# mataiyuan/ASD-SLAM

Hardware: AMD Instinct MI355X
Metric: frames/sec end-to-end tracking+LocalBA, KITTI 00 mono @2000 keypoints (higher is better)
Workload: dtype f32

## Files before the change

### asd-slam_amd/capi.py

```python
import ctypes as C
import os

import numpy as np

_HERE = os.path.dirname(os.path.abspath(__file__))


def lib_path():
    return os.environ.get("ASDHIP_LIB") or os.path.join(_HERE, "libasdhip.so")


class AsdError(RuntimeError):
    def __init__(self, code, msg):
        super().__init__(f"libasdhip error {code}: {msg}")
        self.code = code


class asd_config(C.Structure):
    _fields_ = [("n_features", C.c_int32), ("scale_factor", C.c_float), ("n_levels", C.c_int32),
                ("ini_th_fast", C.c_int32), ("min_th_fast", C.c_int32), ("max_width", C.c_int32),
                ("max_height", C.c_int32), ("max_patches", C.c_int32), ("device", C.c_int32)]


BANK_MAX_ROWS = 1 << 22
# ... 974 lines not shown
        kfs, rows, rank, fixed, pose = i32(ck), i32(cp), i32(cp), i32(cf), i32(cq)
        pfix, e_point, e_pose, e_kf, e_idx = np.full(max(cq, 1), 9, np.uint8), i32(ce), i32(ce), i32(ce), i32(ce)
        e_oct = np.full(max(ce, 1), 99, np.uint8)
        xw = np.full((max(cp, 1), 3), np.nan) if want_Xw else None
        a = asd_ba_graph_args()
        a.kf, a.n_neigh, a.neigh = int(kf), len(neigh), neigh.ctypes.data
        a.kf_capacity, a.local_kfs = ck, kfs.ctypes.data
        a.point_capacity, a.local_rows, a.point_rank = cp, rows.ctypes.data, rank.ctypes.data
        a.fixed_capacity, a.fixed_kfs = cf, fixed.ctypes.data
        a.pose_capacity, a.pose_kfs, a.pose_fixed = cq, pose.ctypes.data, pfix.ctypes.data
        a.edge_capacity, a.e_point, a.e_pose, a.e_kf, a.e_idx, a.e_octave = ce, e_point.ctypes.data, e_pose.ctypes.data, e_kf.ctypes.data, e_idx.ctypes.data, e_oct.ctypes.data
        a.Xw = None if xw is None else xw.ctypes.data
        a.n_local_kfs = a.n_points = a.n_fixed = a.n_poses = a.n_edges = -1
        rc = self.lib.asd_local_ba_graph(self.ctx, C.byref(a))
        out = dict(n_local_kfs=a.n_local_kfs, n_points=a.n_points, n_fixed=a.n_fixed, n_poses=a.n_poses, n_edges=a.n_edges)
        if rc == 0:
            out.update(local_kfs=kfs[:a.n_local_kfs].copy(), local_rows=rows[:a.n_points].copy(), point_rank=rank[:a.n_points].copy(),
                       fixed_kfs=fixed[:a.n_fixed].copy(), pose_kfs=pose[:a.n_poses].copy(), pose_fixed=pfix[:a.n_poses].copy(),
                       e_point=e_point[:a.n_edges].copy(), e_pose=e_pose[:a.n_edges].copy(), e_kf=e_kf[:a.n_edges].copy(),
                       e_idx=e_idx[:a.n_edges].copy(), e_octave=e_oct[:a.n_edges].copy())
            if want_Xw:
                out["Xw"] = xw[:a.n_points].copy()
        return rc, out

    def local_ba_graph(self, kf, neigh, want_Xw=False, caps=(64, 4096, 64, 128, 16384)):
        rc, out = self.local_ba_graph_raw(kf, neigh, caps, want_Xw)
        if rc == -5 and out["n_local_kfs"] > 0:
            rc, out = self.local_ba_graph_raw(kf, neigh, (out["n_local_kfs"], out["n_points"], out["n_fixed"], out["n_poses"], out["n_edges"]), want_Xw)
        self._chk(rc)
        return out

    def local_ba_apply_raw(self, erase, n_points, apply, bad_capacity):
        erase = _c(erase, np.uint8)
        bad, ref = np.full(max(int(bad_capacity), 1), -7, np.int32), np.full(max(int(n_points), 1), -7, np.int32)
        a = asd_ba_apply_args()
        a.n_edges, a.erase, a.apply, a.n_erased = len(erase), erase.ctypes.data, int(bool(apply)), -1
        a.bad_capacity, a.bad_rows, a.n_bad, a.n_points, a.new_ref = int(bad_capacity), bad.ctypes.data, -1, int(n_points), ref.ctypes.data
        rc = self.lib.asd_local_ba_apply(self.ctx, C.byref(a))
        out = dict(n_erased=a.n_erased, n_bad=a.n_bad)
        if rc == 0:
            out.update(bad_rows=bad[:a.n_bad].copy(), new_ref=ref[:int(n_points)].copy())
        return rc, out

    def local_ba_apply(self, erase, n_points, apply=False, bad_capacity=64):
        rc, out = self.local_ba_apply_raw(erase, n_points, apply, bad_capacity)
        if rc == -5 and out["n_bad"] > bad_capacity:
            rc, out = self.local_ba_apply_raw(erase, n_points, apply, out["n_bad"])
        self._chk(rc)
        return out

    def map_debug(self):
        out = np.zeros(8, np.int64)
        self._chk(self.lib.asd_debug_map(self.ctx, _p(out)))
        return tuple(int(x) for x in out)

    def track_local_points_map(self, slot_cur, n_cur, Tcw, K, occupied, cur_Xw, th, nn_ratio, pose7, cos_limit=0.5, obs_positive=None, split=False):
        Tcw, K, occupied, cur_Xw = _c(Tcw, np.float32), _c(K, np.float32), _c(occupied, np.uint8), _c(cur_Xw, np.float32)
        match, outl = np.empty(n_cur, np.int32), np.empty(max(n_cur, 1), np.uint8)
        pose = _c(pose7, np.float64).copy()
        n, ninl = C.c_int32(), C.c_int32()
        if split:
            self._chk(self.lib.asd_track_async(self.ctx))
        self._chk(self.lib.asd_track_local_points_map(self.ctx, slot_cur, _p(Tcw), _p(K), C.c_float(cos_limit), _p(occupied), _p(cur_Xw), C.c_float(th),
                                                      C.c_float(nn_ratio), _p(None if obs_positive is None else _c(obs_positive, np.uint8)), _p(pose),
                                                      _p(match), C.byref(n), _p(outl), C.byref(ninl)))
        if split:
            self._track_job = (match, n, pose, outl, ninl, n_cur)
            return None
        return match, n.value, pose, outl[:n_cur], ninl.value

    def bank_put(self, first_row, desc):
        desc = _c(desc, np.float32)
        self._chk(self.lib.asd_bank_put(self.ctx, first_row, desc.shape[0], _p(desc)))

    def bank_put_from_frame(self, slot, first_row, n):
        self._chk(self.lib.asd_bank_put_from_frame(self.ctx, slot, first_row, n))

    def bank_get(self, first_row, n, desc=True, attr=True):
        d = np.empty((max(n, 0), 128), np.float32) if desc else None
        a = np.empty((max(n, 0), 8), np.float32) if attr else None
        self.lib.asd_debug_bank_get.restype = C.c_int32
        self._chk(self.lib.asd_debug_bank_get(self.ctx, C.c_int32(first_row), C.c_int32(n), _p(d), _p(a)))
        return d, a

    def match_project_frame_bank(self, slot_cur, slot_last, n_cur, has_mp, Xw, mp_rows, Tcw, K, th, check_ori=True, obs_positive=None):
        has_mp, Xw, mp_rows = _c(has_mp, np.uint8), _c(Xw, np.float32), _c(mp_rows, np.int32)
        Tcw, K = _c(Tcw, np.float32), _c(K, np.float32)
        out = np.empty(n_cur, np.int32)
        n = C.c_int32()
        self._chk(self.lib.asd_match_project_frame_bank(self.ctx, slot_cur, slot_last, _p(has_mp), _p(Xw), _p(mp_rows),
                                                        _p(Tcw), _p(K), C.c_float(th), int(check_ori), _p(out), C.byref(n),
                                                        _p(None if obs_positive is None else _c(obs_positive, np.uint8))))
        return out, n.value

    def match_project_points_bank(self, slot_cur, n_cur, in_view, proj, level, view_cos, rows, occupied, th, nn_ratio, obs_positive=None):
        in_view, proj, level = _c(in_view, np.uint8), _c(proj, np.float32), _c(level, np.int32)
        view_cos, rows, occupied = _c(view_cos, np.float32), _c(rows, np.int32), _c(occupied, np.uint8)
        out = np.empty(n_cur, np.int32)
        n = C.c_int32()
        self._chk(self.lib.asd_match_project_points_bank(self.ctx, slot_cur, len(in_view), _p(in_view), _p(proj), _p(level),
                                                         _p(view_cos), _p(rows), _p(occupied), C.c_float(th),
                                                         C.c_float(nn_ratio), _p(out), C.byref(n),
                                                         _p(None if obs_positive is None else _c(obs_positive, np.uint8))))
        return out, n.value

    def frustum(self, slot_cur, Xw, normal, min_dist, max_dist, Tcw, K, cos_limit=0.5):
        Xw, normal = _c(Xw, np.float32), _c(normal, np.float32)
        min_dist, max_dist = _c(min_dist, np.float32), _c(max_dist, np.float32)
        Tcw, K = _c(Tcw, np.float32), _c(K, np.float32)
        n = Xw.shape[0]
        in_view = np.zeros(n, np.uint8)
        proj = np.zeros((n, 2), np.float32)
        level = np.zeros(n, np.int32)
        vc = np.zeros(n, np.float32)
        self._chk(self.lib.asd_frustum(self.ctx, slot_cur, n, _p(Xw), _p(normal), _p(min_dist), _p(max_dist),
                                       _p(Tcw), _p(K), C.c_float(cos_limit), _p(in_view), _p(proj), _p(level),
                                       _p(vc)))
        return in_view, proj, level, vc

    def match_init(self, slot1, slot2, prev_matched, window=100, nn_ratio=0.9, check_ori=True):
        pm = _c(prev_matched, np.float32).copy()
        out = np.empty(pm.shape[0], np.int32)
        n = C.c_int32()
        self._chk(self.lib.asd_match_init(self.ctx, slot1, slot2, _p(pm), window, C.c_float(nn_ratio),
                                          int(check_ori), _p(out), C.byref(n)))
        return out, n.value, pm

    def match_bow(self, slot_kf, slot_f, n_f, nodes_kf, nodes_f, has_mp_kf, nn_ratio=0.7, check_ori=True):
        fa, ka = make_fv(nodes_kf)
        fb, kb = make_fv(nodes_f)
        has = _c(has_mp_kf, np.uint8)
        out = np.empty(n_f, np.int32)
        n = C.c_int32()
        self._chk(self.lib.asd_match_bow(self.ctx, slot_kf, slot_f, C.byref(fa), C.byref(fb), _p(has), C.c_float(nn_ratio),
                                         int(check_ori), _p(out), C.byref(n)))
        return out, n.value

    def match_bow_kf(self, slot1, slot2, n1, nodes1, nodes2, has_mp1, has_mp2, nn_ratio=0.85, check_ori=True):
        fa, ka = make_fv(nodes1)
        fb, kb = make_fv(nodes2)
        h1, h2 = _c(has_mp1, np.uint8), _c(has_mp2, np.uint8)
        out = np.empty(n1, np.int32)
        n = C.c_int32()
        self._chk(self.lib.asd_match_bow_kf(self.ctx, slot1, slot2, C.byref(fa), C.byref(fb), _p(h1), _p(h2), C.c_float(nn_ratio),
                                            int(check_ori), _p(out), C.byref(n)))
        return out, n.value

    def match_triangulate(self, slot1, slot2, n1, nodes1, nodes2, has_mp1, has_mp2, F12, ex, ey, check_ori=False):
        fa, ka = make_fv(nodes1)
        fb, kb = make_fv(nodes2)
        h1, h2, F = _c(has_mp1, np.uint8), _c(has_mp2, np.uint8), _c(F12, np.float32)
        out = np.empty(n1, np.int32)
        n = C.c_int32()
        self._chk(self.lib.asd_match_triangulate(self.ctx, slot1, slot2, C.byref(fa), C.byref(fb), _p(h1), _p(h2), _p(F),
                                                 C.c_float(ex), C.c_float(ey), int(check_ori), _p(out), C.byref(n)))
        return out, n.value

    def pose_optimize(self, pose7, Xw, obs, inv_sigma2, K):
        pose = _c(pose7, np.float64).copy()
        Xw, obs, inv_sigma2, K = (_c(a, np.float64) for a in (Xw, obs, inv_sigma2, K))
        n = Xw.shape[0]
        outlier = np.zeros(n, np.uint8)
        ninl = C.c_int32()
        self._chk(self.lib.asd_pose_optimize(self.ctx, _p(pose), n, _p(Xw), _p(obs), _p(inv_sigma2), _p(K),
                                             _p(outlier), C.byref(ninl)))
        return pose, outlier, ninl.value
# ... 296 lines not shown
```

### asd-slam_amd/csrc/ctx.h

```cpp
#pragma once
#include <hip/hip_runtime.h>

#include <atomic>
#include <cstdarg>
#include <cstdio>
#include <cstdlib>
#include <cstring>
#include <functional>
#include <mutex>
#include <string>
#include <vector>

#include "../../include/asd_slam.h"

#define ASD_HIP_CHECK(ctx, expr)                                                          \
  do {                                                                                    \
    hipError_t _e = (expr);                                                               \
    if (_e != hipSuccess) {                                                               \
      (ctx)->set_error("%s failed: %s (%s:%d)", #expr, hipGetErrorString(_e), __FILE__, __LINE__); \
      return ASD_ERR_HIP;                                                                 \
    }                                                                                     \
  } while (0)

struct AsdPerDeviceOnce {
  std::atomic<uint64_t> bits{0};
  bool need(int dev) const { return !((bits.load(std::memory_order_acquire) >> (dev & 63)) & 1); }
  void done(int dev) { bits.fetch_or(1ull << (dev & 63), std::memory_order_release); }
};

struct AsdDevBuf {
  void* p = nullptr;
  size_t cap = 0, used = 0;
  hipError_t reserve(size_t bytes) {
    used = 0;
    if (bytes <= cap) return hipSuccess;
    if (p) (void)hipFree(p);
    p = nullptr; cap = 0;
    const size_t want = bytes + bytes / 4 + 4096;
    const hipError_t e = hipMalloc(&p, want);
    if (e == hipSuccess) cap = want;
    return e;
  }
  template <typename T> T* carve(size_t count) {
    char* q = static_cast<char*>(p) + used;
    used += (count * sizeof(T) + 255) / 256 * 256;
    return reinterpret_cast<T*>(q);
  }
  static size_t padded(size_t bytes) { return (bytes + 255) / 256 * 256; }
  void release() { if (p) (void)hipFree(p); p = nullptr; cap = used = 0; }
};


hipError_t asd_copy_rows(hipStream_t st, void* dst, const void* src, size_t bytes);

#if defined(__HIPCC__)
#define asd_syncthreads() do { asm volatile("s_waitcnt lgkmcnt(0)" ::: "memory"); __syncthreads(); } while (0)
__device__ inline int asd_syncthreads_or(int pred) { asm volatile("s_waitcnt lgkmcnt(0)" ::: "memory"); return __syncthreads_or(pred); }
#endif


struct AsdWinQuery { float x, y, r; int min_level, max_level, qrow; };
struct AsdBetweenArgs {
  int n_cur, n_last, n_cand;
  const int* match1;
  const double* io1;
  const float* Xw_last;
  const int* last_cand;
  float T_pred[16];
  uint8_t* occ;
  float* cur_Xw;
  uint8_t* skip;
  float* T1;
};
#if defined(__HIPCC__)
template <class F>
__device__ inline void asd_frustum_bank_point(const F& a, const float* T_dev, const uint8_t* skip, const int q) {
#pragma clang fp contract(off)
  AsdWinQuery Q{0.f, 0.f, 0.f, 0, 0, -1};
  const int row = a.rows[q];
  const float4 A0 = reinterpret_cast<const float4*>(a.attr)[2 * (size_t)row], A1 = reinterpret_cast<const float4*>(a.attr)[2 * (size_t)row + 1];
  a.xw_out[3 * (size_t)q] = A0.x; a.xw_out[3 * (size_t)q + 1] = A0.y; a.xw_out[3 * (size_t)q + 2] = A0.z;
  if (!skip || !skip[q]) {
    float T[16], Ow[3];
    for (int i = 0; i < 16; ++i) T[i] = T_dev[i];
    for (int i = 0; i < 3; ++i) Ow[i] = T_dev[16 + i];
    const float P[3] = {A0.x, A0.y, A0.z}, Pn[3] = {A0.w, A1.x, A1.y};
    const float min_dist = A1.z, max_dist = A1.w;
    float Pc[3];
    for (int r = 0; r < 3; ++r) {
      const float t0 = T[r * 4 + 0] * P[0] + T[r * 4 + 1] * P[1] + T[r * 4 + 2] * P[2];
      Pc[r] = (float)((double)t0 + (double)T[r * 4 + 3]);
    }
    bool ok = !(Pc[2] < 0.0f);
    const float invz = 1.0f / Pc[2];
    const float u = a.fx * Pc[0] * invz + a.cx, v = a.fy * Pc[1] * invz + a.cy;
    if (u < a.min_x || u > a.max_x || v < a.min_y || v > a.max_y) ok = false;
    const float maxD = 1.2f * max_dist, minD = 0.8f * min_dist;
    const float PO[3] = {P[0] - Ow[0], P[1] - Ow[1], P[2] - Ow[2]};
    const double nn = (double)PO[0] * PO[0] + (double)PO[1] * PO[1] + (double)PO[2] * PO[2];
    const float dist = (float)sqrt(nn);
    if (dist < minD || dist > maxD) ok = false;
    const double dot = (double)PO[0] * Pn[0] + (double)PO[1] * Pn[1] + (double)PO[2] * Pn[2];
    const float vc = (float)(dot / dist);
    if (vc < a.cos_limit) ok = false;
    if (ok) {
      const float ratio = max_dist / dist;
      int lvl = 0;
      for (int k = 1; k < a.n_levels; ++k) lvl += ratio >= a.level_thr[k];
      float r = vc > 0.998 ? 2.5f : 4.0f;
      if (a.bfactor) r *= a.th;
      Q = AsdWinQuery{u, v, r * a.scale[lvl], lvl - 1, lvl, row};
    }
  }
  a.queries[q] = Q;
}
__device__ inline void asd_between_body(const AsdBetweenArgs& a_dev, const int t, const int nt) {
#pragma clang fp contract(off)
  const AsdBetweenArgs a = a_dev;
  __shared__ int s_nmatch;
  if (t == 0) s_nmatch = 0;
  for (int c = t; c < a.n_cand; c += nt) a.skip[c] = 0;
  asd_syncthreads();
  const uint8_t* outl = reinterpret_cast<const uint8_t*>(a.io1 + 8);
  int mine = 0;
  for (int j = t; j < a.n_cur; j += nt) {
    const int i = a.match1[j];
    mine += i >= 0;
    const int src = i >= 0 ? i : 0;
    for (int k = 0; k < 3; ++k) a.cur_Xw[3 * (size_t)j + k] = a.n_last > 0 ? a.Xw_last[3 * (size_t)src + k] : 0.f;
    const bool keep = i >= 0 && !outl[j];
    a.occ[j] = keep ? 1 : 0;
    if (i >= 0 && a.last_cand) { const int c = a.last_cand[i]; if (c >= 0 && c < a.n_cand) a.skip[c] = 1; }
  }
  if (mine) atomicAdd(&s_nmatch, mine);
  asd_syncthreads();
  if (t == 0) {
    float T[16];
    if (s_nmatch >= 3) {
      const double* p = a.io1;
      const double x = p[0], y = p[1], z = p[2], w = p[3];
      const double tx = 2 * x, ty = 2 * y, tz = 2 * z;
      const double twx = tx * w, twy = ty * w, twz = tz * w, txx = tx * x, txy = ty * x, txz = tz * x, tyy = ty * y, tyz = tz * y, tzz = tz * z;
      const double R[9] = {1 - (tyy + tzz), txy - twz, txz + twy, txy + twz, 1 - (txx + tzz), tyz - twx, txz - twy, tyz + twx, 1 - (txx + tyy)};
      for (int i = 0; i < 3; ++i) {
        for (int j = 0; j < 3; ++j) T[i * 4 + j] = (float)R[i * 3 + j];
        T[i * 4 + 3] = (float)p[4 + i];
      }
      T[12] = T[13] = T[14] = 0.f;
      T[15] = 1.f;
    } else {
      for (int i = 0; i < 16; ++i) T[i] = a.T_pred[i];
    }
    for (int i = 0; i < 16; ++i) a.T1[i] = T[i];
    for (int i = 0; i < 3; ++i) {
      double sum = 0;
      for (int k = 0; k < 3; ++k) sum += (double)T[k * 4 + i] * (double)T[k * 4 + 3];
      a.T1[16 + i] = (float)(-1.0 * sum);
    }
  }
}
#endif

struct AsdXfer {
  char* h = nullptr;
  char* d = nullptr;
  size_t cap = 0, used = 0;
  hipError_t begin(hipStream_t st, size_t bytes) {
    used = 0;
    bytes += 4096;
    if (bytes <= cap) return hipSuccess;
    if (h) { (void)hipStreamSynchronize(st); (void)hipHostFree(h); (void)hipFree(d); }
    h = nullptr; d = nullptr; cap = 0;
    const size_t want = bytes + bytes / 2;
    hipError_t e = hipHostMalloc(&h, want);
    if (e == hipSuccess) e = hipMalloc(&d, want);
    if (e == hipSuccess) cap = want;
    return e;
  }
  size_t reserve(size_t bytes) { const size_t off = used; used += (bytes + 255) / 256 * 256; return off; }
  size_t add(const void* src, size_t bytes) { const size_t off = reserve(bytes); memcpy(h + off, src, bytes); return off; }
  size_t zeros(size_t bytes) { const size_t off = reserve(bytes); memset(h + off, 0, bytes); return off; }
  hipError_t upload(hipStream_t st) {
    if (!used) return hipSuccess;
    static const bool by_kernel = getenv("ASD_UPLOAD_COPY") == nullptr;
    return by_kernel ? asd_copy_rows(st, d, h, (used + 15) / 16 * 16) : hipMemcpyAsync(d, h, used, hipMemcpyHostToDevice, st);
  }
  hipError_t download(hipStream_t st) { return used ? hipMemcpyAsync(h, d, used, hipMemcpyDeviceToHost, st) : hipSuccess; }
  template <typename T> T* dev(size_t off) { return reinterpret_cast<T*>(d + off); }
  template <typename T> T* host(size_t off) { return reinterpret_cast<T*>(h + off); }
  void release() { if (h) (void)hipHostFree(h); if (d) (void)hipFree(d); h = d = nullptr; cap = used = 0; }
};

struct AsdFrameSlot {
  int n = 0;
  float min_x = 0, max_x = 0, min_y = 0, max_y = 0;
  float inv_w = 0, inv_h = 0;
  std::vector<asd_keypoint> kps;
// ... 192 lines not shown
```

### asd-slam_amd/csrc/matcher.h

```cpp
#pragma once
#include <chrono>
#include <vector>

#include "ctx.h"

using WinQuery = AsdWinQuery;

struct MatcherState {
  int q_cap = 0, cand_cap = 0, h_cand_cap = 0, qdesc_cap = 0;
  int last_total[4] = {1 << 15, 1 << 15, 1 << 15, 1 << 15};
  WinQuery *d_queries = nullptr, *h_queries = nullptr;
  int *d_q_off = nullptr, *d_q_cnt = nullptr, *d_total = nullptr, *d_idx = nullptr;
  float* d_dist = nullptr;
  int *h_q = nullptr;
  int* h_idx = nullptr;
  float* h_dist = nullptr;
  float *d_qdesc = nullptr, *h_qdesc = nullptr;
  float* d_bank = nullptr;
  int bank_cap = 0;
  float* d_attr = nullptr;
  int attr_cap = 0;
  float* d_cxw = nullptr;
  size_t cxw_cap = 0;
  float* h_attr[2] = {nullptr, nullptr};
  size_t h_attr_cap[2] = {0, 0};
  hipEvent_t ev_attr[2] = {nullptr, nullptr};
  int attr_turn = 0;
  bool replay_host = false;
};

struct SearchResult { const int* off; const int* cnt; const int* idx; const float* dist; };

struct ListQuery { int qrow, cbeg, cend, ooff; };

MatcherState* matcher_state(asd_ctx* ctx);
AsdFrameSlot* matcher_slot(asd_ctx* ctx, int s);
int matcher_ensure_queries(asd_ctx* ctx, MatcherState* m, int nq);
int matcher_ensure_qdesc(asd_ctx* ctx, MatcherState* m, int n);
int matcher_upload_qdesc(asd_ctx* ctx, MatcherState* m, const float* desc, int n);
int matcher_window_search(asd_ctx* ctx, MatcherState* m, const AsdFrameSlot& F, int nq, const float* d_q, SearchResult* res, int kind = 3);
int matcher_list_search(asd_ctx* ctx, MatcherState* m, const AsdFrameSlot& A, const AsdFrameSlot& B, const asd_feature_vector* fvA,
                        const asd_feature_vector* fvB, const uint8_t* skipA, bool skip_if_set, std::vector<ListQuery>& lq, const float** dist_out);

int matcher_check_bank_rows(asd_ctx* ctx, const MatcherState* m, const int32_t* rows, const uint8_t* used, int n, bool attr_too);

int matcher_replay_frame(asd_ctx* ctx, MatcherState* m, const AsdFrameSlot& C, const AsdFrameSlot& L, const float* d_q, const uint8_t* obs_pos,
                         int check_orientation, int32_t* match_cur, int32_t* n_matches, std::chrono::steady_clock::time_point tm0);
int matcher_replay_points(asd_ctx* ctx, MatcherState* m, const AsdFrameSlot& F, int n_mp, const float* d_q, const uint8_t* occupied,
                          const uint8_t* obs_pos, float nn_ratio, int32_t* match_cur, int32_t* n_matches);

template <class Make>
int matcher_fill_queries(asd_ctx* ctx, MatcherState* m, int n, Make make) {
  const int rc = matcher_ensure_queries(ctx, m, n);
  if (rc != ASD_OK) return rc;
  for (int i = 0; i < n; ++i) {
    WinQuery& Q = m->h_queries[i];
    Q = WinQuery{0.f, 0.f, 0.f, 0, 0, -1};
    make(i, Q);
  }
  return ASD_OK;
}
inline void matcher_transform(const float* T, const float* X, float* out) {
  for (int r = 0; r < 3; ++r) {
    const float t0 = T[r * 4 + 0] * X[0] + T[r * 4 + 1] * X[1] + T[r * 4 + 2] * X[2];
    out[r] = (float)((double)t0 + (double)T[r * 4 + 3]);
  }
}
inline void matcher_camera_centre(const float* R, int ld, const float* t, int inc, float* Ow) {
  for (int i = 0; i < 3; ++i) {
    double sum = 0;
    for (int k = 0; k < 3; ++k) sum += (double)R[k * ld + i] * (double)t[k * inc];
    Ow[i] = (float)(-1.0 * sum);
  }
}
inline void matcher_keyframe_centre(const float* Tcw, float* Ow) {
  for (int i = 0; i < 3; ++i) {
    const float t0 = Tcw[0 * 4 + i] * Tcw[3] + Tcw[1 * 4 + i] * Tcw[7] + Tcw[2 * 4 + i] * Tcw[11];
    Ow[i] = (float)((double)t0 * -1.0);
  }
}
```

### asd-slam_amd/csrc/matcher.hip

```cpp
#include <algorithm>
#include <chrono>
#include <cmath>
#include <cstring>
#include <array>
#include <functional>
#include <memory>

#include "matcher.h"
#include "resolve2.h"

namespace {

constexpr int GC = ASD_GRID_COLS, GR = ASD_GRID_ROWS;

struct GridDev {
  const float4* kp;
  const int* cell_start;
  const int* cell_items;
  float min_x, min_y, inv_w, inv_h;
};

#ifndef ASD_SEARCH_WAVES
#define ASD_SEARCH_WAVES 8
#endif
constexpr int kSearchWaves = ASD_SEARCH_WAVES;
constexpr int kSearchCols = 16;
constexpr int kSearchList = 128;
struct SortArgs {
  const uint8_t* occ;
  float th_cut;
  uint16_t* top_idx;
};
template <bool SORT>
__global__ __launch_bounds__(64 * kSearchWaves) void k_window_search(GridDev G, const WinQuery* __restrict__ queries, int nq,
                                                       const float* __restrict__ qdesc, const float* __restrict__ cdesc,
                                                       int* __restrict__ q_off, int* __restrict__ q_cnt,
                                                       int* __restrict__ total, int cap, int* __restrict__ out_idx,
                                                       float* __restrict__ out_dist, SortArgs S) {
  const int lane = threadIdx.x & 63, wave = threadIdx.x >> 6;
  const int q = blockIdx.x * kSearchWaves + wave;
  __shared__ int wg_cnt[kSearchWaves], wg_base;
  __shared__ int cand_l[kSearchWaves][kSearchList];
  __shared__ unsigned dist_l[SORT ? kSearchWaves : 1][kSearchList];
  const bool live = q < nq;
  const WinQuery Q = live ? queries[q] : WinQuery{0.f, 0.f, 0.f, 0, 0, -1};
  int cnt = 0, off = 0;
  bool empty = Q.qrow < 0;
  const int nMinCellX = max(0, (int)floorf((Q.x - G.min_x - Q.r) * G.inv_w));
  const int nMaxCellX = min(ASD_GRID_COLS - 1, (int)ceilf((Q.x - G.min_x + Q.r) * G.inv_w));
  const int nMinCellY = max(0, (int)floorf((Q.y - G.min_y - Q.r) * G.inv_h));
  const int nMaxCellY = min(ASD_GRID_ROWS - 1, (int)ceilf((Q.y - G.min_y + Q.r) * G.inv_h));
  if (nMinCellX >= ASD_GRID_COLS || nMaxCellX < 0 || nMinCellY >= ASD_GRID_ROWS || nMaxCellY < 0) empty = true;
  const bool check = (Q.min_level > 0) || (Q.max_level >= 0);
  auto accept = [&](const float4& kp) {
    const int oct = __float_as_int(kp.z);
    bool ok = true;
    if (check) {
      if (oct < Q.min_level) ok = false;
      if (Q.max_level >= 0 && oct > Q.max_level) ok = false;
    }
    const float dx = kp.x - Q.x, dy = kp.y - Q.y;
    if (!(fabsf(dx) < Q.r && fabsf(dy) < Q.r)) ok = false;
    return ok;
  };
  const int qrow_u = __builtin_amdgcn_readfirstlane(Q.qrow < 0 ? 0 : Q.qrow);
  auto distance = [&](int idx) {
    const float4* a = reinterpret_cast<const float4*>(qdesc + (size_t)qrow_u * 128);
    const float4* bb = reinterpret_cast<const float4*>(cdesc + (size_t)idx * 128);
    float sqd = 0.f;
#pragma unroll 16
    for (int k = 0; k < 32; ++k) {
      const float4 x = a[k], y = bb[k];
      float d;
      d = x.x - y.x; sqd = sqd + d * d;
      d = x.y - y.y; sqd = sqd + d * d;
      d = x.z - y.z; sqd = sqd + d * d;
      d = x.w - y.w; sqd = sqd + d * d;
    }
    return sqd;
  };
  auto score = [&](int idx, int p) {
    const float sqd = distance(idx);
    out_idx[off + p] = idx;
    out_dist[off + p] = sqd;
  };
  auto walk = [&](int pass) {
    int pos = 0;
    for (int ix = nMinCellX; ix <= nMaxCellX; ++ix) {
      const int b = G.cell_start[ix * ASD_GRID_ROWS + nMinCellY], e = G.cell_start[ix * ASD_GRID_ROWS + nMaxCellY + 1];
      for (int base = b; base < e; base += 64) {
        const int it = base + lane;
        bool ok = false;
        int idx = 0;
        if (it < e) {
          idx = G.cell_items[it];
          ok = accept(G.kp[idx]);
          if (SORT && ok && S.occ && S.occ[idx]) ok = false;
        }
        const unsigned long long m = __ballot(ok);
        if (pass == 1 && ok) {
          const int p = pos + __popcll(m & ((1ull << lane) - 1));
          if (off + p < cap) score(idx, p);
        }
        pos += __popcll(m);
      }
    }
    return pos;
  };
  const int ncol = nMaxCellX - nMinCellX + 1;
  bool fast = !empty && ncol <= kSearchCols;
  int cb[kSearchCols], ce[kSearchCols];
  if (fast) {
#pragma unroll
    for (int c = 0; c < kSearchCols; ++c) {
      const int ix = min(nMinCellX + c, nMaxCellX);
      cb[c] = G.cell_start[ix * ASD_GRID_ROWS + nMinCellY];
      ce[c] = G.cell_start[ix * ASD_GRID_ROWS + nMaxCellY + 1];
    }
#pragma unroll
    for (int c = 0; c < kSearchCols; ++c) {
      if (c >= ncol) ce[c] = cb[c];
      if (ce[c] - cb[c] > 64) fast = false;
    }
  }
  if (fast) {
    int idxc[kSearchCols];
#pragma unroll
    for (int c = 0; c < kSearchCols; ++c) idxc[c] = cb[c] + lane < ce[c] ? G.cell_items[cb[c] + lane] : -1;
    float4 kpc[kSearchCols];
#pragma unroll
    for (int c = 0; c < kSearchCols; ++c) kpc[c] = idxc[c] >= 0 ? G.kp[idxc[c]] : make_float4(0.f, 0.f, 0.f, 0.f);
    if (SORT && S.occ) {
      uint8_t oc[kSearchCols];
#pragma unroll
      for (int c = 0; c < kSearchCols; ++c) oc[c] = idxc[c] >= 0 ? S.occ[idxc[c]] : (uint8_t)0;
#pragma unroll
      for (int c = 0; c < kSearchCols; ++c) if (oc[c]) idxc[c] = -1;
    }
    int pos = 0;
#pragma unroll
    for (int c = 0; c < kSearchCols; ++c) {
      const bool ok = idxc[c] >= 0 && accept(kpc[c]);
      const unsigned long long m = __ballot(ok);
      if (ok) {
        const int p = pos + __popcll(m & ((1ull << lane) - 1));
        if (p < kSearchList) cand_l[wave][p] = idxc[c];
      }
      pos += __popcll(m);
    }
    cnt = pos;
    if (cnt > kSearchList) fast = false;
  } else if (!empty) {
    cnt = walk(0);
  }
  if (lane == 0) wg_cnt[wave] = cnt;
  asd_syncthreads();
  if (threadIdx.x == 0) {
    int sum = 0;
    for (int w = 0; w < kSearchWaves; ++w) sum += wg_cnt[w];
    wg_base = sum ? atomicAdd(total, sum) : 0;
  }
  asd_syncthreads();
  off = wg_base;
  for (int w = 0; w < wave; ++w) off += wg_cnt[w];
  if (!SORT) {
    if (cnt > 0) {
      if (fast) {
        for (int p = lane; p < cnt; p += 64)
          if (off + p < cap) score(cand_l[wave][p], p);
      } else {
        (void)walk(1);
      }
    }
    if (lane == 0 && live) { q_cnt[q] = cnt; q_off[q] = cnt ? off : 0; }
    return;
  }
  if (!live) return;
  const bool fits = off + cnt <= cap;
  int n_keep = 0, s_off = off;
  auto put = [&](int base, int rank, int idx, float d) {
    out_idx[base + rank] = idx;
    out_dist[base + rank] = d;
    if (rank < kTop) S.top_idx[(size_t)q * kTop + rank] = (uint16_t)idx;
  };
  if (cnt > 0 && fits) {
    if (fast) {
      const bool v0 = lane < cnt, v1 = lane + 64 < cnt;
      const int i0 = v0 ? cand_l[wave][lane] : 0, i1 = v1 ? cand_l[wave][lane + 64] : 0;
      const float d0 = v0 ? distance(i0) : 0.f, d1 = v1 ? distance(i1) : 0.f;
      const unsigned b0 = __float_as_uint(d0), b1 = __float_as_uint(d1);
      if (v0) dist_l[wave][lane] = b0;
      if (v1) dist_l[wave][lane + 64] = b1;
      asm volatile("s_waitcnt lgkmcnt(0)" ::: "memory");
      __builtin_amdgcn_wave_barrier();
      int r0 = 0, r1 = 0;
      for (int i = 0; i < cnt; ++i) {
        const unsigned di = dist_l[wave][i];
        r0 += (di < b0) || (di == b0 && i < lane);
        r1 += (di < b1) || (di == b1 && i < lane + 64);
      }
      if (v0) put(off, r0, i0, d0);
      if (v1) put(off, r1, i1, d1);
      n_keep = __popcll(__ballot(v0 && d0 <= S.th_cut)) + __popcll(__ballot(v1 && d1 <= S.th_cut));
    } else {
      (void)walk(1);
      asm volatile("s_waitcnt vmcnt(0)" ::: "memory");
      __builtin_amdgcn_fence(__ATOMIC_SEQ_CST, "workgroup");
      s_off = cap + off;
      constexpr int R = 4;
      for (int pb = 0; pb < cnt; pb += 64 * R) {
        int pi[R], ii[R], rk[R]; unsigned bi[R];
#pragma unroll
        for (int r = 0; r < R; ++r) {
          pi[r] = pb + 64 * r + lane;
          const int pc = min(pi[r], cnt - 1);
          ii[r] = __hip_atomic_load(out_idx + off + pc, __ATOMIC_RELAXED, __HIP_MEMORY_SCOPE_AGENT);
          bi[r] = __float_as_uint(__hip_atomic_load(out_dist + off + pc, __ATOMIC_RELAXED, __HIP_MEMORY_SCOPE_AGENT));
          rk[r] = 0;
        }
        for (int cbase = 0; cbase < cnt; cbase += kSearchList) {
          __builtin_amdgcn_wave_barrier();
          for (int i = lane; i < kSearchList; i += 64)
            dist_l[wave][i] = cbase + i < cnt ? __float_as_uint(__hip_atomic_load(out_dist + off + cbase + i, __ATOMIC_RELAXED, __HIP_MEMORY_SCOPE_AGENT)) : 0xffffffffu;
          asm volatile("s_waitcnt lgkmcnt(0)" ::: "memory");
          __builtin_amdgcn_wave_barrier();
          const int m = min(kSearchList, cnt - cbase);
          for (int i = 0; i < m; ++i) {
            const unsigned di = dist_l[wave][i];
#pragma unroll
            for (int r = 0; r < R; ++r) rk[r] += (di < bi[r]) || (di == bi[r] && cbase + i < pi[r]);
          }
          asm volatile("s_waitcnt lgkmcnt(0)" ::: "memory");
        }
#pragma unroll
        for (int r = 0; r < R; ++r) {
          const bool v = pi[r] < cnt;
          if (v) put(s_off, rk[r], ii[r], __uint_as_float(bi[r]));
          n_keep += __popcll(__ballot(v && __uint_as_float(bi[r]) <= S.th_cut));
        }
      }
    }
  }
  if (lane < kTop && lane >= (fits ? cnt : 0)) S.top_idx[(size_t)q * kTop + lane] = 0xffffu;
  if (lane == 0) { q_cnt[q] = n_keep; q_off[q] = cnt ? s_off : 0; }
}

__global__ __launch_bounds__(256) void k_list_dist(const ListQuery* __restrict__ queries, int nq,
                                                   const int* __restrict__ cand, const float* __restrict__ qdesc,
                                                   const float* __restrict__ cdesc, float* __restrict__ out) {
  const int lane = threadIdx.x & 63;
  const int q = blockIdx.x * 4 + (threadIdx.x >> 6);
  if (q >= nq) return;
  const ListQuery Q = queries[q];
  const float4* a = reinterpret_cast<const float4*>(qdesc + (size_t)Q.qrow * 128);
  for (int t = Q.cbeg + lane; t < Q.cend; t += 64) {
    const float4* b = reinterpret_cast<const float4*>(cdesc + (size_t)cand[t] * 128);
    float sqd = 0.f;
#pragma unroll 8
    for (int k = 0; k < 32; ++k) {
      const float4 x = a[k], y = b[k];
      float d;
      d = x.x - y.x; sqd = sqd + d * d;
      d = x.y - y.y; sqd = sqd + d * d;
      d = x.z - y.z; sqd = sqd + d * d;
      d = x.w - y.w; sqd = sqd + d * d;
    }
    out[Q.ooff + (t - Q.cbeg)] = sqd;
  }
}

constexpr int kDistinctMax = 64;
__global__ __launch_bounds__(256) void k_distinctive(const float* __restrict__ desc, const int* __restrict__ set_start, int* __restrict__ best_out) {
  extern __shared__ __attribute__((aligned(16))) float smem_d[];
  const int s0 = set_start[blockIdx.x], n = set_start[blockIdx.x + 1] - s0;
  float* sd = smem_d;
  float* D = smem_d + kDistinctMax * 132;
  float* med = D + kDistinctMax * (kDistinctMax + 1);
// ... 11 lines not shown
      const float4* y = reinterpret_cast<const float4*>(sd + j * 132);
      for (int k = 0; k < 32; ++k) {
        const float4 a = x[k], b = y[k];
        float d;
        d = a.x - b.x; acc = acc + d * d;
        d = a.y - b.y; acc = acc + d * d;
        d = a.z - b.z; acc = acc + d * d;
        d = a.w - b.w; acc = acc + d * d;
      }
    }
    D[i * (n + 1) + j] = acc;
  }
  asd_syncthreads();
  const int kth = (int)(0.5 * (n - 1));
  for (int p = t; p < n * n; p += 256) {
    const int i = p / n, j = p % n;
    const float v = D[i * (n + 1) + j];
    int rank = 0;
    for (int l = 0; l < n; ++l) {
      const float u = D[i * (n + 1) + l];
      rank += (u < v || (u == v && l < j)) ? 1 : 0;
    }
    if (rank == kth) med[i] = v;
  }
  asd_syncthreads();
  if (t == 0) {
    float best_median = 100;
    int best = 0;
    for (int i = 0; i < n; ++i)
      if (med[i] < best_median) { best_median = med[i]; best = i; }
    best_out[blockIdx.x] = best;
  }
}

__global__ __launch_bounds__(256) void k_dist_matrix(const float* __restrict__ a, int na, const float* __restrict__ b,
                                                     int nb, float* __restrict__ out) {
  __shared__ float4 sa[16][32];
  const int j = blockIdx.x * 256 + threadIdx.x;
  const int i0 = blockIdx.y * 16;
  for (int idx = threadIdx.x; idx < 16 * 32; idx += 256) {
    const int r = idx >> 5, c = idx & 31;
    const int ia = min(i0 + r, na - 1);
    sa[r][c] = reinterpret_cast<const float4*>(a + (size_t)ia * 128)[c];
  }
  asd_syncthreads();
  const float4* brow = reinterpret_cast<const float4*>(b + (size_t)min(j, nb - 1) * 128);
  float acc[16];
#pragma unroll
  for (int r = 0; r < 16; ++r) acc[r] = 0.f;
  for (int k = 0; k < 32; ++k) {
    const float4 y = brow[k];
#pragma unroll
    for (int r = 0; r < 16; ++r) {
      const float4 x = sa[r][k];
      float d;
      d = x.x - y.x; acc[r] = acc[r] + d * d;
      d = x.y - y.y; acc[r] = acc[r] + d * d;
      d = x.z - y.z; acc[r] = acc[r] + d * d;
      d = x.w - y.w; acc[r] = acc[r] + d * d;
    }
  }
  if (j < nb)
    for (int r = 0; r < 16; ++r)
      if (i0 + r < na) out[(size_t)(i0 + r) * nb + j] = acc[r];
}


__global__ __launch_bounds__(256) void k_copy16(const uint4* __restrict__ src, uint4* __restrict__ dst, size_t n16) {
  for (size_t i = (size_t)blockIdx.x * 256 + threadIdx.x; i < n16; i += (size_t)gridDim.x * 256) dst[i] = src[i];
}
hipError_t copy_rows(hipStream_t st, void* dst, const void* src, size_t bytes) {
  const size_t n16 = bytes / 16;
  if (!n16) return hipSuccess;
  hipLaunchKernelGGL(k_copy16, dim3((unsigned)std::min<size_t>((n16 + 255) / 256, 1024)), dim3(256), 0, st, static_cast<const uint4*>(src),
                     static_cast<uint4*>(dst), n16);
  return hipGetLastError();
}

template <int KIND, int QPT>
__global__ __launch_bounds__(kResolve2Threads) void k_resolve2(Resolve2Args a) {
  resolve2_body<KIND, QPT, kResolve2Threads>(a);
}

struct UploadTail {
  const uint4* src; uint4* dst;
  size_t first16, n16;
  int q_blocks;
};
__device__ inline bool upload_tail_block(const UploadTail& u) {
  if ((int)blockIdx.x < u.q_blocks) return false;
  const size_t nb = gridDim.x - u.q_blocks;
  for (size_t i = u.first16 + (size_t)(blockIdx.x - u.q_blocks) * 256 + threadIdx.x; i < u.n16; i += nb * 256) u.dst[i] = u.src[i];
  return true;
}
constexpr int kUploadTailBlocks = 64;

struct FrustumArgs {
  int n, n_levels, bfactor;
  const float* Xw; const float* normal; const float* min_dist; const float* max_dist;
  const int* rows;
  float T[16], Ow[3];
  float fx, fy, cx, cy, min_x, max_x, min_y, max_y, cos_limit, th;
  float level_thr[ASD_MAX_LEVELS], scale[ASD_MAX_LEVELS];
  WinQuery* queries;
  UploadTail up;
  const float* T_dev; const float* attr; const uint8_t* skip; float* xw_out;
};
__global__ __launch_bounds__(256) void k_frustum_queries(FrustumArgs a) {
  if (upload_tail_block(a.up)) return;
  const int q = blockIdx.x * 256 + threadIdx.x;
  if (q >= a.n) return;
  WinQuery Q{0.f, 0.f, 0.f, 0, 0, -1};
  if (a.attr) {
    if (a.T_dev) asd_frustum_bank_point(a, a.T_dev, a.skip, q);
    else {
      float Tl[19];
      for (int i = 0; i < 16; ++i) Tl[i] = a.T[i];
      for (int i = 0; i < 3; ++i) Tl[16 + i] = a.Ow[i];
      asd_frustum_bank_point(a, Tl, a.skip, q);
    }
    return;
  }
  const float* P = a.Xw + 3 * (size_t)q;
  float Pc[3];
  for (int r = 0; r < 3; ++r) {
    const float t0 = a.T[r * 4 + 0] * P[0] + a.T[r * 4 + 1] * P[1] + a.T[r * 4 + 2] * P[2];
    Pc[r] = (float)((double)t0 + (double)a.T[r * 4 + 3]);
  }
  bool ok = !(Pc[2] < 0.0f);
  const float invz = 1.0f / Pc[2];
  const float u = a.fx * Pc[0] * invz + a.cx, v = a.fy * Pc[1] * invz + a.cy;
  if (u < a.min_x || u > a.max_x || v < a.min_y || v > a.max_y) ok = false;
  const float maxD = 1.2f * a.max_dist[q], minD = 0.8f * a.min_dist[q];
  const float PO[3] = {P[0] - a.Ow[0], P[1] - a.Ow[1], P[2] - a.Ow[2]};
  const double nn = (double)PO[0] * PO[0] + (double)PO[1] * PO[1] + (double)PO[2] * PO[2];
  const float dist = (float)sqrt(nn);
  if (dist < minD || dist > maxD) ok = false;
  const float* Pn = a.normal + 3 * (size_t)q;
  const double dot = (double)PO[0] * Pn[0] + (double)PO[1] * Pn[1] + (double)PO[2] * Pn[2];
  const float vc = (float)(dot / dist);
  if (vc < a.cos_limit) ok = false;
  if (ok) {
    const float ratio = a.max_dist[q] / dist;
    int lvl = 0;
    for (int k = 1; k < a.n_levels; ++k) lvl += ratio >= a.level_thr[k];
    float r = vc > 0.998 ? 2.5f : 4.0f;
    if (a.bfactor) r *= a.th;
    Q = WinQuery{u, v, r * a.scale[lvl], lvl - 1, lvl, a.rows ? a.rows[q] : q};
  }
  a.queries[q] = Q;
}

struct ProjectArgs {
  int n;
  const uint8_t* has_mp; const float* Xw; const int* rows; const float4* kp_last;
  float T[16];
  float fx, fy, cx, cy, min_x, max_x, min_y, max_y, th;
  float scale[ASD_MAX_LEVELS];
  WinQuery* queries;
  UploadTail up;
};
__global__ __launch_bounds__(256) void k_project_queries(ProjectArgs a) {
  if (upload_tail_block(a.up)) return;
  const int i = blockIdx.x * 256 + threadIdx.x;
  if (i >= a.n) return;
  WinQuery Q{0.f, 0.f, 0.f, 0, 0, -1};
  if (a.has_mp[i]) {
    const float* X = a.Xw + 3 * (size_t)i;
    float Xc[3];
    for (int r = 0; r < 3; ++r) {
      const float t0 = a.T[r * 4 + 0] * X[0] + a.T[r * 4 + 1] * X[1] + a.T[r * 4 + 2] * X[2];
      Xc[r] = (float)((double)t0 + (double)a.T[r * 4 + 3]);
    }
    const float invzc = (float)(1.0 / (double)Xc[2]);
    if (!(invzc < 0)) {
      const float u = a.fx * Xc[0] * invzc + a.cx;
      const float v = a.fy * Xc[1] * invzc + a.cy;
      if (!(u < a.min_x || u > a.max_x) && !(v < a.min_y || v > a.max_y)) {
        const int oct = __float_as_int(a.kp_last[i].z);
        Q = WinQuery{u, v, a.th * a.scale[oct], oct - 1, oct + 1, a.rows ? a.rows[i] : i};
      }
    }
  }
  a.queries[i] = Q;
}

int ensure_cands_dev(asd_ctx* ctx, MatcherState* m, size_t n) {
  if (n <= (size_t)m->cand_cap) return ASD_OK;
  if (n > ((size_t)1 << 30)) { ctx->set_error("candidate buffers: %zu entries asked for", n); return ASD_ERR_CAPACITY; }
  const size_t cap = std::max(n + n / 2, (size_t)1 << 18);
  if (m->d_idx) { (void)hipFree(m->d_idx); (void)hipFree(m->d_dist); }
  m->d_idx = nullptr; m->d_dist = nullptr;
  m->cand_cap = 0;
  ASD_HIP_CHECK(ctx, hipMalloc(&m->d_idx, 2 * cap * sizeof(int)));
  ASD_HIP_CHECK(ctx, hipMalloc(&m->d_dist, 2 * cap * sizeof(float)));
  m->cand_cap = (int)std::min(cap, (size_t)0x7fffffff);
  return ASD_OK;
}
int ensure_cands(asd_ctx* ctx, MatcherState* m, int n) {
  int rc = ensure_cands_dev(ctx, m, (size_t)n);
  if (rc != ASD_OK) return rc;
  if (m->cand_cap <= m->h_cand_cap) return ASD_OK;
  if (m->h_idx) { (void)hipHostFree(m->h_idx); (void)hipHostFree(m->h_dist); }
  m->h_idx = nullptr; m->h_dist = nullptr;
  m->h_cand_cap = 0;
  ASD_HIP_CHECK(ctx, hipHostMalloc(&m->h_idx, (size_t)m->cand_cap * sizeof(int)));
  ASD_HIP_CHECK(ctx, hipHostMalloc(&m->h_dist, (size_t)m->cand_cap * sizeof(float)));
  m->h_cand_cap = m->cand_cap;
  return ASD_OK;
}
}

MatcherState* matcher_state(asd_ctx* ctx) {
  if (!ctx->matcher) {
    MatcherState* m = new MatcherState();
    m->replay_host = ctx->match_replay_host;
    ctx->matcher = m;
  }
  return static_cast<MatcherState*>(ctx->matcher);
}

int matcher_ensure_queries(asd_ctx* ctx, MatcherState* m, int nq) {
  if (nq <= m->q_cap) return ASD_OK;
  const int cap = std::max(nq * 3 / 2, 8192);
  if (m->d_queries) { (void)hipFree(m->d_queries); (void)hipHostFree(m->h_queries); (void)hipFree(m->d_q_off); (void)hipHostFree(m->h_q); }
  m->q_cap = 0;
  ASD_HIP_CHECK(ctx, hipMalloc(&m->d_queries, (size_t)cap * sizeof(WinQuery)));
  ASD_HIP_CHECK(ctx, hipHostMalloc(&m->h_queries, (size_t)cap * sizeof(WinQuery)));
  ASD_HIP_CHECK(ctx, hipMalloc(&m->d_q_off, ((size_t)2 * cap + 4) * sizeof(int)));
  ASD_HIP_CHECK(ctx, hipHostMalloc(&m->h_q, ((size_t)2 * cap + 4) * sizeof(int)));
  m->q_cap = cap;
  return ASD_OK;
}
int matcher_ensure_qdesc(asd_ctx* ctx, MatcherState* m, int n) {
  if (n <= m->qdesc_cap) return ASD_OK;
  const int cap = std::max(n * 3 / 2, 8192);
  if (m->d_qdesc) { (void)hipFree(m->d_qdesc); (void)hipHostFree(m->h_qdesc); }
  m->qdesc_cap = 0;
  ASD_HIP_CHECK(ctx, hipMalloc(&m->d_qdesc, (size_t)cap * 512));
  ASD_HIP_CHECK(ctx, hipHostMalloc(&m->h_qdesc, (size_t)cap * 512));
  m->qdesc_cap = cap;
  return ASD_OK;
}

int matcher_upload_qdesc(asd_ctx* ctx, MatcherState* m, const float* desc, int n) {
  int rc = matcher_ensure_qdesc(ctx, m, n);
  if (rc != ASD_OK) return rc;
  memcpy(m->h_qdesc, desc, (size_t)n * 512);
  ASD_HIP_CHECK(ctx, hipMemcpyAsync(m->d_qdesc, m->h_qdesc, (size_t)n * 512, hipMemcpyHostToDevice, ctx->stream));
  return ASD_OK;
}

AsdFrameSlot* matcher_slot(asd_ctx* ctx, int s) {
  if (!ctx || s < 0 || s >= ASD_MAX_FRAMES) return nullptr;
  return &ctx->frames[s];
}

int matcher_window_search(asd_ctx* ctx, MatcherState* m, const AsdFrameSlot& F, int nq, const float* d_q, SearchResult* res, int kind) {
  if (asd_track_busy(ctx, "matcher call")) return ASD_ERR_INVALID;
  static const bool timing = getenv("ASD_TIMING") != nullptr;
  static double tacc[4][3]; static long tcalls[4];
  const auto tw0 = std::chrono::steady_clock::now();
  auto tw1 = tw0;
  int rc = ensure_cands(ctx, m, 1);
  if (rc != ASD_OK) return rc;
  hipStream_t st = ctx->stream;
  int* d_off = m->d_q_off;
  int* d_cnt = m->d_q_off + nq;
  int* d_total = m->d_q_off + 2 * nq;
  const int optimistic = std::min(m->cand_cap, std::max(4096, m->last_total[kind] + m->last_total[kind] / 4));
  for (int attempt = 0; attempt < 2; ++attempt) {
    ASD_HIP_CHECK(ctx, hipMemcpyAsync(m->d_queries, m->h_queries, (size_t)nq * sizeof(WinQuery), hipMemcpyHostToDevice, st));
    ASD_HIP_CHECK(ctx, hipMemsetAsync(d_total, 0, sizeof(int), st));
    GridDev G{F.d_kp, F.d_cell_start, F.d_cell_items, F.min_x, F.min_y, F.inv_w, F.inv_h};
    ASD_HIP_CHECK(ctx, hipEventRecord(ctx->ev0, st));
    hipLaunchKernelGGL(k_window_search<false>, dim3((nq + kSearchWaves - 1) / kSearchWaves), dim3(64 * kSearchWaves), 0, st, G, m->d_queries, nq, d_q, F.d_desc, d_off, d_cnt,
                       d_total, m->cand_cap, m->d_idx, m->d_dist, SortArgs{});
    ASD_HIP_CHECK(ctx, hipGetLastError());
    ASD_HIP_CHECK(ctx, hipEventRecord(ctx->ev1, st));
    ASD_HIP_CHECK(ctx, hipMemcpyAsync(m->h_q, d_off, ((size_t)2 * nq + 1) * sizeof(int), hipMemcpyDeviceToHost, st));
    ASD_HIP_CHECK(ctx, hipMemcpyAsync(m->h_idx, m->d_idx, (size_t)optimistic * sizeof(int), hipMemcpyDeviceToHost, st));
    ASD_HIP_CHECK(ctx, hipMemcpyAsync(m->h_dist, m->d_dist, (size_t)optimistic * sizeof(float), hipMemcpyDeviceToHost, st));
    tw1 = std::chrono::steady_clock::now();
    ASD_HIP_CHECK(ctx, hipStreamSynchronize(st));
    const int total = m->h_q[2 * nq];
    m->last_total[kind] = total;
    if (total > m->cand_cap) {
      if ((rc = ensure_cands(ctx, m, total)) != ASD_OK) return rc;
      continue;
    }
    if (total > optimistic) {
      ASD_HIP_CHECK(ctx, hipMemcpyAsync(m->h_idx + optimistic, m->d_idx + optimistic, (size_t)(total - optimistic) * sizeof(int), hipMemcpyDeviceToHost, st));
      ASD_HIP_CHECK(ctx, hipMemcpyAsync(m->h_dist + optimistic, m->d_dist + optimistic, (size_t)(total - optimistic) * sizeof(float), hipMemcpyDeviceToHost, st));
      ASD_HIP_CHECK(ctx, hipStreamSynchronize(st));
    }
    break;
  }
  ASD_HIP_CHECK(ctx, hipEventElapsedTime(&ctx->ms_match, ctx->ev0, ctx->ev1));
  if (timing) {
    const auto tw2 = std::chrono::steady_clock::now();
    auto ms = [](auto a, auto b) { return std::chrono::duration<double, std::milli>(b - a).count(); };
    tacc[kind][0] += ms(tw0, tw1); tacc[kind][1] += ms(tw1, tw2); tacc[kind][2] += ctx->ms_match;
    if (++tcalls[kind] % 200 == 0)
      fprintf(stderr, "[window_search kind %d] enqueue %.3f sync %.3f kernel %.3f ms, %d candidates copied (last total %d)\n", kind,
              tacc[kind][0] / tcalls[kind], tacc[kind][1] / tcalls[kind], tacc[kind][2] / tcalls[kind], optimistic, m->last_total[kind]);
  }
  res->off = m->h_q;
  res->cnt = m->h_q + nq;
  res->idx = m->h_idx;
  res->dist = m->h_dist;
  return ASD_OK;
}

namespace {
size_t resolve_lds_bytes(int kind, int n_cur, int nq) {
  return resolve2_fixed_lds(kind, n_cur) + (size_t)n_cur * 4 + (kind == 1 ? ((size_t)nq * 2 + 15) / 16 * 16 : 0);
}
bool replay_on_device(const MatcherState* m, int kind, int n_cur, int nq) {
  const int max_q = kind == 0 ? kResolve2Threads * 4 : std::min(kResolve2MaxRounds * 512, 65535);
  return !m->replay_host && n_cur > 0 && n_cur < 65536 && nq <= max_q && resolve_lds_bytes(kind, n_cur, nq) <= 96 * 1024;
}

struct StageSolver {
  const float* d_points;
  const uint8_t* d_hold;
  const float* d_own;
  double pose0[7];
  const double* d_pose0;
  double K[4];
  double* io;
  double* d_io_dev;
  const AsdBetweenArgs* d_between;
};
enum QuerySource { kQueriesUploaded, kQueriesProject, kQueriesFrustum };
enum StageUpload { kUploadElsewhere, kUploadCopy, kUploadCarried };
struct TrackStage {
  int kind, nq;
  const AsdFrameSlot* F;
  QuerySource source;
  ProjectArgs project;
  FrustumArgs frustum;
  StageUpload upload;
  const WinQuery* d_queries;
  const float* d_qdesc;
  const float4* kp_last;
  const uint8_t* d_obs_pos;
  const uint8_t* d_occupied;
  int check_ori;
  float nn_ratio;
  int *d_off, *d_cnt;
  int* d_total;
  uint16_t* d_top;
  int *d_out, *h_out;
  bool timed;
  bool has_solver;
  StageSolver solver;
};

UploadTail upload_tail(const AsdXfer& up, int nq, bool carried) {
  return UploadTail{reinterpret_cast<const uint4*>(up.h), reinterpret_cast<uint4*>(up.d), carried ? ((size_t)nq * sizeof(WinQuery) + 255) / 256 * 16 : 0,
                    carried ? (up.used + 15) / 16 : 0, (nq + 255) / 256};
}

ProjectArgs project_args(const asd_ctx* ctx, const AsdFrameSlot& C, const AsdFrameSlot& L, const float* Tcw, const float* K, float th) {
  ProjectArgs pa{};
  pa.n = L.n; pa.kp_last = L.d_kp;
  memcpy(pa.T, Tcw, sizeof pa.T);
  pa.fx = K[0]; pa.fy = K[1]; pa.cx = K[2]; pa.cy = K[3];
  pa.min_x = C.min_x; pa.max_x = C.max_x; pa.min_y = C.min_y; pa.max_y = C.max_y; pa.th = th;
  for (int l = 0; l < ASD_MAX_LEVELS; ++l) pa.scale[l] = l < ctx->cfg.n_levels ? ctx->scale[l] : 0.f;
  return pa;
}
FrustumArgs frustum_args(const asd_ctx* ctx, const AsdFrameSlot& F, int n, const float* Tcw, const float* T_dev, const float* K, float cos_limit, float th) {
  FrustumArgs fa{};
  fa.n = n; fa.n_levels = ctx->cfg.n_levels; fa.bfactor = th != 1.0;
  if (Tcw) {
    memcpy(fa.T, Tcw, sizeof fa.T);
    matcher_camera_centre(Tcw, 4, Tcw + 3, 4, fa.Ow);
  }
  fa.T_dev = T_dev;
  fa.fx = K[0]; fa.fy = K[1]; fa.cx = K[2]; fa.cy = K[3];
  fa.min_x = F.min_x; fa.max_x = F.max_x; fa.min_y = F.min_y; fa.max_y = F.max_y;
  fa.cos_limit = cos_limit; fa.th = th;
  for (int l = 0; l < ASD_MAX_LEVELS; ++l) { fa.level_thr[l] = ctx->level_thr[l]; fa.scale[l] = l < ctx->cfg.n_levels ? ctx->scale[l] : 0.f; }
  return fa;
}
size_t resolve2_args(const MatcherState* m, const TrackStage& s, Resolve2Args* out) {
  const int n_cur = s.F->n;
  Resolve2Args a{};
  a.nq = s.nq; a.n_cur = n_cur;
  a.q_off = s.d_off; a.q_cnt = s.d_cnt; a.idx = m->d_idx; a.dist = m->d_dist; a.top_idx = s.d_top;
  a.total = s.d_total; a.cap = m->cand_cap;
  a.obs_pos = s.d_obs_pos;
  a.kp_cur = s.F->d_kp; a.kp_last = s.kp_last;
  a.check_ori = s.check_ori; a.nn_ratio = s.nn_ratio;
  a.match_cur = s.d_out; a.n_matches = s.d_out + n_cur; a.mirror = s.h_out;
  const size_t fixed = resolve_lds_bytes(s.kind, n_cur, s.nq), per = s.kind == 1 ? 6 : 2;
  a.stage_cap = (int)std::min<size_t>(((size_t)m->last_total[s.kind] * 5 / 4 + 1023) / 1024 * 1024, ((size_t)96 * 1024 - fixed) / per / 8 * 8);
  *out = a;
  return fixed + (size_t)a.stage_cap * per;
}
int resolve2_attributes(asd_ctx* ctx) {
  static AsdPerDeviceOnce attrs;
  if (!attrs.need(ctx->cfg.device)) return ASD_OK;
  const void* ks[] = {reinterpret_cast<const void*>(k_resolve2<0, 2>), reinterpret_cast<const void*>(k_resolve2<0, 4>),
                      reinterpret_cast<const void*>(k_resolve2<1, 2>), reinterpret_cast<const void*>(k_resolve2<1, 4>)};
  for (const void* k : ks) ASD_HIP_CHECK(ctx, hipFuncSetAttribute(k, hipFuncAttributeMaxDynamicSharedMemorySize, 96 * 1024));
  attrs.done(ctx->cfg.device);
  return ASD_OK;
}
hipError_t launch_resolve2(hipStream_t st, int kind, const Resolve2Args& a, size_t lds) {
  auto go = [&](auto kern) { hipLaunchKernelGGL(kern, dim3(1), dim3(kResolve2Threads), lds, st, a); };
  const bool two = a.nq <= 2 * kResolve2Threads;
  if (kind == 0) { if (two) go(k_resolve2<0, 2>); else go(k_resolve2<0, 4>); }
  else { if (two) go(k_resolve2<1, 2>); else go(k_resolve2<1, 4>); }
  return hipGetLastError();
}
bool stage_fuses(const asd_ctx* ctx, const MatcherState* m, const TrackStage& s) {
  Resolve2Args a;
  return s.has_solver && pose_chain_fused_ok(ctx, s.kind, s.nq, s.F->n, resolve2_args(m, s, &a));
}

int enqueue_stage(asd_ctx* ctx, const MatcherState* m, const TrackStage& s, bool fuse) {
  hipStream_t st = ctx->stream;
  const AsdFrameSlot& F = *s.F;
  int rc;
  if (s.upload == kUploadCopy) ASD_HIP_CHECK(ctx, ctx->up.upload(st));
  if (s.source == kQueriesProject) {
    const UploadTail& t = s.project.up;
    hipLaunchKernelGGL(k_project_queries, dim3(t.q_blocks + (t.n16 ? kUploadTailBlocks : 0)), dim3(256), 0, st, s.project);
    ASD_HIP_CHECK(ctx, hipGetLastError());
  } else if (s.source == kQueriesFrustum) {
    const UploadTail& t = s.frustum.up;
    hipLaunchKernelGGL(k_frustum_queries, dim3(t.q_blocks + (t.n16 ? kUploadTailBlocks : 0)), dim3(256), 0, st, s.frustum);
    ASD_HIP_CHECK(ctx, hipGetLastError());
  }
  if (s.timed) ASD_HIP_CHECK(ctx, hipEventRecord(ctx->ev0, st));
  const GridDev G{F.d_kp, F.d_cell_start, F.d_cell_items, F.min_x, F.min_y, F.inv_w, F.inv_h};
  const SortArgs sa{s.d_occupied, s.kind == 0 ? TH_HIGH : __builtin_huge_valf(), s.d_top};
  hipLaunchKernelGGL(k_window_search<true>, dim3((s.nq + kSearchWaves - 1) / kSearchWaves), dim3(64 * kSearchWaves), 0, st, G, s.d_queries, s.nq, s.d_qdesc, F.d_desc, s.d_off,
                     s.d_cnt, s.d_total, m->cand_cap, m->d_idx, m->d_dist, sa);
  ASD_HIP_CHECK(ctx, hipGetLastError());
  Resolve2Args ra;
  const size_t lds = resolve2_args(m, s, &ra);
  if (!fuse) {
    ASD_HIP_CHECK(ctx, launch_resolve2(st, s.kind, ra, lds));
    if (s.timed) ASD_HIP_CHECK(ctx, hipEventRecord(ctx->ev1, st));
  }
  if (s.has_solver) {
    const StageSolver& v = s.solver;
    const AsdFusedReplay fr{&ra, s.kind, s.nq, lds};
    AsdPoseChainArgs c{};
    c.n_cur = F.n; c.d_match = s.d_out; c.d_kp = F.d_kp;
    c.d_points = v.d_points; c.d_hold = v.d_hold; c.d_own = v.d_own;
    c.pose7 = v.d_pose0 ? nullptr : v.pose0; c.K = v.K;
    c.d_io = v.io; c.d_pose0 = v.d_pose0; c.d_io_dev = v.d_io_dev; c.between = v.d_between;
    c.fused = fuse ? &fr : nullptr;
    if ((rc = pose_chain_enqueue(ctx, c)) != ASD_OK) return rc;
  }
  if (fuse && s.timed) ASD_HIP_CHECK(ctx, hipEventRecord(ctx->ev1, st));
  return ASD_OK;
}
int record_chain_end(asd_ctx* ctx) {
  if (!ctx->ev_chain) ASD_HIP_CHECK(ctx, hipEventCreateWithFlags(&ctx->ev_chain, hipEventDisableTiming));
  ASD_HIP_CHECK(ctx, hipEventRecord(ctx->ev_chain, ctx->stream));
  return ASD_OK;
}

void unpack_solver_block(const double* h_io, int n_cur, bool kp_flags, const int32_t* match, const uint8_t* hold, const double* pose_start, double* pose,
                         uint8_t* outlier, int32_t* n_inliers) {
  int ne = 0;
  if (kp_flags) {
    ne = (int)(h_io[8 + (n_cur + 7) / 8] + 0.5);
    memcpy(outlier, h_io + 8, (size_t)n_cur);
  } else {
    auto edge = [&](int j) { return (hold && hold[j]) || match[j] >= 0; };
    for (int j = 0; j < n_cur; ++j) ne += edge(j);
    const uint8_t* flags = reinterpret_cast<const uint8_t*>(h_io + 8);
    for (int j = 0, e = 0; j < n_cur; ++j) outlier[j] = edge(j) && ne >= 3 ? flags[e++] : 0;
  }
  memcpy(pose, ne < 3 ? pose_start : h_io, 56);
  *n_inliers = ne < 3 ? 0 : ne - (int)(h_io[7] + 0.5);
}

struct StageInputs {
  int kind = 0, nq = 0;
  const float* d_qdesc = nullptr;
  const float4* kp_last = nullptr;
  const uint8_t* obs_pos = nullptr;
  const uint8_t* occupied = nullptr;
  int check_ori = 0;
  float nn_ratio = 0.f;
  QuerySource source = kQueriesUploaded;
  ProjectArgs project{};
  FrustumArgs frustum{};
  bool has_solver = false;
  double pose0[7] = {}, K[4] = {};
  const float* points = nullptr;
  int n_points = 0;
  const float* d_points = nullptr;
  const uint8_t* has_mp = nullptr;
  const float* own = nullptr;
  const uint8_t* hold = nullptr;
  const float* normal = nullptr;
  const float* min_dist = nullptr;
  const float* max_dist = nullptr;
  const int32_t* rows = nullptr;
  const int32_t* d_rows = nullptr;
};

int search_and_resolve(asd_ctx* ctx, MatcherState* m, const AsdFrameSlot& F, const StageInputs& in, int32_t* match_cur, int32_t* n_matches,
                       const double** solver_io = nullptr, std::function<int()>* defer = nullptr) {
  if (asd_track_busy(ctx, "matcher call")) return ASD_ERR_INVALID;
  static const bool timing = getenv("ASD_TIMING") != nullptr;
  static const bool tail_upload = getenv("ASD_UPLOAD_COPY") == nullptr;
  const int n_cur = F.n, nq = in.nq, kind = in.kind;
  const bool deferred = defer != nullptr;
  int rc = ensure_cands_dev(ctx, m, deferred ? std::max((size_t)nq * (size_t)std::max(n_cur, 1), (size_t)1) : (size_t)1);
  if (rc != ASD_OK) return rc;
  hipStream_t st = ctx->stream;
  AsdXfer &up = ctx->up, &down = ctx->down;
  const size_t io_bytes = in.has_solver ? pose_chain_io_bytes(n_cur) : 0;
  ASD_HIP_CHECK(ctx, up.begin(st, (size_t)nq * (sizeof(WinQuery) + 1 + 12 + 12 + 4 + 4 + 4) + (size_t)in.n_points * 12 + (size_t)n_cur * (1 + 12 + 1) + 16 * 256));
  ASD_HIP_CHECK(ctx, down.begin(st, ((size_t)n_cur + 16) * sizeof(int) + 256 + io_bytes));
  ASD_HIP_CHECK(ctx, ctx->scratch.reserve(AsdDevBuf::padded((size_t)nq * kTop * 2)));
  if ((rc = resolve2_attributes(ctx)) != ASD_OK || (in.has_solver && (rc = pose_chain_reserve(ctx, n_cur)) != ASD_OK)) return rc;

  TrackStage s{};
  s.kind = kind; s.nq = nq; s.F = &F;
  s.source = in.source;
  s.upload = in.source != kQueriesUploaded && tail_upload ? kUploadCarried : kUploadCopy;
  s.d_qdesc = in.d_qdesc; s.kp_last = in.kp_last; s.check_ori = in.check_ori; s.nn_ratio = in.nn_ratio;
  s.d_off = m->d_q_off; s.d_cnt = m->d_q_off + nq;
  s.d_top = ctx->scratch.carve<uint16_t>((size_t)nq * kTop);
  s.timed = timing;
  const size_t o_q = in.source == kQueriesUploaded ? up.add(m->h_queries, (size_t)nq * sizeof(WinQuery)) : up.reserve((size_t)nq * sizeof(WinQuery));
  const size_t o_total = up.zeros(sizeof(int));
  s.d_queries = up.dev<WinQuery>(o_q);
  s.d_total = up.dev<int>(o_total);
  if (in.obs_pos) s.d_obs_pos = up.dev<uint8_t>(up.add(in.obs_pos, nq));
  if (kind == 1) s.d_occupied = up.dev<uint8_t>(up.add(in.occupied, n_cur));
  const bool carried = s.upload == kUploadCarried;
  const void *q_points = nullptr, *q_has = nullptr, *q_normal = nullptr, *q_min = nullptr, *q_max = nullptr, *q_rows = nullptr;
  auto table = [&](const void* src, size_t bytes, const void** for_query) -> const void* {
    if (!src) return nullptr;
    const size_t o = up.add(src, bytes);
    if (for_query) *for_query = carried ? up.host<void>(o) : up.dev<void>(o);
    return up.dev<void>(o);
  };
  const void* d_points = table(in.points, (size_t)in.n_points * 12, &q_points);
  (void)table(in.has_mp, nq, &q_has);
  const void* d_own = table(in.own, (size_t)n_cur * 12, nullptr);
  const void* d_hold = table(in.hold, n_cur, nullptr);
  (void)table(in.normal, (size_t)nq * 12, &q_normal);
  (void)table(in.min_dist, (size_t)nq * 4, &q_min);
  (void)table(in.max_dist, (size_t)nq * 4, &q_max);
  if (in.d_rows) q_rows = in.d_rows;
  else (void)table(in.rows, (size_t)nq * 4, &q_rows);
  if (in.source == kQueriesProject) {
    s.project = in.project;
    s.project.Xw = static_cast<const float*>(q_points); s.project.has_mp = static_cast<const uint8_t*>(q_has); s.project.rows = static_cast<const int*>(q_rows);
    s.project.queries = up.dev<WinQuery>(o_q);
    s.project.up = upload_tail(up, nq, carried);
  } else if (in.source == kQueriesFrustum) {
    s.frustum = in.frustum;
    s.frustum.Xw = static_cast<const float*>(q_points); s.frustum.normal = static_cast<const float*>(q_normal);
    s.frustum.min_dist = static_cast<const float*>(q_min); s.frustum.max_dist = static_cast<const float*>(q_max);
    s.frustum.rows = static_cast<const int*>(q_rows);
    s.frustum.queries = up.dev<WinQuery>(o_q);
    s.frustum.up = upload_tail(up, nq, carried);
  }
  const size_t o_out = down.reserve(((size_t)n_cur + 16) * sizeof(int));
  s.d_out = down.dev<int>(o_out); s.h_out = down.host<int>(o_out);
  s.has_solver = in.has_solver;
  if (in.has_solver) {
    StageSolver& v = s.solver;
    v.d_points = in.d_points ? in.d_points : static_cast<const float*>(d_points);
    v.d_hold = static_cast<const uint8_t*>(d_hold); v.d_own = static_cast<const float*>(d_own);
    memcpy(v.pose0, in.pose0, sizeof v.pose0); memcpy(v.K, in.K, sizeof v.K);
    v.io = down.host<double>(down.reserve(io_bytes));
    if (solver_io) *solver_io = v.io;
  }
  int* const h_total = up.host<int>(o_total);
  const int* const h_out = s.h_out;

  auto attempt = [ctx, m, s]() -> int {
    const int rc = enqueue_stage(ctx, m, s, stage_fuses(ctx, m, s));
    return rc != ASD_OK ? rc : record_chain_end(ctx);
  };

  auto complete = [=]() -> int {
    int rc;
    for (int round = 0;; ++round) {
      ASD_HIP_CHECK(ctx, hipEventSynchronize(ctx->ev_chain));
      const int total = h_out[n_cur + 1];
      m->last_total[kind] = total;
      if (total > m->cand_cap && deferred) {
        ctx->set_error("asd_track_finish: %d candidates overflowed the %d-entry buffers of a deferred stage", total, m->cand_cap);
        return ASD_ERR_CAPACITY;
      }
      if (total > m->cand_cap && round == 0) {
        if ((rc = ensure_cands_dev(ctx, m, (size_t)total)) != ASD_OK) return rc;
        *h_total = 0;
        if ((rc = attempt()) != ASD_OK) return rc;
        continue;
      }
      break;
    }
    if (timing) ASD_HIP_CHECK(ctx, hipEventElapsedTime(&ctx->ms_match, ctx->ev0, ctx->ev1));
    else ctx->ms_match = 0.f;
    memcpy(match_cur, h_out, (size_t)n_cur * sizeof(int));
    *n_matches = h_out[n_cur];
    if (timing) {
      static double acc[2]; static long calls[2]; static long rounds[2]; static double st_us[2][8];
      acc[kind] += ctx->ms_match; rounds[kind] += h_out[n_cur + 2];
      for (int i = 0; i < 8; ++i) st_us[kind][i] += 0.01 * h_out[n_cur + 3 + i];
      if (++calls[kind] % 200 == 0)
        fprintf(stderr, "[search+resolve kind %d] device %.3f ms, %.1f iterations, %d candidates; replay: staging %.1f us, iterations %.1f us (the first %.1f; thread 0 work %.1f, barrier + verdict %.1f), outputs %.1f us\n", kind,
                acc[kind] / calls[kind], (double)rounds[kind] / calls[kind], h_out[n_cur + 1], st_us[kind][0] / calls[kind], st_us[kind][1] / calls[kind],
                st_us[kind][3] / calls[kind], st_us[kind][4] / calls[kind], st_us[kind][5] / calls[kind], st_us[kind][2] / calls[kind]);
    }
    return ASD_OK;
  };

  if ((rc = attempt()) != ASD_OK) return rc;
  if (defer) { *defer = complete; return ASD_OK; }
  return complete();
}

}

hipError_t asd_copy_rows(hipStream_t st, void* dst, const void* src, size_t bytes) { return copy_rows(st, dst, src, bytes); }

void matcher_free(asd_ctx* ctx) {
  if (ctx->matcher && static_cast<MatcherState*>(ctx->matcher)->d_cxw) (void)hipFree(static_cast<MatcherState*>(ctx->matcher)->d_cxw);
  for (auto& f : ctx->frames) {
    if (f.d_desc) (void)hipFree(f.d_desc);
    if (f.d_fv) (void)hipFree(f.d_fv);
    f.d_fv = nullptr;
    if (f.d_kp) (void)hipFree(f.d_kp);
    if (f.h_stage) (void)hipHostFree(f.h_stage);
    if (f.ev_staged) (void)hipEventDestroy(f.ev_staged);
    f.ev_staged = nullptr;
    f.d_desc = nullptr; f.d_kp = nullptr; f.d_cell_start = nullptr; f.d_cell_items = nullptr; f.h_stage = nullptr;
  }
  if (ctx->matcher) {
    MatcherState* m = static_cast<MatcherState*>(ctx->matcher);
    void* dev[] = {m->d_queries, m->d_q_off, m->d_idx, m->d_dist, m->d_qdesc, m->d_bank, m->d_attr};
    for (void* p : dev) if (p) (void)hipFree(p);
    void* host[] = {m->h_queries, m->h_q, m->h_idx, m->h_dist, m->h_qdesc, m->h_attr[0], m->h_attr[1]};
    for (void* p : host) if (p) (void)hipHostFree(p);
    for (hipEvent_t e : m->ev_attr) if (e) (void)hipEventDestroy(e);
    delete m;
    ctx->matcher = nullptr;
  }
}

extern "C" {

static int frame_set_impl(asd_ctx* ctx, int32_t slot, const asd_keypoint* kps, const float* desc, int32_t n, float min_x,
                          float max_x, float min_y, float max_y, asd_ctx* src);
int asd_frame_set(asd_ctx* ctx, int32_t slot, const asd_keypoint* kps, const float* desc, int32_t n, float min_x,
                  float max_x, float min_y, float max_y) {
  return frame_set_impl(ctx, slot, kps, desc, n, min_x, max_x, min_y, max_y, ctx);
}
int asd_frame_set_from_ctx(asd_ctx* ctx, int32_t slot, const asd_keypoint* kps, int32_t n, float min_x, float max_x, float min_y, float max_y,
                           asd_ctx* src) {
  if (!ctx || !src || src->cfg.device != ctx->cfg.device) return ASD_ERR_INVALID;
  return frame_set_impl(ctx, slot, kps, nullptr, n, min_x, max_x, min_y, max_y, src);
}
static int frame_set_impl(asd_ctx* ctx, int32_t slot, const asd_keypoint* kps, const float* desc, int32_t n, float min_x,
                          float max_x, float min_y, float max_y, asd_ctx* src) {
  AsdFrameSlot* F = matcher_slot(ctx, slot);
  if (!F || n < 0 || (n > 0 && !kps) || !(max_x > min_x) || !(max_y > min_y)) return ASD_ERR_INVALID;
  if (n > ctx->cfg.max_patches) { ctx->set_error("frame has %d keypoints, capacity %d", n, ctx->cfg.max_patches); return ASD_ERR_CAPACITY; }
  if (!desc && !src->d_desc_last) { ctx->set_error("desc == NULL: no extraction has completed on the source context yet"); return ASD_ERR_INVALID; }
  if (!desc && n != src->last_n) { ctx->set_error("desc == NULL adopts the last extract (%d keypoints), got n=%d", src->last_n, n); return ASD_ERR_INVALID; }
  (void)hipSetDevice(ctx->cfg.device);
  const size_t cap = ctx->cfg.max_patches;
  if (!F->d_desc) {
    ASD_HIP_CHECK(ctx, hipMalloc(&F->d_desc, cap * 128 * sizeof(float)));
    char* blk = nullptr;
    ASD_HIP_CHECK(ctx, hipMalloc(&blk, cap * (sizeof(float4) + sizeof(int)) + (GC * GR + 1) * sizeof(int) + 16));
    F->d_kp = reinterpret_cast<float4*>(blk);
    F->d_cell_start = reinterpret_cast<int32_t*>(blk + cap * sizeof(float4));
    F->d_cell_items = F->d_cell_start + (GC * GR + 1);
    ASD_HIP_CHECK(ctx, hipHostMalloc(&F->h_stage, cap * (sizeof(float4) + sizeof(int)) + (GC * GR + 1) * sizeof(int) + 16));
    ASD_HIP_CHECK(ctx, hipEventCreateWithFlags(&F->ev_staged, hipEventDisableTiming));
  } else {
    ASD_HIP_CHECK(ctx, hipEventSynchronize(F->ev_staged));
  }
  hipStream_t st = asd_prep_stream(ctx);
  if (n > 0) {
    if (desc) ASD_HIP_CHECK(ctx, hipMemcpyAsync(F->d_desc, desc, (size_t)n * 128 * sizeof(float), hipMemcpyHostToDevice, st));
    else ASD_HIP_CHECK(ctx, copy_rows(st, F->d_desc, src->d_desc_last, (size_t)n * 128 * sizeof(float)));
  }
  F->n = n;
  F->min_x = min_x; F->max_x = max_x; F->min_y = min_y; F->max_y = max_y;
  F->inv_w = static_cast<float>(GC) / static_cast<float>(max_x - min_x);
  F->inv_h = static_cast<float>(GR) / static_cast<float>(max_y - min_y);
  F->kps.assign(kps, kps + n);
  std::vector<int> cell(n);
  F->cell_start.assign(GC * GR + 1, 0);
  for (int i = 0; i < n; ++i) {
    const int px = (int)std::round((kps[i].x - min_x) * F->inv_w);
    const int py = (int)std::round((kps[i].y - min_y) * F->inv_h);
    if (px < 0 || px >= GC || py < 0 || py >= GR) { cell[i] = -1; continue; }
    cell[i] = px * GR + py;
    ++F->cell_start[cell[i] + 1];
  }
  for (int c = 0; c < GC * GR; ++c) F->cell_start[c + 1] += F->cell_start[c];
  F->cell_items.assign(F->cell_start[GC * GR], 0);
  std::vector<int> cur(F->cell_start.begin(), F->cell_start.end() - 1);
  for (int i = 0; i < n; ++i)
    if (cell[i] >= 0) F->cell_items[cur[cell[i]]++] = i;
  float4* hk = reinterpret_cast<float4*>(F->h_stage);
  int* hs = reinterpret_cast<int*>(F->h_stage + cap * sizeof(float4));
  int* hi = hs + (GC * GR + 1);
  for (int i = 0; i < n; ++i) {
    float ob;
    memcpy(&ob, &kps[i].octave, sizeof ob);
    hk[i] = make_float4(kps[i].x, kps[i].y, ob, kps[i].angle);
  }
  memcpy(hs, F->cell_start.data(), (GC * GR + 1) * sizeof(int));
  if (!F->cell_items.empty()) memcpy(hi, F->cell_items.data(), F->cell_items.size() * sizeof(int));
  {
    static const bool by_kernel = getenv("ASD_UPLOAD_COPY") == nullptr;
    const size_t bytes = cap * sizeof(float4) + (GC * GR + 1 + F->cell_items.size()) * sizeof(int);
    if (by_kernel) ASD_HIP_CHECK(ctx, copy_rows(st, F->d_kp, hk, (bytes + 15) / 16 * 16));
    else ASD_HIP_CHECK(ctx, hipMemcpyAsync(F->d_kp, hk, bytes, hipMemcpyHostToDevice, st));
  }
  ASD_HIP_CHECK(ctx, hipEventRecord(F->ev_staged, st));
  if (!desc && n > 0) {
    if (!src->ev_adopt) ASD_HIP_CHECK(ctx, hipEventCreateWithFlags(&src->ev_adopt, hipEventDisableTiming));
    ASD_HIP_CHECK(ctx, hipEventRecord(src->ev_adopt, st));
    src->adopt_pending = true;
  } else {
    ASD_HIP_CHECK(ctx, hipStreamSynchronize(st));
  }
  return ASD_OK;
}

int asd_dist_matrix(asd_ctx* ctx, const float* a, int32_t na, const float* b, int32_t nb, float* out) {
  if (!ctx || na < 0 || nb < 0 || ((na > 0 && nb > 0) && (!a || !b || !out))) return ASD_ERR_INVALID;
  if (na == 0 || nb == 0) return ASD_OK;
  if (asd_track_busy(ctx, "asd_dist_matrix")) return ASD_ERR_INVALID;
  (void)hipSetDevice(ctx->cfg.device);
  float *da = nullptr, *db = nullptr, *dout = nullptr;
  hipStream_t st = ctx->stream;
  ASD_HIP_CHECK(ctx, ctx->scratch.reserve(AsdDevBuf::padded((size_t)na * 512) + AsdDevBuf::padded((size_t)nb * 512) +
                                          AsdDevBuf::padded((size_t)na * nb * sizeof(float))));
  da = ctx->scratch.carve<float>((size_t)na * 128);
  db = ctx->scratch.carve<float>((size_t)nb * 128);
  dout = ctx->scratch.carve<float>((size_t)na * nb);
  ASD_HIP_CHECK(ctx, hipMemcpyAsync(da, a, (size_t)na * 512, hipMemcpyHostToDevice, st));
  ASD_HIP_CHECK(ctx, hipMemcpyAsync(db, b, (size_t)nb * 512, hipMemcpyHostToDevice, st));
  ASD_HIP_CHECK(ctx, hipEventRecord(ctx->ev0, st));
  hipLaunchKernelGGL(k_dist_matrix, dim3((nb + 255) / 256, (na + 15) / 16), dim3(256), 0, st, da, na, db, nb, dout);
  ASD_HIP_CHECK(ctx, hipGetLastError());
  ASD_HIP_CHECK(ctx, hipEventRecord(ctx->ev1, st));
  ASD_HIP_CHECK(ctx, hipMemcpyAsync(out, dout, (size_t)na * nb * sizeof(float), hipMemcpyDeviceToHost, st));
  ASD_HIP_CHECK(ctx, hipStreamSynchronize(st));
  ASD_HIP_CHECK(ctx, hipEventElapsedTime(&ctx->ms_match, ctx->ev0, ctx->ev1));
  return ASD_OK;
}

int asd_distinctive_descriptor(asd_ctx* ctx, const float* desc, int32_t n, int32_t* best_idx) {
  if (!ctx || !desc || !best_idx || n < 1) return ASD_ERR_INVALID;
  std::vector<float> D((size_t)n * n);
  int rc = asd_dist_matrix(ctx, desc, n, desc, n, D.data());
  if (rc != ASD_OK) return rc;
  float best_median = 100;
  int best = 0;
  std::vector<float> row(n);
  for (int i = 0; i < n; ++i) {
    std::copy(D.begin() + (size_t)i * n, D.begin() + (size_t)(i + 1) * n, row.begin());
    row[i] = 0;
    std::sort(row.begin(), row.end());
    const float median = row[(size_t)(0.5 * (n - 1))];
    if (median < best_median) { best_median = median; best = i; }
  }
  *best_idx = best;
  return ASD_OK;
}

int asd_distinctive_descriptor_batch(asd_ctx* ctx, int32_t n_sets, const int32_t* set_start, const float* desc, int32_t* best_idx) {
  if (!ctx || n_sets < 0 || (n_sets > 0 && (!set_start || !desc || !best_idx))) return ASD_ERR_INVALID;
  if (n_sets == 0) return ASD_OK;
  if (set_start[0] != 0) { ctx->set_error("asd_distinctive_descriptor_batch: set_start[0] must be 0"); return ASD_ERR_INVALID; }
  bool any_big = false;
  for (int s = 0; s < n_sets; ++s) {
    const int n = set_start[s + 1] - set_start[s];
    if (n < 1) { ctx->set_error("asd_distinctive_descriptor_batch: set %d is empty", s); return ASD_ERR_INVALID; }
    any_big |= n > kDistinctMax;
  }
  (void)hipSetDevice(ctx->cfg.device);
  hipStream_t st = ctx->stream;
  const int total = set_start[n_sets];
  hipError_t e = ctx->scratch.reserve(AsdDevBuf::padded((size_t)total * 512) + 2 * AsdDevBuf::padded((size_t)(n_sets + 1) * sizeof(int)));
  float* dd = ctx->scratch.carve<float>((size_t)total * 128);
  int* ds = ctx->scratch.carve<int>((size_t)n_sets + 1);
  int* db = ctx->scratch.carve<int>((size_t)n_sets + 1);
  if (e == hipSuccess) e = hipMemcpyAsync(dd, desc, (size_t)total * 512, hipMemcpyHostToDevice, st);
  if (e == hipSuccess) e = hipMemcpyAsync(ds, set_start, (size_t)(n_sets + 1) * sizeof(int), hipMemcpyHostToDevice, st);
  if (e == hipSuccess) e = hipMemsetAsync(db, 0, (size_t)n_sets * sizeof(int), st);
  if (e == hipSuccess) {
    static AsdPerDeviceOnce attr;
    const size_t lds = (size_t)(kDistinctMax * 132 + kDistinctMax * (kDistinctMax + 1) + kDistinctMax) * sizeof(float);
    if (attr.need(ctx->cfg.device)) { (void)hipFuncSetAttribute(reinterpret_cast<const void*>(k_distinctive), hipFuncAttributeMaxDynamicSharedMemorySize, (int)lds); attr.done(ctx->cfg.device); }
    for (int s = 0; s < n_sets;) {
      if (set_start[s + 1] - set_start[s] > kDistinctMax) { ++s; continue; }
      int r = s;
      while (r < n_sets && set_start[r + 1] - set_start[r] <= kDistinctMax) ++r;
      hipLaunchKernelGGL(k_distinctive, dim3(r - s), dim3(256), lds, st, dd, ds + s, db + s);
      s = r;
    }
    e = hipGetLastError();
  }
  if (e == hipSuccess) e = hipMemcpyAsync(best_idx, db, (size_t)n_sets * sizeof(int), hipMemcpyDeviceToHost, st);
  if (e == hipSuccess) e = hipStreamSynchronize(st);
  if (e != hipSuccess) { ctx->set_error("asd_distinctive_descriptor_batch: %s", hipGetErrorString(e)); return ASD_ERR_HIP; }
  if (any_big)
// ... 346 lines not shown
                           const uint8_t* occupied, const float* cur_Xw, float th, float nn_ratio, const uint8_t* mp_obs_positive, double* pose7,
                           int32_t* match_cur, int32_t* n_matches, uint8_t* outlier, int32_t* n_inliers) {
  if (n_mp > 0 && !desc) return ASD_ERR_INVALID;
  return run_track(ctx, [&](std::function<int()>* defer) {
    return track_local_points_impl(ctx, slot_cur, n_mp, Xw, normal, min_dist, max_dist, desc, nullptr, Tcw, K, viewing_cos_limit, occupied, cur_Xw, th,
                                   nn_ratio, mp_obs_positive, pose7, match_cur, n_matches, outlier, n_inliers, defer); });
}
int asd_track_local_points_bank(asd_ctx* ctx, int32_t slot_cur, int32_t n_mp, const float* Xw, const float* normal, const float* min_dist,
                                const float* max_dist, const int32_t* rows, const float* Tcw, const float* K, float viewing_cos_limit,
                                const uint8_t* occupied, const float* cur_Xw, float th, float nn_ratio, const uint8_t* mp_obs_positive,
                                double* pose7, int32_t* match_cur, int32_t* n_matches, uint8_t* outlier, int32_t* n_inliers) {
  if (n_mp > 0 && !rows) return ASD_ERR_INVALID;
  return run_track(ctx, [&](std::function<int()>* defer) {
    return track_local_points_impl(ctx, slot_cur, n_mp, Xw, normal, min_dist, max_dist, nullptr, rows, Tcw, K, viewing_cos_limit, occupied, cur_Xw, th,
                                   nn_ratio, mp_obs_positive, pose7, match_cur, n_matches, outlier, n_inliers, defer); });

}

int asd_track_local_points_rows(asd_ctx* ctx, int32_t slot_cur, int32_t n_mp, const int32_t* rows, const float* Tcw, const float* K, float viewing_cos_limit,
                                const uint8_t* occupied, const float* cur_Xw, float th, float nn_ratio, const uint8_t* mp_obs_positive,
                                double* pose7, int32_t* match_cur, int32_t* n_matches, uint8_t* outlier, int32_t* n_inliers) {
  return run_track(ctx, [&](std::function<int()>* defer) {
    return track_local_points_rows_impl(ctx, slot_cur, n_mp, rows, Tcw, K, viewing_cos_limit, occupied, cur_Xw, th, nn_ratio, mp_obs_positive, pose7, match_cur,
                                        n_matches, outlier, n_inliers, defer); });
}

int asd_track_local_points_map(asd_ctx* ctx, int32_t slot_cur, const float* Tcw, const float* K, float viewing_cos_limit, const uint8_t* occupied,
                               const float* cur_Xw, float th, float nn_ratio, const uint8_t* mp_obs_positive, double* pose7, int32_t* match_cur,
                               int32_t* n_matches, uint8_t* outlier, int32_t* n_inliers) {
  return run_track(ctx, [&](std::function<int()>* defer) {
    const int32_t *h_rows = nullptr, *d_rows = nullptr;
    int n_mp = 0;
    const int rc = localmap_search_list(ctx, "asd_track_local_points_map", &h_rows, &d_rows, &n_mp);
    if (rc != ASD_OK) return rc;
    return track_local_points_rows_impl(ctx, slot_cur, n_mp, h_rows, Tcw, K, viewing_cos_limit, occupied, cur_Xw, th, nn_ratio, mp_obs_positive, pose7, match_cur,
                                        n_matches, outlier, n_inliers, defer, d_rows); });
}


namespace {
int track_frame_impl(asd_ctx* ctx, const asd_track_frame_args& A, std::function<int()>* defer) {
  AsdFrameSlot *C = matcher_slot(ctx, A.slot_cur), *L = matcher_slot(ctx, A.slot_last);
  if (!C || !L || !A.has_mp || !A.Xw_last || !A.last_rows || !A.Tcw || !A.K || !A.cand_rows || A.n_cand < 1 || !A.pose7 || !A.pose1 || !A.match1 ||
      !A.n_matches1 || !A.outlier1 || !A.n_inliers1 || !A.match2 || !A.n_matches2 || !A.outlier2 || !A.n_inliers2)
    return ASD_ERR_INVALID;
  if (asd_track_busy(ctx, "asd_track_frame")) return ASD_ERR_INVALID;
  static const bool timing = getenv("ASD_TIMING") != nullptr;
  (void)hipSetDevice(ctx->cfg.device);
  MatcherState* m = matcher_state(ctx);
  const int nl = L->n, nc = C->n, ncand = A.n_cand;
  if (nl < 1 || nc < 1 || !replay_on_device(m, 0, nc, nl) || !replay_on_device(m, 1, nc, ncand) || !pose_chain_lds_form(ctx, nc)) {
    ctx->set_error("asd_track_frame: %d / %d keypoints, %d candidates are outside what the one-submission form handles (empty frame, more than "
                   "%d last-frame points or %d candidates, or tables beyond the workgroup's LDS): use asd_track_motion_model_bank + asd_track_local_points_bank", nc, nl, ncand,
                   kResolve2Threads * 4, kResolve2MaxRounds * 512);
    return ASD_ERR_CAPACITY;
  }
  int rc;
  if ((rc = matcher_check_bank_rows(ctx, m, A.last_rows, A.has_mp, nl, false)) != ASD_OK || (rc = matcher_check_bank_rows(ctx, m, A.cand_rows, nullptr, ncand, true)) != ASD_OK) return rc;
  if ((rc = ensure_cands_dev(ctx, m, (size_t)std::max(nl, ncand) * (size_t)nc)) != ASD_OK) return rc;
  hipStream_t st = ctx->stream;
  AsdXfer &up = ctx->up, &down = ctx->down;
  const size_t io_bytes = pose_chain_io_bytes(nc);
  ASD_HIP_CHECK(ctx, up.begin(st, (size_t)nl * sizeof(WinQuery) + (size_t)nl * (1 + 1 + 12 + 4 + 4) + (size_t)ncand * 5 + 16 * 256));
  ASD_HIP_CHECK(ctx, down.begin(st, 2 * (((size_t)nc + 16) * sizeof(int) + 256 + io_bytes + 256)));
  size_t need = 0;
  auto pad = [](size_t b) { return AsdDevBuf::padded(b); };
  need += pad((size_t)ncand * sizeof(WinQuery)) + 2 * pad((size_t)nl * 4) + 2 * pad((size_t)ncand * 4) + pad((size_t)nl * kTop * 2) + pad((size_t)ncand * kTop * 2) +
          pad(nc) + pad((size_t)nc * 12) + pad(ncand) + pad((size_t)ncand * 12) + pad(32 * 4) + pad(io_bytes);
  ASD_HIP_CHECK(ctx, ctx->scratch.reserve(need));
  if ((rc = pose_chain_reserve(ctx, nc)) != ASD_OK || (rc = resolve2_attributes(ctx)) != ASD_OK) return rc;
  TrackStage s1{}, s2{};
  s1.kind = 0; s1.nq = nl; s2.kind = 1; s2.nq = ncand;
  s1.F = s2.F = C;
  s1.d_qdesc = s2.d_qdesc = m->d_bank;
  WinQuery* d_q2 = ctx->scratch.carve<WinQuery>(ncand);
  s1.d_off = ctx->scratch.carve<int>(nl); s1.d_cnt = ctx->scratch.carve<int>(nl); s2.d_off = ctx->scratch.carve<int>(ncand); s2.d_cnt = ctx->scratch.carve<int>(ncand);
  s1.d_top = ctx->scratch.carve<uint16_t>((size_t)nl * kTop); s2.d_top = ctx->scratch.carve<uint16_t>((size_t)ncand * kTop);
  uint8_t* d_occ = ctx->scratch.carve<uint8_t>(nc);
  float* d_curXw = ctx->scratch.carve<float>((size_t)nc * 3);
  uint8_t* d_skip = ctx->scratch.carve<uint8_t>(ncand);
  float* d_cXw = ctx->scratch.carve<float>((size_t)ncand * 3);
  float* d_T1 = ctx->scratch.carve<float>(32);
  double* d_io1 = reinterpret_cast<double*>(ctx->scratch.carve<char>(io_bytes));
  const size_t o_q1 = up.reserve((size_t)nl * sizeof(WinQuery));
  s1.d_total = up.dev<int>(up.zeros(sizeof(int))); s2.d_total = up.dev<int>(up.zeros(sizeof(int)));
  if (A.last_obs_positive) s1.d_obs_pos = up.dev<uint8_t>(up.add(A.last_obs_positive, nl));
  if (A.cand_obs_positive) s2.d_obs_pos = up.dev<uint8_t>(up.add(A.cand_obs_positive, ncand));
  const size_t o_has = up.add(A.has_mp, nl), o_Xw = up.add(A.Xw_last, (size_t)nl * 12), o_rows1 = up.add(A.last_rows, (size_t)nl * 4);
  const size_t o_lc = A.last_cand ? up.add(A.last_cand, (size_t)nl * 4) : 0, o_crows = up.add(A.cand_rows, (size_t)ncand * 4);
  const size_t o_btw = up.reserve(sizeof(AsdBetweenArgs));
  const size_t o_out1 = down.reserve(((size_t)nc + 16) * sizeof(int)), o_res1 = down.reserve(io_bytes);
  const size_t o_out2 = down.reserve(((size_t)nc + 16) * sizeof(int)), o_res2 = down.reserve(io_bytes);
  s1.d_out = down.dev<int>(o_out1); s1.h_out = down.host<int>(o_out1);
  s2.d_out = down.dev<int>(o_out2); s2.h_out = down.host<int>(o_out2);
  {
    AsdBetweenArgs b{};
    b.n_cur = nc; b.n_last = nl; b.n_cand = ncand;
    b.match1 = s1.d_out; b.io1 = d_io1; b.Xw_last = up.dev<float>(o_Xw); b.last_cand = A.last_cand ? up.dev<int>(o_lc) : nullptr;
    memcpy(b.T_pred, A.Tcw, sizeof b.T_pred);
    b.occ = d_occ; b.cur_Xw = d_curXw; b.skip = d_skip; b.T1 = d_T1;
    memcpy(up.host<char>(o_btw), &b, sizeof b);
  }
  s1.source = kQueriesProject; s1.upload = kUploadCarried;
  s1.project = project_args(ctx, *C, *L, A.Tcw, A.K, A.th);
  s1.project.Xw = up.host<float>(o_Xw); s1.project.has_mp = up.host<uint8_t>(o_has); s1.project.rows = up.host<int>(o_rows1);
  s1.project.queries = up.dev<WinQuery>(o_q1);
  s1.project.up = upload_tail(up, nl, true);
  s1.d_queries = up.dev<WinQuery>(o_q1);
  s1.kp_last = L->d_kp; s1.check_ori = A.check_orientation;
  s1.has_solver = true;
  s1.solver.d_points = up.dev<float>(o_Xw);
  memcpy(s1.solver.pose0, A.pose7, sizeof s1.solver.pose0);
  for (int i = 0; i < 4; ++i) s1.solver.K[i] = s2.solver.K[i] = (double)A.K[i];
  s1.solver.io = down.host<double>(o_res1); s1.solver.d_io_dev = d_io1; s1.solver.d_between = up.dev<AsdBetweenArgs>(o_btw);
  s2.source = kQueriesFrustum; s2.upload = kUploadElsewhere;
  s2.frustum = frustum_args(ctx, *C, ncand, nullptr, d_T1, A.K, A.viewing_cos_limit, A.th_local);
  s2.frustum.rows = up.dev<int>(o_crows); s2.frustum.queries = d_q2;
  s2.frustum.up = upload_tail(up, ncand, false);
  s2.frustum.attr = m->d_attr; s2.frustum.skip = d_skip; s2.frustum.xw_out = d_cXw;
  s2.d_queries = d_q2;
  s2.d_occupied = d_occ; s2.nn_ratio = A.nn_ratio;
  s2.has_solver = true;
  s2.solver.d_points = d_cXw; s2.solver.d_hold = d_occ; s2.solver.d_own = d_curXw;
  s2.solver.d_pose0 = d_io1; s2.solver.io = down.host<double>(o_res2);
  const bool fuse = stage_fuses(ctx, m, s1) && stage_fuses(ctx, m, s2);
  if ((rc = enqueue_stage(ctx, m, s1, fuse)) != ASD_OK || (rc = enqueue_stage(ctx, m, s2, fuse)) != ASD_OK || (rc = record_chain_end(ctx)) != ASD_OK) return rc;

  asd_track_frame_args O = A;
  std::array<double, 7> p_in;
  memcpy(p_in.data(), A.pose7, 56);
  auto complete = [=]() -> int {
    ASD_HIP_CHECK(ctx, hipEventSynchronize(ctx->ev_chain));
    const int *h1 = ctx->down.host<int>(o_out1), *h2 = ctx->down.host<int>(o_out2);
    m->last_total[0] = h1[nc + 1]; m->last_total[1] = h2[nc + 1];
    if (h1[nc + 1] > m->cand_cap || h2[nc + 1] > m->cand_cap) {
      ctx->set_error("asd_track_frame: %d / %d candidates overflowed the %d-entry buffers", h1[nc + 1], h2[nc + 1], m->cand_cap);
      return ASD_ERR_CAPACITY;
    }
    auto unpack = [&](const int* h_out, const double* h_io, const double* p_start, int32_t* match, int32_t* n_matches, uint8_t* outlier, double* pose, int32_t* n_inl) {
      memcpy(match, h_out, (size_t)nc * sizeof(int));
      *n_matches = h_out[nc];
      unpack_solver_block(h_io, nc, true, match, nullptr, p_start, pose, outlier, n_inl);
    };
    unpack(h1, ctx->down.host<double>(o_res1), p_in.data(), O.match1, O.n_matches1, O.outlier1, O.pose1, O.n_inliers1);
    double p1[7];
    memcpy(p1, O.pose1, 56);
    unpack(h2, ctx->down.host<double>(o_res2), p1, O.match2, O.n_matches2, O.outlier2, O.pose7, O.n_inliers2);
    ctx->ms_match = 0.f;
    if (timing) {
      static double acc[2][5], tl[8]; static long calls;
      const int* hh[2] = {h1, h2};
      for (int k = 0; k < 2; ++k) { acc[k][0] += hh[k][nc + 2]; for (int i = 0; i < 4; ++i) acc[k][1 + i] += 0.01 * hh[k][nc + 3 + i]; }
      const double* io[2] = {ctx->down.host<double>(o_res1), ctx->down.host<double>(o_res2)};
      const int nw = (nc + 7) / 8;
      double st[8];
      for (int k = 0; k < 2; ++k) {
        st[4 * k] = hh[k][nc + 9]; st[4 * k + 1] = hh[k][nc + 10];
        st[4 * k + 2] = (double)((long long)io[k][8 + nw + 1] & 0x7fffffff); st[4 * k + 3] = (double)((long long)io[k][8 + nw + 2] & 0x7fffffff);
      }
      auto d = [](double a, double b) { double x = b - a; if (x < 0) x += 2147483648.0; return 0.01 * x; };
      tl[0] += d(st[0], st[1]); tl[1] += d(st[1], st[2]); tl[2] += d(st[2], st[3]); tl[3] += d(st[3], st[4]);
      tl[4] += d(st[4], st[5]); tl[5] += d(st[5], st[6]); tl[6] += d(st[6], st[7]); tl[7] += d(st[0], st[7]);
      if (++calls % 200 == 0) {
        for (int k = 0; k < 2; ++k)
          fprintf(stderr, "[track_frame resolve kind %d] %.1f iterations, %d candidates; staging %.1f us, iterations %.1f us (the first %.1f), outputs %.1f us; last frame: thread 0 work %.1f us, barrier + verdict %.1f us\n", k,
                  acc[k][0] / calls, hh[k][nc + 1], acc[k][1] / calls, acc[k][2] / calls, acc[k][4] / calls, acc[k][3] / calls, 0.01 * hh[k][nc + 7], 0.01 * hh[k][nc + 8]);
        fprintf(stderr, "[track_frame device clock] resolve1 %.1f | -> pose1 %.1f | pose1 %.1f | -> (frustum, search) resolve2 %.1f | resolve2 %.1f | -> pose2 %.1f | pose2 %.1f | resolve1 start -> pose2 end %.1f us\n",
                tl[0] / calls, tl[1] / calls, tl[2] / calls, tl[3] / calls, tl[4] / calls, tl[5] / calls, tl[6] / calls, tl[7] / calls);
      }
    }
    return ASD_OK;
  };
  if (defer) { *defer = complete; return ASD_OK; }
  return complete();
}
}

int asd_track_frame(asd_ctx* ctx, const asd_track_frame_args* args) {
  if (!args) return ASD_ERR_INVALID;
  return run_track(ctx, [&](std::function<int()>* defer) { return track_frame_impl(ctx, *args, defer); });
}

int asd_track_async(asd_ctx* ctx) {
  if (!ctx) return ASD_ERR_INVALID;
  if (asd_track_busy(ctx, "asd_track_async")) return ASD_ERR_INVALID;
  ctx->track_async_armed = true;
  return ASD_OK;
}

int asd_track_finish(asd_ctx* ctx) {
  if (!ctx) return ASD_ERR_INVALID;
// ... 234 lines not shown
```

### asd-slam_amd/csrc/resolve2.h

```cpp
#pragma once
#include <stdint.h>

#include <hip/hip_runtime.h>

#include "ctx.h"

namespace {
constexpr float TH_HIGH = 1.5f, TH_LOW = 0.5f;
constexpr int HISTO = ASD_HISTO_LENGTH;
constexpr int kTop = 4;

struct Resolve2Args {
  int nq, n_cur;
  const int* q_off; const int* q_cnt; const int* idx; const float* dist;
  const uint16_t* top_idx;
  const int* total; int cap;
  const uint8_t* obs_pos;
  const float4* kp_cur;
  const float4* kp_last;
  int check_ori;
  float nn_ratio;
  int* match_cur;
  int* n_matches;
  int* mirror;
  int stage_cap;
};
__host__ __device__ inline size_t resolve2_fixed_lds(int kind, int n_cur) {
  return (size_t)n_cur * 8 + (kind == 0 ? (size_t)n_cur * 4 : ((size_t)n_cur + 15) / 16 * 16);
}
constexpr int kResolve2Threads = 1024;
constexpr int kResolve2MaxRounds = 64;
template <int KIND, int QPT, int NT, class A>
__device__ __forceinline__ void resolve2_body(A& a) {
#pragma clang fp contract(off)
#define OUT(i, v) do { const int v_ = (v); a.match_cur[i] = v_; if (a.mirror) a.mirror[i] = v_; } while (0)
#define CNT(i, v) do { const int v_ = (v); a.n_matches[i] = v_; if (a.mirror) a.mirror[a.n_cur + (i)] = v_; } while (0)
  __builtin_amdgcn_s_setprio(3);
  extern __shared__ unsigned lds_c[];
  unsigned* claim0 = lds_c;
  float* ang = reinterpret_cast<float*>(claim0 + 2 * a.n_cur);
  uint8_t* octv = reinterpret_cast<uint8_t*>(claim0 + 2 * a.n_cur);
  char* tail = reinterpret_cast<char*>(lds_c) + resolve2_fixed_lds(KIND, a.n_cur);
  float* sdist = reinterpret_cast<float*>(tail);
  uint16_t* sidx = reinterpret_cast<uint16_t*>(tail + (KIND == 1 ? (size_t)a.stage_cap * 4 : 0));
  __shared__ int n_written, hist[HISTO], n_removed, flag[3];
  int* last = reinterpret_cast<int*>(tail + (size_t)a.stage_cap * (KIND == 1 ? 6 : 2));
  const int t = threadIdx.x;
  const unsigned long long ts0 = __builtin_amdgcn_s_memrealtime();
  const int total = *a.total;
  if (total > a.cap || total == 0) {
    for (int j = t; j < a.n_cur; j += NT) OUT(j, -1);
    if (t == 0) { CNT(0, 0); CNT(1, total); CNT(2, 0); }
    return;
  }
  int cnt[QPT], pick[QPT], qoff[QPT];
  constexpr int HD = KIND == 1 ? 2 : kTop;
  uint2 tj[QPT];
  float ang_last[KIND == 0 ? QPT : 1];
  unsigned posmask = 0;
  int qid[QPT];
  int ka = QPT;
  int n_act = a.nq;
  unsigned short* act_s = reinterpret_cast<unsigned short*>(last + a.n_cur);
  if constexpr (KIND == 1) {
    constexpr int NW = NT / 64;
    __shared__ int wbase[kResolve2MaxRounds * NW + 1];
    const int lane = t & 63, wave = t >> 6;
    const int rounds = (a.nq + NT - 1) / NT;
    for (int kb = 0; kb < rounds; ++kb) {
      const int q = t + kb * NT;
      const bool actv = q < a.nq && a.q_cnt[min(q, a.nq - 1)] > 0;
      const unsigned long long bal = __ballot(actv);
      if (lane == 0) wbase[kb * NW + wave] = __popcll(bal);
    }
    asd_syncthreads();
    if (t < 64) {
      int loc[NW];
      int sum = 0;
      for (int base = 0; base < rounds * NW; base += 64 * NW) {
        int mine_ = 0;
#pragma unroll
        for (int i = 0; i < NW; ++i) { const int e = base + t * NW + i; loc[i] = e < rounds * NW ? wbase[e] : 0; mine_ += loc[i]; }
        int inc = mine_;
        for (int off = 1; off < 64; off <<= 1) { const int v = __shfl_up(inc, off); if (t >= off) inc += v; }
        int run = sum + inc - mine_;
#pragma unroll
        for (int i = 0; i < NW; ++i) { const int e = base + t * NW + i; if (e < rounds * NW) wbase[e] = run; run += loc[i]; }
        sum += __shfl(inc, 63);
      }
      if (t == 0) wbase[rounds * NW] = sum;
    }
    asd_syncthreads();
    for (int kb = 0; kb < rounds; ++kb) {
      const int q = t + kb * NT;
      const bool actv = q < a.nq && a.q_cnt[min(q, a.nq - 1)] > 0;
      const unsigned long long bal = __ballot(actv);
      if (actv) act_s[wbase[kb * NW + wave] + __popcll(bal & ((1ull << lane) - 1))] = (unsigned short)q;
    }
    asd_syncthreads();
    n_act = wbase[rounds * NW];
  }
  auto load_chunk = [&](int c0) {
    posmask = 0;
    if constexpr (KIND == 1) {
      ka = __builtin_amdgcn_readfirstlane((min(n_act - c0, NT * QPT) + NT - 1) / NT);
#pragma unroll
      for (int k = 0; k < QPT; ++k) {
        const int slot = c0 + t + k * NT;
        const bool v = slot < n_act && k < ka;
        const int q = v ? (int)act_s[slot] : 0;
        qid[k] = q;
        cnt[k] = v ? a.q_cnt[q] : 0;
        qoff[k] = a.q_off[q];
        tj[k] = make_uint2(*reinterpret_cast<const unsigned*>(a.top_idx + (size_t)q * kTop), 0u);
        if (v && (!a.obs_pos || a.obs_pos[q])) posmask |= 1u << k;
        pick[k] = -1;
      }
    } else {
#pragma unroll
      for (int k = 0; k < QPT; ++k) {
        const int q = t + k * NT;
        const bool v = q < a.nq;
        const int qc = v ? q : 0;
        qid[k] = q;
        cnt[k] = v ? a.q_cnt[qc] : 0;
        qoff[k] = a.q_off[qc];
        tj[k] = *reinterpret_cast<const uint2*>(a.top_idx + (size_t)qc * kTop);
        ang_last[k] = a.check_ori ? a.kp_last[qc].w : 0.f;
        if (v && (!a.obs_pos || a.obs_pos[q])) posmask |= 1u << k;
        pick[k] = -1;
      }
    }
  };
  load_chunk(0);
  for (int j = t; j < 2 * a.n_cur; j += NT) claim0[j] = 0xffffffffu;
// ... 110 lines not shown
#pragma unroll
      for (int k = 0; k < QPT; ++k) {
        if (k >= ka) break;
        best[k] = p[k] >= 0 ? dist_at(k, i1[k]) : 0.f;
        best2[k] = p2[k] >= 0 ? dist_at(k, i2[k]) : 256.f;
        lvl[k] = p[k] >= 0 ? (int)octv[p[k]] : -1;
        lvl2[k] = p2[k] >= 0 ? (int)octv[p2[k]] : -1;
      }
#pragma unroll
      for (int k = 0; k < QPT; ++k) {
        if (k >= ka) break;
        const int q = qid[k];
        int pk = p[k];
        if (pk >= 0 && (!(best[k] <= TH_HIGH) || (lvl[k] == lvl2[k] && best2[k] < 256.f && best[k] > a.nn_ratio * best2[k]))) pk = -1;
        changed |= pk != pick[k];
        pick[k] = pk;
        if (pk >= 0 && (posmask >> k & 1)) atomicMin(&lds_c[wr + pk], (tag_wr << 16) | (unsigned)q);
      }
    }
    if (changed) flag[f_cur] = 1;
    const int f_next = f_cur == 2 ? 0 : f_cur + 1;
    if (t == 0) flag[f_next] = 0;
    const unsigned long long p1 = __builtin_amdgcn_s_memrealtime();
    asd_syncthreads();
    if (KIND == 1) load_claims(wr);
    const bool more = flag[f_cur] != 0 && it < it_limit;
    f_cur = f_next;
    { const unsigned long long p2 = __builtin_amdgcn_s_memrealtime(); ph_work += (int)(p1 - p0); ph_bar += (int)(p2 - p1); }
    if (it == 0) ts_it0 = __builtin_amdgcn_s_memrealtime();
    if (!more) break;
  }
#pragma unroll
  for (int k = 0; k < QPT; ++k) {
    bin[k] = -1;
    if (pick[k] < 0) continue;
    atomicMax(&last[pick[k]], qid[k]);
    ++mine;
    if (KIND == 0 && a.check_ori) {
      float rot = ang_last[k] - ang[pick[k]];
      if (rot < 0.0) rot += 360.0f;
      int b = (int)roundf(rot * (1.0f / HISTO));
      if (b == HISTO) b = 0;
      bin[k] = b;
      atomicAdd(&hist[b], 1);
    }
  }
  if (KIND == 0) break;
  c0 += NT * QPT;
  if (c0 >= n_act) break;
#pragma unroll
  for (int k = 0; k < QPT; ++k)
    if (pick[k] >= 0 && (posmask >> k & 1)) { lds_c[pick[k]] = (unsigned)qid[k]; lds_c[a.n_cur + pick[k]] = (unsigned)qid[k]; }
  it += 2;
  it_limit = it + min(n_act - c0, NT * QPT) + 2;
  load_chunk(c0);
  asd_syncthreads();
  load_claims((it & 1) ? a.n_cur : 0);
  }
  const unsigned long long ts2 = __builtin_amdgcn_s_memrealtime();
  if (mine) atomicAdd(&n_written, mine);
  asd_syncthreads();
  if (KIND == 0 && a.check_ori) {
    int hs[HISTO];
#pragma unroll
    for (int i = 0; i < HISTO; i++) hs[i] = hist[i];
    int max1 = 0, max2 = 0, max3 = 0, ind1 = -1, ind2 = -1, ind3 = -1;
#pragma unroll
    for (int i = 0; i < HISTO; i++) {
      const int s = hs[i];
      if (s > max1) { max3 = max2; max2 = max1; max1 = s; ind3 = ind2; ind2 = ind1; ind1 = i; }
      else if (s > max2) { max3 = max2; max2 = s; ind3 = ind2; ind2 = i; }
      else if (s > max3) { max3 = s; ind3 = i; }
    }
    if (max2 < 0.1f * (float)max1) { ind2 = -1; ind3 = -1; }
    else if (max3 < 0.1f * (float)max1) { ind3 = -1; }
    int removed = 0;
#pragma unroll
    for (int k = 0; k < QPT; ++k)
      if (bin[k] >= 0 && bin[k] != ind1 && bin[k] != ind2 && bin[k] != ind3) { last[pick[k]] = -1; ++removed; }
    if (removed) atomicAdd(&n_removed, removed);
    asd_syncthreads();
  }
  for (int j = t; j < a.n_cur; j += NT) OUT(j, last[j]);
  if (t == 0) { CNT(0, (KIND == 1 ? 2 : 1) * n_written - n_removed); CNT(1, total); CNT(2, it + 1);
    CNT(3, (int)(ts1 - ts0)); CNT(4, (int)(ts2 - ts1)); CNT(5, (int)(__builtin_amdgcn_s_memrealtime() - ts2)); CNT(6, (int)(ts_it0 - ts1));
    CNT(7, ph_work); CNT(8, ph_bar); CNT(9, (int)(ts0 & 0x7fffffffull)); CNT(10, (int)(__builtin_amdgcn_s_memrealtime() & 0x7fffffffull)); }
}
#undef OUT
#undef CNT
}
```

### asd-slam_amd/host/track_loop.cpp

```cpp
#include <algorithm>
#include <cmath>
#include <cstdint>
#include <cstdio>
#include <chrono>
#include <cstdlib>
#include <cstring>
#include <deque>
#include <vector>

#include "track_loop.h"

extern "C" {

struct asd_track_handle {
  asd_ctx* ctx;
  std::vector<const uint8_t*> d_frames;
  int W, H;
  float K32[4], T[16], scale32[8];
  double K64[4], pose0[7], inv_sigma2[8];
  asd_ba_problem ba;
  int kf_interval, lookahead;
  bool fused = true;
  bool async_ba = false;
  bool split = true;
  bool chain = false;
  int tables_for = -1;
  int map_copies = 2;
  const asd_do_mapping_inputs* dm = nullptr;
  std::vector<int32_t> dm_matches, dm_nmatch, dm_best, dm_distinct;
  std::vector<float> dm_x3d, dm_bdist;
  std::vector<uint8_t> dm_ok;
  double dm_ms = 0.0;
  long dm_calls = 0;
  asd_ctx* ctx_r = nullptr;
  std::vector<const uint8_t*> d_frames_r;
  float mb = 0.f, mbf = 0.f;
  std::vector<float> u_right, depth_r;
  std::vector<asd_keypoint> kps_r;
  std::vector<float> desc_sync_r;
  int32_t prep_stereo = -1;
  int frames_on_host = 0;
  int bank_base = 0;
  std::vector<int32_t> last_cand, cand_rows, sel_rows;
  asd_track_frame_args fa;
  int32_t f_n1 = 0, f_inl1 = 0, f_n2 = 0, f_inl2 = 0;
  double f_pose[7], f_pose1[7];
  float drift_cx = 620.5f, drift_cy = 188.0f, drift_z = 1.003f, drift_dx = 3.0f, drift_dy = 0.2f;
  int stop_after = -1;
  int prep_t = -1;
  const asd_keypoint* prep_kps = nullptr;
  int32_t prep_n = 0;
  int32_t c2_n2 = 0, c2_ninl = 0;
  double c2_pose[7];
  std::vector<uint8_t> outl2;
  bool ba_out = false;
  long ba_step = -1;
  asd_ba_problem ba_p;
  asd_ba_result ba_r;
  int slot = 0;
  std::deque<int> pending;
  bool have_last = false;
  std::vector<asd_keypoint> last_kps;
  int last_slot = 0;
  std::vector<asd_keypoint> kps;
  std::vector<float> desc_sync;
  std::vector<float> uv, Xw, Xw2, nrm, dist, maxd, mind, proj, vc;
  std::vector<uint8_t> has, in_view, occ, outl;
  std::vector<float> cur_Xw, Xs, ns, mind_s, maxd_s;
  std::vector<int32_t> sel;
  std::vector<uint8_t> keep, in_frame;
  std::vector<double> ba_obs;
  float T1[16];
  std::vector<int32_t> rows, m1, m2, level;
  std::vector<double> Xd, obs, info;
  std::vector<double> ba_poses, ba_points, ba_chi2;
  std::vector<uint8_t> ba_dpos, ba_out1;
  double wait_ms = 0.0, ba_ms = 0.0;
  double ba_prep_ms = 0.0;
  double seg_ms[8] = {};
  double kern_ms[4] = {};
  long steps = 0;
};

asd_track_handle* asd_track_create(asd_ctx* ctx, int32_t n_frames, const void* const* d_frames, int32_t W, int32_t H, const float* K32,
                                   const float* T, const double* pose0, const double* inv_sigma2, const float* scale32,
                                   const asd_ba_problem* ba, int32_t kf_interval, int32_t lookahead) {
  if (!ctx || n_frames < 1 || !d_frames || !K32 || !T || !pose0 || !inv_sigma2 || !scale32 || !ba || kf_interval < 1 || lookahead < 0 ||
      lookahead > ASD_EXTRACT_QUEUE)
    return nullptr;
  asd_track_handle* h = new asd_track_handle();
  h->ctx = ctx;
  for (int i = 0; i < n_frames; ++i) h->d_frames.push_back(static_cast<const uint8_t*>(d_frames[i]));
  h->W = W; h->H = H;
  for (int i = 0; i < 4; ++i) { h->K32[i] = K32[i]; h->K64[i] = (double)K32[i]; }
  memcpy(h->T, T, sizeof h->T);
  memcpy(h->pose0, pose0, sizeof h->pose0);
  memcpy(h->inv_sigma2, inv_sigma2, sizeof h->inv_sigma2);
  memcpy(h->scale32, scale32, sizeof h->scale32);
  h->ba = *ba;
  h->kf_interval = kf_interval; h->lookahead = lookahead;
  h->kps.resize(1 << 13);
  h->desc_sync.resize((size_t)(1 << 13) * 128);
  return h;
}

void asd_track_set_fused(asd_track_handle* h, int32_t on) { if (h) h->fused = on != 0; }
void asd_track_set_async_ba(asd_track_handle* h, int32_t on) { if (h) h->async_ba = on != 0; }
void asd_track_set_split(asd_track_handle* h, int32_t on) { if (h) h->split = on != 0; }
void asd_track_set_chain(asd_track_handle* h, int32_t on) { if (h) h->chain = on != 0; }
void asd_track_set_map_copies(asd_track_handle* h, int32_t copies) {
  if (!h || copies < 1 || copies > 16 || copies == h->map_copies) return;
  h->map_copies = copies;
  h->prep_t = -1;
  h->tables_for = -1;
}
int asd_track_drain(asd_track_handle* h) {
  if (!h) return ASD_ERR_INVALID;
  int rc = ASD_OK;
  while (!h->pending.empty()) {
    const asd_keypoint* k; const float* d; int32_t n;
    const int r = asd_extract_wait_view(h->ctx, &k, &d, &n);
    if (r != ASD_OK) rc = r;
    if (h->ctx_r) { const int r2 = asd_extract_wait_view(h->ctx_r, &k, &d, &n); if (r2 != ASD_OK) rc = r2; }
    h->pending.pop_front();
  }
  h->prep_t = -1;
  h->have_last = false;
  return rc;
}
void asd_track_set_frames_on_host(asd_track_handle* h, int32_t on) { if (h) h->frames_on_host = on != 0; }
int asd_track_set_stereo(asd_track_handle* h, asd_ctx* ctx_right, const void* const* d_frames_right, float mb, float mbf) {
  if (!h || !ctx_right || !d_frames_right || !(mb > 0) || !(mbf > 0) || !h->pending.empty()) return ASD_ERR_INVALID;
  int rc;
  if ((rc = asd_extract_keep_pyramid(h->ctx, 1)) != ASD_OK || (rc = asd_extract_keep_pyramid(ctx_right, 1)) != ASD_OK) return rc;
  h->ctx_r = ctx_right;
  h->d_frames_r.clear();
  for (size_t i = 0; i < h->d_frames.size(); ++i) h->d_frames_r.push_back(static_cast<const uint8_t*>(d_frames_right[i]));
  h->mb = mb; h->mbf = mbf;
  return ASD_OK;
}
void asd_track_set_do_mapping(asd_track_handle* h, const asd_do_mapping_inputs* in, int32_t n_cur) {
  if (!h) return;
  h->dm = in;
  if (!in) return;
  h->dm_matches.assign((size_t)in->n_nb * n_cur, -1); h->dm_nmatch.assign(std::max(in->n_nb, 1), 0);
  h->dm_x3d.assign((size_t)in->n_nb * n_cur * 3, 0.f); h->dm_ok.assign((size_t)in->n_nb * n_cur, 0);
  h->dm_best.assign(std::max(in->n_fuse_total, 1), -1); h->dm_bdist.assign(std::max(in->n_fuse_total, 1), 0.f);
  h->dm_distinct.assign(std::max(in->n_sets, 1), 0);
}
void asd_track_get_do_mapping_times(const asd_track_handle* h, double* ms, int64_t* calls) {
  if (!h) return;
  if (ms) *ms = h->dm_ms;
  if (calls) *calls = h->dm_calls;
}
void asd_track_get_times(const asd_track_handle* h, double* ba_ms, double* extract_wait_ms, int64_t* steps) {
  if (!h) return;
  if (ba_ms) *ba_ms = h->ba_ms;
  if (extract_wait_ms) *extract_wait_ms = h->wait_ms;
  if (steps) *steps = h->steps;
}
void asd_track_set_drift(asd_track_handle* h, float cx, float cy, float z, float dx, float dy) {
  if (h) { h->drift_cx = cx; h->drift_cy = cy; h->drift_z = z; h->drift_dx = dx; h->drift_dy = dy; }
}

static int collect_ba(asd_track_handle* h, asd_track_stats* st, long st_step) {
  if (!h->ba_out) return ASD_OK;
  const auto b0 = std::chrono::steady_clock::now();
  const int rc = asd_local_ba_wait(h->ctx);
  h->ba_ms += std::chrono::duration<double, std::milli>(std::chrono::steady_clock::now() - b0).count();
  h->ba_out = false;
  if (rc != ASD_OK) return rc;
  if (st && st_step == h->ba_step) { st->ba_chi2 = h->ba_r.chi2_second; st->has_ba = 1; }
  return ASD_OK;
}

void asd_track_destroy(asd_track_handle* h) {
  if (!h) return;
  while (!h->pending.empty()) {
    const asd_keypoint* k; const float* d; int32_t n;
    (void)asd_extract_wait_view(h->ctx, &k, &d, &n);
    if (h->ctx_r) (void)asd_extract_wait_view(h->ctx_r, &k, &d, &n);
    h->pending.pop_front();
  }
  (void)collect_ba(h, nullptr, -1);
  if (getenv("ASD_TIMING") && h->steps)
  {
    fprintf(stderr, "[track_loop] steps %ld  extract wait %.3f ms/step  local BA %.3f ms/step (+ %.3f ms/step putting its problem together on the host)\n", h->steps,
            h->wait_ms / h->steps, h->ba_ms / h->steps, h->ba_prep_ms / h->steps);
    static const char* nm[8] = {"frame_set", "submit", "bank+M1", "pose1", "frustum", "M2", "pose2", "host glue"};
    for (int i = 0; i < 8; ++i) fprintf(stderr, "[track_loop]   %-10s %.3f ms/step\n", nm[i], h->seg_ms[i] / h->steps);
    fprintf(stderr, "[track_loop]   device time: M1 %.3f pose1 %.3f M2 %.3f pose2 %.3f ms/step\n", h->kern_ms[0] / h->steps, h->kern_ms[1] / h->steps,
            h->kern_ms[2] / h->steps, h->kern_ms[3] / h->steps);
  }
  delete h;
}

static void build_candidate_tables(asd_track_handle* h, int nl) {
  const std::vector<asd_keypoint>& lk = h->last_kps;
  const int nc = h->map_copies * nl;
  h->Xw2.resize((size_t)3 * nc); h->nrm.resize((size_t)3 * nc); h->dist.resize(nc); h->maxd.resize(nc); h->mind.resize(nc);
  for (int c = 0; c < h->map_copies; ++c)
    for (int i = 0; i < nl; ++i)
      for (int k = 0; k < 3; ++k) h->Xw2[3 * ((size_t)c * nl + i) + k] = c == 0 ? h->Xw[3 * i + k] : h->Xw[3 * i + k] + (c == 1 ? 0.02f : 0.02f * (float)c);
  for (int i = 0; i < nc; ++i) {
    const float* P = &h->Xw2[3 * (size_t)i];
    const float nn = std::sqrt((P[0] * P[0] + P[1] * P[1]) + P[2] * P[2]);
    for (int k = 0; k < 3; ++k) h->nrm[3 * (size_t)i + k] = P[k] / nn;
    h->dist[i] = nn;
    const int lv = lk[i % nl].octave;
    h->maxd[i] = nn * h->scale32[lv];
    h->mind[i] = h->maxd[i] / h->scale32[7];
  }
}

static int prepare_frame(asd_track_handle* h, int t, const std::vector<int>& next) {
  asd_ctx* ctx = h->ctx;
  asd_ctx* ctxr = h->ctx_r;
  const int nf = (int)h->d_frames.size();
  int rc;
  auto tp = std::chrono::steady_clock::now();
  auto seg = [&](int i) {
    const auto now = std::chrono::steady_clock::now();
    h->seg_ms[i] += std::chrono::duration<double, std::milli>(now - tp).count();
    tp = now;
  };
  auto drop_pending = [&]() -> int {
    while (!h->pending.empty()) {
      const asd_keypoint* k; const float* d; int32_t nn;
      int r = asd_extract_wait_view(ctx, &k, &d, &nn);
      if (r == ASD_OK && ctxr) r = asd_extract_wait_view(ctxr, &k, &d, &nn);
      if (r != ASD_OK) return r;
      h->pending.pop_front();
    }
    return ASD_OK;
  };
  const asd_keypoint *kps = nullptr, *kps_r = nullptr;
  int32_t n = 0, n_r = 0;
  if (!h->pending.empty() && h->pending.front() == t) {
    const float* d = nullptr;
    const auto w0 = std::chrono::steady_clock::now();
    if ((rc = asd_extract_wait_view(ctx, &kps, &d, &n)) != ASD_OK) return rc;
    if (ctxr && (rc = asd_extract_wait_view(ctxr, &kps_r, &d, &n_r)) != ASD_OK) return rc;
    h->wait_ms += std::chrono::duration<double, std::milli>(std::chrono::steady_clock::now() - w0).count();
    h->pending.pop_front();
  } else {
    if ((rc = drop_pending()) != ASD_OK) return rc;
    if ((rc = (h->frames_on_host ? asd_extract : asd_extract_device)(ctx, h->d_frames[t % nf], h->W, h->H, h->W, 0, h->kps.data(), h->desc_sync.data(), &n)) != ASD_OK) return rc;
    kps = h->kps.data();
    if (ctxr) {
      h->kps_r.resize(1 << 13); h->desc_sync_r.resize((size_t)(1 << 13) * 128);
      if ((rc = asd_extract_device(ctxr, h->d_frames_r[t % nf], h->W, h->H, h->W, 0, h->kps_r.data(), h->desc_sync_r.data(), &n_r)) != ASD_OK) return rc;
      kps_r = h->kps_r.data();
    }
  }
  const bool chain = h->fused && h->split;
  if (chain) h->slot = (h->slot + 1) % 3; else h->slot ^= 1;
  seg(7);
  if ((rc = asd_frame_set(ctx, h->slot, kps, nullptr, n, 0.f, (float)h->W, 0.f, (float)h->H)) != ASD_OK) return rc;
  seg(0);
  if (ctxr) {
    const int slot_r = 3 + h->slot;
    if ((rc = asd_frame_set_from_ctx(ctx, slot_r, kps_r, n_r, 0.f, (float)h->W, 0.f, (float)h->H, ctxr)) != ASD_OK) return rc;
    h->u_right.resize(std::max(n, 1)); h->depth_r.resize(std::max(n, 1));
    int32_t nm = 0;
    if ((rc = asd_stereo_match(ctx, ctxr, h->slot, slot_r, h->mb, h->mbf, h->u_right.data(), h->depth_r.data(), &nm)) != ASD_OK) return rc;
    h->prep_stereo = nm;
    seg(4);
  }
  if (h->lookahead > 0) {
    bool same = h->pending.size() <= next.size();
    for (size_t i = 0; same && i < h->pending.size(); ++i) same = h->pending[i] == next[i];
    if (!same && (rc = drop_pending()) != ASD_OK) return rc;
    for (size_t i = h->pending.size(); i < next.size(); ++i) {
      if ((rc = asd_extract_submit(ctx, h->d_frames[next[i] % nf], h->frames_on_host ? 0 : 1, h->W, h->H, h->W, 0)) != ASD_OK) return rc;
      if (ctxr && (rc = asd_extract_submit(ctxr, h->d_frames_r[next[i] % nf], 1, h->W, h->H, h->W, 0)) != ASD_OK) return rc;
      h->pending.push_back(next[i]);
    }
  }
  seg(1);
  if (h->have_last) {
    const std::vector<asd_keypoint>& lk = h->last_kps;
    const int nl = (int)lk.size();
    const float fx = h->K32[0], fy = h->K32[1], cx = h->K32[2], cy = h->K32[3];
    const float z = h->drift_z, c3 = (float)((double)h->drift_dx * (double)(h->drift_z == 1.003f ? 1.003 : (double)h->drift_z)),
                c02 = (float)((double)(h->drift_dy == 0.2f ? 0.2 : (double)h->drift_dy) * (double)(h->drift_z == 1.003f ? 1.003 : (double)h->drift_z)), depth = 20.0f;
    h->Xw.resize((size_t)3 * nl);
    for (int i = 0; i < nl; ++i) {
      const float u = (lk[i].x - h->drift_cx) * z + h->drift_cx - c3;
      const float v = (lk[i].y - h->drift_cy) * z + h->drift_cy - c02;
      h->Xw[3 * i + 0] = (u - cx) / fx * depth;
      h->Xw[3 * i + 1] = (v - cy) / fy * depth;
      h->Xw[3 * i + 2] = depth;
    }
    const int n2p = h->map_copies * nl;
    build_candidate_tables(h, nl);
    seg(7);
    h->bank_base = h->bank_base ? 0 : 65536;
    const int base = h->bank_base;
    if (n2p > 65536) return ASD_ERR_CAPACITY;
    for (int c = 0; c < h->map_copies; ++c)
      if ((rc = asd_bank_put_from_frame(ctx, h->last_slot, base + c * nl, nl)) != ASD_OK) return rc;
    if ((rc = asd_mpbank_put(ctx, base, n2p, h->Xw2.data(), h->nrm.data(), h->mind.data(), h->maxd.data())) != ASD_OK) return rc;
    h->rows.resize(nl); h->last_cand.resize(nl); h->cand_rows.resize(n2p);
    for (int i = 0; i < nl; ++i) { h->rows[i] = base + i; h->last_cand[i] = i; }
    for (int i = 0; i < n2p; ++i) h->cand_rows[i] = base + i;
    h->tables_for = t;
    seg(2);
  }
  h->prep_t = t; h->prep_kps = kps; h->prep_n = n;
  return ASD_OK;
}

static int submit_ba(asd_track_handle* h, asd_track_stats* st, int t);

static int select_local_points(asd_track_handle* h, int n, int nl, const uint8_t* outl1, const double* pose1, bool gather = true) {
  h->keep.assign(n, 0); h->occ.assign(n, 0);
  h->in_frame.assign((size_t)h->map_copies * nl, 0);
  h->cur_Xw.assign((size_t)3 * n, 0.f);
  int nmatch = 0;
  for (int j = 0; j < n; ++j) {
    const int i = h->m1[j];
    nmatch += i >= 0;
    const int src = i >= 0 ? i : 0;
    for (int k = 0; k < 3; ++k) h->cur_Xw[3 * j + k] = h->Xw[3 * src + k];
    if (i >= 0 && !outl1[j]) { h->keep[j] = 1; h->occ[j] = 1; }
    if (i >= 0) h->in_frame[i] = 1;
// ... 113 lines not shown
  auto tp = std::chrono::steady_clock::now();
  auto seg = [&](int i) {
    const auto now = std::chrono::steady_clock::now();
    h->seg_ms[i] += std::chrono::duration<double, std::milli>(now - tp).count();
    tp = now;
  };
  if (h->prep_t != t && (rc = prepare_frame(h, t, next)) != ASD_OK) return rc;
  tp = std::chrono::steady_clock::now();
  const asd_keypoint* kps = h->prep_kps;
  const int32_t n = h->prep_n;
  const int cur = h->slot;
  h->prep_t = -1;
  memset(st, 0, sizeof *st);
  st->n_kp = n;
  if (h->ctx_r) { st->stereo_matched = h->prep_stereo; st->has_stereo = 1; }
  const bool had_last = h->have_last;
  if (had_last) {
    h->m1.assign(n, -1); h->m2.assign(n, -1);
    h->outl.assign(n, 0); h->outl2.assign(n, 0);
    memcpy(h->f_pose, h->pose0, sizeof h->f_pose);
    asd_track_frame_args& a = h->fa;
    memset(&a, 0, sizeof a);
    a.slot_cur = cur; a.slot_last = h->last_slot;
    a.has_mp = h->has.data(); a.Xw_last = h->Xw.data(); a.last_rows = h->rows.data(); a.last_cand = h->last_cand.data();
    a.Tcw = h->T; a.th = 15.0f; a.check_orientation = 1;
    a.n_cand = (int32_t)h->cand_rows.size(); a.cand_rows = h->cand_rows.data();
    a.viewing_cos_limit = 0.5f; a.th_local = 1.0f; a.nn_ratio = 0.8f; a.K = h->K32;
    a.pose7 = h->f_pose; a.pose1 = h->f_pose1;
    a.match1 = h->m1.data(); a.n_matches1 = &h->f_n1; a.outlier1 = h->outl.data(); a.n_inliers1 = &h->f_inl1;
    a.match2 = h->m2.data(); a.n_matches2 = &h->f_n2; a.outlier2 = h->outl2.data(); a.n_inliers2 = &h->f_inl2;
    if ((rc = asd_track_async(ctx)) != ASD_OK) return rc;
    if ((rc = asd_track_frame(ctx, &a)) != ASD_OK) return rc;
    seg(2);
  }
  h->last_kps.assign(kps, kps + n);
  h->last_slot = cur;
  h->have_last = true;
  if (do_ba && h->async_ba && (rc = submit_ba(h, st, t)) != ASD_OK) return rc;
  seg(7);
  if (!next.empty() && next[0] == t + 1) {
    std::vector<int> after(next.begin() + 1, next.end());
    after.push_back(next.back() + 1);
    if ((int)after.size() > h->lookahead) after.resize(h->lookahead);
    if (h->stop_after >= 0) while (!after.empty() && after.back() > h->stop_after) after.pop_back();
    if ((rc = asd_prep_async(ctx, 1)) != ASD_OK) { if (had_last) (void)asd_track_finish(ctx); return rc; }
    rc = prepare_frame(h, t + 1, after);
    const int rc2 = asd_prep_async(ctx, 0);
    if (rc != ASD_OK || rc2 != ASD_OK) { if (had_last) (void)asd_track_finish(ctx); return rc != ASD_OK ? rc : rc2; }
    tp = std::chrono::steady_clock::now();
  }
  if (had_last) {
    if ((rc = asd_track_finish(ctx)) != ASD_OK) return rc;
    st->m1 = h->f_n1; st->has_m1 = 1;
    st->m2 = h->f_n2; st->has_m2 = 1;
    int nedge = 0;
    for (int j = 0; j < n; ++j) nedge += (h->m1[j] >= 0 && !h->outl[j]) || h->m2[j] >= 0;
    if (nedge >= 3) { st->inliers = h->f_inl2; st->has_inliers = 1; } else std::fill(h->outl2.begin(), h->outl2.end(), (uint8_t)0);
    h->keep.resize(n);
    for (int j = 0; j < n; ++j) h->keep[j] = h->m1[j] >= 0 && !h->outl[j];
    seg(6);
  }
  final_matches_to_has(h, n, had_last, h->keep.data(), h->m2.data(), h->outl2.data());
  if (do_ba && !h->async_ba && (rc = submit_ba(h, st, t)) != ASD_OK) return rc;
  ++h->steps;
  return ASD_OK;
}

static int track_step(asd_track_handle* h, int t, bool do_ba, const std::vector<int>& next, asd_track_stats* st) {
  asd_ctx* ctx = h->ctx;
  const int nf = (int)h->d_frames.size();
  int rc;
  auto tp = std::chrono::steady_clock::now();
  auto seg = [&](int i) {
    const auto now = std::chrono::steady_clock::now();
    h->seg_ms[i] += std::chrono::duration<double, std::milli>(now - tp).count();
    tp = now;
  };
  const asd_keypoint* kps = nullptr;
  int32_t n = 0;
  if (!h->pending.empty() && h->pending.front() == t) {
    const float* d = nullptr;
    const auto w0 = std::chrono::steady_clock::now();
    if ((rc = asd_extract_wait_view(ctx, &kps, &d, &n)) != ASD_OK) return rc;
    h->wait_ms += std::chrono::duration<double, std::milli>(std::chrono::steady_clock::now() - w0).count();
    h->pending.pop_front();
  } else {
    while (!h->pending.empty()) {
      const asd_keypoint* k; const float* d; int32_t nn;
      if ((rc = asd_extract_wait_view(ctx, &k, &d, &nn)) != ASD_OK) return rc;
      h->pending.pop_front();
    }
    if ((rc = (h->frames_on_host ? asd_extract : asd_extract_device)(ctx, h->d_frames[t % nf], h->W, h->H, h->W, 0, h->kps.data(), h->desc_sync.data(), &n)) != ASD_OK) return rc;
    kps = h->kps.data();
  }
  h->slot ^= 1;
  const int cur = h->slot;
  seg(7);
  if ((rc = asd_frame_set(ctx, cur, kps, nullptr, n, 0.f, (float)h->W, 0.f, (float)h->H)) != ASD_OK) return rc;
  seg(0);
  if (h->lookahead > 0) {
    bool same = h->pending.size() <= next.size();
    for (size_t i = 0; same && i < h->pending.size(); ++i) same = h->pending[i] == next[i];
    if (!same) {
      while (!h->pending.empty()) {
        const asd_keypoint* k; const float* d; int32_t nn;
        if ((rc = asd_extract_wait_view(ctx, &k, &d, &nn)) != ASD_OK) return rc;
        h->pending.pop_front();
      }
    }
    for (size_t i = h->pending.size(); i < next.size(); ++i) {
      if ((rc = asd_extract_submit(ctx, h->d_frames[next[i] % nf], h->frames_on_host ? 0 : 1, h->W, h->H, h->W, 0)) != ASD_OK) return rc;
      h->pending.push_back(next[i]);
    }
  }
  seg(1);
  memset(st, 0, sizeof *st);
  st->n_kp = n;
  if (h->have_last) {
    const std::vector<asd_keypoint>& lk = h->last_kps;
    const int nl = (int)lk.size();
    const float fx = h->K32[0], fy = h->K32[1], cx = h->K32[2], cy = h->K32[3];
    const float z = h->drift_z, c3 = (float)((double)h->drift_dx * (double)(h->drift_z == 1.003f ? 1.003 : (double)h->drift_z)),
                c02 = (float)((double)(h->drift_dy == 0.2f ? 0.2 : (double)h->drift_dy) * (double)(h->drift_z == 1.003f ? 1.003 : (double)h->drift_z)), depth = 20.0f;
    h->Xw.resize((size_t)3 * nl);
    for (int i = 0; i < nl; ++i) {
      const float u = (lk[i].x - h->drift_cx) * z + h->drift_cx - c3;
      const float v = (lk[i].y - h->drift_cy) * z + h->drift_cy - c02;
      h->Xw[3 * i + 0] = (u - cx) / fx * depth;
      h->Xw[3 * i + 1] = (v - cy) / fy * depth;
      h->Xw[3 * i + 2] = depth;
    }
    if ((int)h->has.size() != nl) h->has.assign(nl, 1);
    seg(7);
    for (int c = 0; c < h->map_copies; ++c)
      if ((rc = asd_bank_put_from_frame(ctx, h->last_slot, c * nl, nl)) != ASD_OK) return rc;
    h->rows.resize((size_t)h->map_copies * nl);
    for (int i = 0; i < h->map_copies * nl; ++i) h->rows[i] = i;
    h->m1.assign(n, -1);
    int32_t n1 = 0;
    auto dev = [&](int i, const char* stage) { float ms = 0.f; if (asd_last_stage_ms(ctx, stage, &ms) == ASD_OK) h->kern_ms[i] += ms; };
    auto pose_opt = [&](const std::vector<int>& sel, auto point_of, double* pose_io, uint8_t* outl_k, int32_t* ninl) -> int {
      const int m = (int)sel.size();
      h->Xd.resize((size_t)3 * m); h->obs.resize((size_t)2 * m); h->info.resize(m); h->outl.resize(m);
      for (int q = 0; q < m; ++q) {
        const int j = sel[q];
        const float* P = point_of(j);
        for (int k = 0; k < 3; ++k) h->Xd[3 * q + k] = (double)P[k];
        h->obs[2 * q] = (double)kps[j].x; h->obs[2 * q + 1] = (double)kps[j].y;
        h->info[q] = h->inv_sigma2[kps[j].octave];
      }
      const int r = asd_pose_optimize(ctx, pose_io, m, h->Xd.data(), h->obs.data(), h->info.data(), h->K64, h->outl.data(), ninl);
      if (r == ASD_OK && outl_k) for (int q = 0; q < m; ++q) outl_k[sel[q]] = h->outl[q];
      return r;
    };
    build_candidate_tables(h, nl);
    std::vector<int> sel;
    std::vector<uint8_t> outl1(n, 0);
    double pose1[7];
    memcpy(pose1, h->pose0, sizeof pose1);
    seg(7);
    if (h->fused) {
      int32_t ninl = 0;
      if ((rc = asd_track_motion_model_bank(ctx, cur, h->last_slot, h->has.data(), h->Xw.data(), h->rows.data(), h->T, h->K32, 15.0f, 1, nullptr,
                                            pose1, h->m1.data(), &n1, outl1.data(), &ninl)) != ASD_OK)
        return rc;
      st->m1 = n1; st->has_m1 = 1;
      seg(2);
// ... 35 lines not shown
                                            h->K32, 0.5f, h->occ.data(), h->cur_Xw.data(), 1.0f, 0.8f, nullptr, pose, h->m2.data(), &n2,
                                            h->outl.data(), &ninl)) != ASD_OK)
        return rc;
      st->m2 = n2; st->has_m2 = 1;
      dev(2, "match");
      seg(5);
      for (int j = 0; j < n; ++j) nedge += h->keep[j] || h->m2[j] >= 0;
      if (nedge >= 3) { st->inliers = ninl; st->has_inliers = 1; h->outl2.assign(h->outl.begin(), h->outl.begin() + n); } else h->outl2.assign(n, 0);
      seg(6);
    } else {
      if ((rc = asd_match_project_points_bank(ctx, cur, nsel, h->in_view.data(), h->proj.data(), h->level.data(), h->vc.data(), h->sel.data(),
                                              h->occ.data(), 1.0f, 0.8f, h->m2.data(), &n2, nullptr)) != ASD_OK)
        return rc;
      st->m2 = n2; st->has_m2 = 1;
      dev(2, "match");
      seg(5);
      sel.clear();
      for (int j = 0; j < n; ++j) if (h->keep[j] || h->m2[j] >= 0) sel.push_back(j);
      h->outl2.assign(n, 0);
      if (sel.size() >= 3) {
        int32_t ninl = 0;
        double pose[7];
        memcpy(pose, pose1, sizeof pose);
        if ((rc = pose_opt(sel, [&](int j) { return h->keep[j] ? &h->Xw[3 * h->m1[j]] : &h->Xw2[3 * h->sel[std::max(h->m2[j], 0)]]; }, pose, h->outl2.data(), &ninl)) != ASD_OK)
          return rc;
        st->inliers = ninl; st->has_inliers = 1;
      }
      dev(3, "ba");
      seg(6);
    }
  }
  final_matches_to_has(h, n, h->have_last, h->keep.data(), h->m2.data(), h->outl2.data());
  if (do_ba && (rc = submit_ba(h, st, t)) != ASD_OK) return rc;
  seg(7);
  h->last_kps.assign(kps, kps + n);
  h->last_slot = cur;
  h->have_last = true;
  ++h->steps;
  return ASD_OK;
}


static int do_mapping_stage(asd_track_handle* h) {
  const asd_do_mapping_inputs& D = *h->dm;
  asd_ctx* ctx = h->ctx;
  const auto t0 = std::chrono::steady_clock::now();
  int rc;
  if (D.n_nb > 0 && (rc = asd_create_map_points_batch(ctx, D.slot_cur, D.has_mp_cur, D.Tcw_cur, D.K_cur, D.n_nb, D.nb, h->dm_matches.data(), h->dm_nmatch.data(),
                                                      h->dm_x3d.data(), h->dm_ok.data())) != ASD_OK)
    return rc;
  if (D.n_fuse_calls > 0 && (rc = asd_fuse_search_batch(ctx, D.n_fuse_calls, D.fuse_calls, D.n_fuse_total, D.valid, D.Xw, D.normal, D.min_dist, D.max_dist, nullptr,
                                                        D.desc_rows, D.th, h->dm_best.data(), h->dm_bdist.data())) != ASD_OK)
    return rc;
  if (D.n_sets > 0 && (rc = asd_distinctive_descriptor_batch(ctx, D.n_sets, D.set_start, D.set_desc, h->dm_distinct.data())) != ASD_OK) return rc;
  h->dm_ms += std::chrono::duration<double, std::milli>(std::chrono::steady_clock::now() - t0).count();
  ++h->dm_calls;
  return ASD_OK;
}

static int submit_ba(asd_track_handle* h, asd_track_stats* st, int t) {
  asd_ctx* ctx = h->ctx;
  int rc;
  if ((rc = collect_ba(h, nullptr, -1)) != ASD_OK) return rc;
  const auto p0 = std::chrono::steady_clock::now();
  const asd_ba_problem& B = h->ba;
  h->ba_poses.assign(B.poses, B.poses + (size_t)7 * B.n_poses);
  h->ba_points.assign(B.points, B.points + (size_t)3 * B.n_points);
  h->ba_chi2.assign(B.n_edges, 0.0); h->ba_dpos.assign(B.n_edges, 0); h->ba_out1.assign(B.n_edges, 0);
  h->ba_obs.resize((size_t)2 * B.n_edges);
  const uint32_t kf = (uint32_t)(t / h->kf_interval);
  for (uint32_t i = 0; i < (uint32_t)(2 * B.n_edges); ++i) {
    uint32_t x = i * 2654435761u + kf * 40503u + 12345u;
    x ^= x >> 15;
    x *= 2246822519u;
    x ^= x >> 13;
    const double u = (double)((x >> 8) & 0xFFFFu);
    h->ba_obs[i] = B.e_obs[i] + (u / 65536.0 - 0.5) * 0.2;
  }
  h->ba_p = B;
  h->ba_p.poses = h->ba_poses.data(); h->ba_p.points = h->ba_points.data(); h->ba_p.e_obs = h->ba_obs.data();
  memset(&h->ba_r, 0, sizeof h->ba_r);
  h->ba_r.edge_chi2 = h->ba_chi2.data(); h->ba_r.edge_depth_pos = h->ba_dpos.data(); h->ba_r.edge_outlier1 = h->ba_out1.data();
  h->ba_prep_ms += std::chrono::duration<double, std::milli>(std::chrono::steady_clock::now() - p0).count();
  struct ExtractHold {
    asd_ctx *a, *b;
    ExtractHold(asd_ctx* a_, asd_ctx* b_, bool on) : a(on ? a_ : nullptr), b(on ? b_ : nullptr) { if (a) (void)asd_extract_hold(a, 1); if (b) (void)asd_extract_hold(b, 1); }
    ~ExtractHold() { if (a) (void)asd_extract_hold(a, 0); if (b) (void)asd_extract_hold(b, 0); }
  } hold(ctx, h->ctx_r, !h->async_ba);
  if (h->dm && !h->async_ba && (rc = do_mapping_stage(h)) != ASD_OK) return rc;
  const auto b0 = std::chrono::steady_clock::now();
  if (h->async_ba) {
    if ((rc = asd_local_ba_submit(ctx, &h->ba_p, &h->ba_r)) != ASD_OK) return rc;
    h->ba_out = true;
    h->ba_step = h->steps;
  } else {
    rc = asd_local_ba(ctx, &h->ba_p, &h->ba_r);
    if (rc != ASD_OK) return rc;
    st->ba_chi2 = h->ba_r.chi2_second; st->has_ba = 1;
  }
  h->ba_ms += std::chrono::duration<double, std::milli>(std::chrono::steady_clock::now() - b0).count();
  return ASD_OK;
}

int asd_track_run(asd_track_handle* h, int32_t t0, int32_t n, int32_t prefetch_beyond, asd_track_stats* stats) {
  if (!h || n < 0 || !stats) return ASD_ERR_INVALID;
  std::vector<int> next;
  for (int i = 0; i < n; ++i) {
    const int t = t0 + i;
    next.clear();
    for (int k = 1; k <= h->lookahead; ++k)
      if (i + k < n || prefetch_beyond) next.push_back(t + k);
    h->stop_after = prefetch_beyond ? -1 : t0 + n - 1;
    const bool split = h->fused && h->split;
    if (!split && h->prep_t >= 0) { h->prep_t = -1; }
    const bool ba_now = t % h->kf_interval == h->kf_interval - 1;
    const int rc = split ? (h->chain ? track_step_chain(h, t, ba_now, next, stats) : track_step_split(h, t, ba_now, next, stats))
                         : track_step(h, t, ba_now, next, stats);
    if (rc != ASD_OK) return rc;
  }
  return collect_ba(h, stats, h->steps - 1);
}

}
```

### asd-slam_amd/host/track_loop.h

```cpp
#pragma once
#include <stdint.h>

#include "../../include/asd_slam.h"

#ifdef __cplusplus
extern "C" {
#endif

typedef struct asd_track_stats {
  int32_t n_kp, m1, m2, inliers;
  double ba_chi2;
  int32_t has_m1, has_m2, has_inliers, has_ba;
  int32_t stereo_matched, has_stereo;
} asd_track_stats;

typedef struct asd_track_handle asd_track_handle;

asd_track_handle* asd_track_create(asd_ctx* ctx, int32_t n_frames, const void* const* d_frames, int32_t W, int32_t H, const float* K32,
                                   const float* T, const double* pose0, const double* inv_sigma2, const float* scale32,
                                   const asd_ba_problem* ba, int32_t kf_interval, int32_t lookahead);
void asd_track_destroy(asd_track_handle* h);
void asd_track_set_fused(asd_track_handle* h, int32_t on);
void asd_track_set_async_ba(asd_track_handle* h, int32_t on);
void asd_track_set_split(asd_track_handle* h, int32_t on);
void asd_track_set_chain(asd_track_handle* h, int32_t on);
void asd_track_set_map_copies(asd_track_handle* h, int32_t copies);
void asd_track_set_frames_on_host(asd_track_handle* h, int32_t on);
int asd_track_set_stereo(asd_track_handle* h, asd_ctx* ctx_right, const void* const* d_frames_right, float mb, float mbf);
int asd_track_drain(asd_track_handle* h);
void asd_track_get_times(const asd_track_handle* h, double* ba_ms, double* extract_wait_ms, int64_t* steps);
void asd_track_set_drift(asd_track_handle* h, float cx, float cy, float z, float dx, float dy);
typedef struct asd_do_mapping_inputs {
  int32_t slot_cur; const uint8_t* has_mp_cur; const float* Tcw_cur; const float* K_cur;
  int32_t n_nb; const asd_kf_neighbor* nb;
  int32_t n_fuse_calls; const asd_fuse_call* fuse_calls;
  int32_t n_fuse_total; const uint8_t* valid; const float* Xw; const float* normal; const float* min_dist; const float* max_dist;
  const int32_t* desc_rows; float th;
  int32_t n_sets; const int32_t* set_start; const float* set_desc;
} asd_do_mapping_inputs;
void asd_track_set_do_mapping(asd_track_handle* h, const asd_do_mapping_inputs* in, int32_t n_cur );
void asd_track_get_do_mapping_times(const asd_track_handle* h, double* ms, int64_t* calls);
int asd_track_run(asd_track_handle* h, int32_t t0, int32_t n, int32_t prefetch_beyond, asd_track_stats* stats);

#ifdef __cplusplus
}
#endif
```

### include/asd_slam.h

```cpp
#ifndef ASD_SLAM_H
#define ASD_SLAM_H

#include <stdint.h>

#ifdef __cplusplus
extern "C" {
#endif

#define ASD_DESC_DIM 128
#define ASD_PATCH 32
#define ASD_MAX_LEVELS 16
#define ASD_GRID_COLS 64
#define ASD_GRID_ROWS 48
#define ASD_HISTO_LENGTH 30

typedef enum asd_status {
  ASD_OK = 0,
  ASD_ERR_INVALID = -1,
  ASD_ERR_NO_DEVICE = -2,
  ASD_ERR_HIP = -3,
  ASD_ERR_NO_WEIGHTS = -4,
  ASD_ERR_CAPACITY = -5,
  ASD_ERR_NUMERIC = -6,
  ASD_ERR_RANGE = -7
// ... 505 lines not shown
                         int32_t capacity, int32_t* scored_kf, float* scored_score, int32_t* n_scored);
int asd_kfdb_select(asd_ctx* ctx, int32_t mode, int32_t n_scored, const int32_t* neigh, int32_t capacity, int32_t* cand,
                    int32_t* n_cand);
int32_t asd_debug_kfdb(asd_ctx* ctx, int64_t out[5]);
int32_t asd_debug_kfdb_entry(asd_ctx* ctx, int32_t kf, int32_t out[4], float score[2]);
int asd_map_put(asd_ctx* ctx, int32_t kf, int32_t n, const int32_t* rows);
int asd_map_set(asd_ctx* ctx, int32_t kf, int32_t count, const int32_t* idx, const int32_t* rows);
int asd_map_erase(asd_ctx* ctx, int32_t kf);
int asd_map_clear(asd_ctx* ctx);
int asd_map_kf_links(asd_ctx* ctx, int32_t kf, int32_t n_cov, const int32_t* cov, int32_t n_children, const int32_t* children,
                     int32_t parent);
int asd_map_kf_bad(asd_ctx* ctx, int32_t kf, int32_t flag);
int asd_map_point_bad(asd_ctx* ctx, int32_t n, const int32_t* rows, int32_t flag);

typedef struct asd_local_map_args {
  int32_t n_cur;  const int32_t* cur_rows;
  int32_t n_seen; const int32_t* seen_rows;
  int32_t n_prev; const int32_t* prev_kfs;
  int32_t max_kfs;
  int32_t kf_capacity;     int32_t* local_kfs;   int32_t n_local_kfs; int32_t ref_kf;
  int32_t row_capacity;    int32_t* local_rows;  int32_t n_local;
  int32_t search_capacity; int32_t* search_rows; int32_t n_search;
} asd_local_map_args;
int asd_update_local_map(asd_ctx* ctx, asd_local_map_args* args);

int asd_track_local_points_map(asd_ctx* ctx, int32_t slot_cur, const float* Tcw, const float* K, float viewing_cos_limit,
                               const uint8_t* occupied, const float* cur_Xw, float th, float nn_ratio, const uint8_t* mp_obs_positive,
                               double* pose7, int32_t* match_cur, int32_t* n_matches, uint8_t* outlier, int32_t* n_inliers);

int asd_map_shared_counts(asd_ctx* ctx, int32_t kf, int32_t capacity, int32_t* kfs, int32_t* counts, int32_t* n);

int asd_map_put_octaves(asd_ctx* ctx, int32_t kf, int32_t n, const uint8_t* octave);

typedef struct asd_kf_culling_args {
  int32_t n_cand; const int32_t* cand;
  const uint8_t* cand_flags;
  int32_t apply;
  uint8_t* decision;
  int32_t* n_mps; int32_t* n_redundant;
  int32_t bad_capacity; int32_t* bad_rows; int32_t n_bad;
} asd_kf_culling_args;
int asd_keyframe_culling(asd_ctx* ctx, asd_kf_culling_args* args);

int asd_map_observations(asd_ctx* ctx, int32_t n, const int32_t* rows, int32_t* counts);

int asd_map_kf_centers(asd_ctx* ctx, int32_t n, const int32_t* kfs, const float* Ow );

typedef struct asd_normal_depth_args {
  int32_t n; const int32_t* rows;
  const int32_t* ref_kf;
  const float* Xw;
  float* normal; float* min_dist; float* max_dist;
  uint8_t* status;
} asd_normal_depth_args;
int asd_update_normal_and_depth(asd_ctx* ctx, asd_normal_depth_args* args);

int asd_normal_and_depth_point(int32_t n_obs, const float* Ow , int32_t ref ,
                               const float* Pos, float scale_level, float scale_top, float normal[3], float* min_dist, float* max_dist);

typedef struct asd_ba_graph_args {
  int32_t kf; int32_t n_neigh; const int32_t* neigh;
  int32_t kf_capacity;    int32_t* local_kfs;  int32_t n_local_kfs;
  int32_t point_capacity; int32_t* local_rows; int32_t* point_rank; int32_t n_points;
  int32_t fixed_capacity; int32_t* fixed_kfs;  int32_t n_fixed;
  int32_t pose_capacity;  int32_t* pose_kfs;   uint8_t* pose_fixed; int32_t n_poses;
  int32_t edge_capacity;  int32_t* e_point; int32_t* e_pose; int32_t* e_kf; int32_t* e_idx; uint8_t* e_octave; int32_t n_edges;
  double* Xw;
} asd_ba_graph_args;
int asd_local_ba_graph(asd_ctx* ctx, asd_ba_graph_args* args);

typedef struct asd_ba_apply_args {
  int32_t n_edges; const uint8_t* erase;
  int32_t apply;
  int32_t n_erased;
  int32_t bad_capacity; int32_t* bad_rows; int32_t n_bad;
  int32_t n_points; int32_t* new_ref;
} asd_ba_apply_args;
int asd_local_ba_apply(asd_ctx* ctx, asd_ba_apply_args* args);

int32_t asd_debug_map(asd_ctx* ctx, int64_t out[8]);

int32_t asd_debug_bank_get(asd_ctx* ctx, int32_t first_row, int32_t n, float* desc, float* attr);

int asd_describe_timed(asd_ctx* ctx, const uint8_t* d_patches, int32_t n, float* d_desc,
                       int32_t reps, float* avg_ms);

#ifdef __cplusplus
}
#endif
#endif
```

Measured before the change: 1305.

## Fuse query generation into window search and restructure distance computation

Removes the separate frustum/project query kernels by computing each query inside the window-search kernel through a templated query-args type, with upload-tail blocks folded into the same launch. The candidate distance computation now has 4-lane groups each load a full 128-float row as float4 and reduce with shuffles, prefetching the query and first chunk before the block barrier. The total counter becomes a persistent buffer that the resolve kernel resets, so per-call zero uploads go away. It also adds an env-controlled option to skip holding extraction during BA, plus a debug API for reading the window lists. Computing queries redundantly per lane and adding register pressure are the main risks.

New measurement: 1299, median of 2. About the same (-0.5%).

```diff
diff --git a/asd-slam_amd/capi.py b/asd-slam_amd/capi.py
--- a/asd-slam_amd/capi.py
+++ b/asd-slam_amd/capi.py
@@ -1080,6 +1080,18 @@
         self.lib.asd_debug_bank_get.restype = C.c_int32
         self._chk(self.lib.asd_debug_bank_get(self.ctx, C.c_int32(first_row), C.c_int32(n), _p(d), _p(a)))
         return d, a
+
+    def window_lists(self):
+        f = self.lib.asd_debug_window_lists
+        f.restype = C.c_int32
+        nq, srt, total = C.c_int32(), C.c_int32(), C.c_int64()
+        null = C.c_void_p()
+        self._chk(f(self.ctx, C.byref(nq), C.byref(srt), C.c_int32(0), null, null, null, C.c_int32(0), null, null, C.byref(total)))
+        n, m = nq.value, int(total.value)
+        cnt, off, top = np.empty(n, np.int32), np.empty(n, np.int32), np.empty((n, 4), np.uint16)
+        idx, bits = np.empty(m, np.int32), np.empty(m, np.uint32)
+        self._chk(f(self.ctx, C.byref(nq), C.byref(srt), C.c_int32(n), _p(cnt), _p(off), _p(top), C.c_int32(m), _p(idx), _p(bits), C.byref(total)))
+        return dict(sorted=bool(srt.value), q_cnt=cnt, q_off=off, top_idx=top, idx=idx, dist_bits=bits)
 
     def match_project_frame_bank(self, slot_cur, slot_last, n_cur, has_mp, Xw, mp_rows, Tcw, K, th, check_ori=True, obs_positive=None):
         has_mp, Xw, mp_rows = _c(has_mp, np.uint8), _c(Xw, np.float32), _c(mp_rows, np.int32)
diff --git a/asd-slam_amd/csrc/ctx.h b/asd-slam_amd/csrc/ctx.h
--- a/asd-slam_amd/csrc/ctx.h
+++ b/asd-slam_amd/csrc/ctx.h
@@ -74,12 +74,12 @@
 };
 #if defined(__HIPCC__)
 template <class F>
-__device__ inline void asd_frustum_bank_point(const F& a, const float* T_dev, const uint8_t* skip, const int q) {
+__device__ inline AsdWinQuery asd_frustum_bank_point(const F& a, const float* T_dev, const uint8_t* skip, const int q, const bool store) {
 #pragma clang fp contract(off)
   AsdWinQuery Q{0.f, 0.f, 0.f, 0, 0, -1};
   const int row = a.rows[q];
   const float4 A0 = reinterpret_cast<const float4*>(a.attr)[2 * (size_t)row], A1 = reinterpret_cast<const float4*>(a.attr)[2 * (size_t)row + 1];
-  a.xw_out[3 * (size_t)q] = A0.x; a.xw_out[3 * (size_t)q + 1] = A0.y; a.xw_out[3 * (size_t)q + 2] = A0.z;
+  if (store) { a.xw_out[3 * (size_t)q] = A0.x; a.xw_out[3 * (size_t)q + 1] = A0.y; a.xw_out[3 * (size_t)q + 2] = A0.z; }
   if (!skip || !skip[q]) {
     float T[16], Ow[3];
     for (int i = 0; i < 16; ++i) T[i] = T_dev[i];
@@ -112,7 +112,7 @@
       Q = AsdWinQuery{u, v, r * a.scale[lvl], lvl - 1, lvl, row};
     }
   }
-  a.queries[q] = Q;
+  return Q;
 }
 __device__ inline void asd_between_body(const AsdBetweenArgs& a_dev, const int t, const int nt) {
 #pragma clang fp contract(off)
diff --git a/asd-slam_amd/csrc/matcher.h b/asd-slam_amd/csrc/matcher.h
--- a/asd-slam_amd/csrc/matcher.h
+++ b/asd-slam_amd/csrc/matcher.h
@@ -6,11 +6,15 @@
 
 using WinQuery = AsdWinQuery;
 
+struct LastLists { int nq = 0; bool sorted = false; const int* d_off = nullptr; const int* d_cnt = nullptr; const uint16_t* d_top = nullptr; };
+
 struct MatcherState {
   int q_cap = 0, cand_cap = 0, h_cand_cap = 0, qdesc_cap = 0;
   int last_total[4] = {1 << 15, 1 << 15, 1 << 15, 1 << 15};
   WinQuery *d_queries = nullptr, *h_queries = nullptr;
-  int *d_q_off = nullptr, *d_q_cnt = nullptr, *d_total = nullptr, *d_idx = nullptr;
+  int *d_q_off = nullptr, *d_q_cnt = nullptr, *d_idx = nullptr;
+  int* d_total = nullptr;
+  LastLists last_lists;
   float* d_dist = nullptr;
   int *h_q = nullptr;
   int* h_idx = nullptr;
@@ -37,6 +41,7 @@
 AsdFrameSlot* matcher_slot(asd_ctx* ctx, int s);
 int matcher_ensure_queries(asd_ctx* ctx, MatcherState* m, int nq);
 int matcher_ensure_qdesc(asd_ctx* ctx, MatcherState* m, int n);
+int matcher_total(asd_ctx* ctx, MatcherState* m);
 int matcher_upload_qdesc(asd_ctx* ctx, MatcherState* m, const float* desc, int n);
 int matcher_window_search(asd_ctx* ctx, MatcherState* m, const AsdFrameSlot& F, int nq, const float* d_q, SearchResult* res, int kind = 3);
 int matcher_list_search(asd_ctx* ctx, MatcherState* m, const AsdFrameSlot& A, const AsdFrameSlot& B, const asd_feature_vector* fvA,
diff --git a/asd-slam_amd/csrc/matcher.hip b/asd-slam_amd/csrc/matcher.hip
--- a/asd-slam_amd/csrc/matcher.hip
+++ b/asd-slam_amd/csrc/matcher.hip
@@ -5,6 +5,7 @@
 #include <array>
 #include <functional>
 #include <memory>
+#include <type_traits>
 
 #include "matcher.h"
 #include "resolve2.h"
@@ -20,10 +21,114 @@
   float min_x, min_y, inv_w, inv_h;
 };
 
+struct UploadTail {
+  const uint4* src; uint4* dst;
+  size_t first16, n16;
+  int q_blocks;
+};
+__device__ inline bool upload_tail_block(const UploadTail& u) {
+  if ((int)blockIdx.x < u.q_blocks) return false;
+  const size_t nb = gridDim.x - u.q_blocks, nt = blockDim.x;
+  for (size_t i = u.first16 + (size_t)(blockIdx.x - u.q_blocks) * nt + threadIdx.x; i < u.n16; i += nb * nt) u.dst[i] = u.src[i];
+  return true;
+}
+constexpr int kUploadTailBlocks = 32;
+
+struct TableQueries {};
+struct FrustumArgs {
+  int n, n_levels, bfactor;
+  const float* Xw; const float* normal; const float* min_dist; const float* max_dist;
+  const int* rows;
+  float T[16], Ow[3];
+  float fx, fy, cx, cy, min_x, max_x, min_y, max_y, cos_limit, th;
+  float level_thr[ASD_MAX_LEVELS], scale[ASD_MAX_LEVELS];
+  WinQuery* queries;
+  UploadTail up;
+  const float* T_dev; const float* attr; const uint8_t* skip; float* xw_out;
+};
+struct ProjectArgs {
+  int n;
+  const uint8_t* has_mp; const float* Xw; const int* rows; const float4* kp_last;
+  float T[16];
+  float fx, fy, cx, cy, min_x, max_x, min_y, max_y, th;
+  float scale[ASD_MAX_LEVELS];
+  UploadTail up;
+};
+__device__ inline bool query_tail_block(const TableQueries&) { return false; }
+__device__ inline bool query_tail_block(const ProjectArgs& a) { return upload_tail_block(a.up); }
+__device__ inline bool query_tail_block(const FrustumArgs& a) { return upload_tail_block(a.up); }
+
+__device__ inline WinQuery make_query(const TableQueries&, const WinQuery* __restrict__ queries, const int q, const bool) { return queries[q]; }
+__device__ inline WinQuery make_query(const FrustumArgs& a, const WinQuery*, const int q, const bool store) {
+  WinQuery Q{0.f, 0.f, 0.f, 0, 0, -1};
+  if (a.attr) {
+    if (a.T_dev) {
+      Q = asd_frustum_bank_point(a, a.T_dev, a.skip, q, store);
+      if (store) a.queries[q] = Q;
+      return Q;
+    }
+    float Tl[19];
+    for (int i = 0; i < 16; ++i) Tl[i] = a.T[i];
+    for (int i = 0; i < 3; ++i) Tl[16 + i] = a.Ow[i];
+    return asd_frustum_bank_point(a, Tl, a.skip, q, store);
+  }
+  const float* P = a.Xw + 3 * (size_t)q;
+  float Pc[3];
+  for (int r = 0; r < 3; ++r) {
+    const float t0 = a.T[r * 4 + 0] * P[0] + a.T[r * 4 + 1] * P[1] + a.T[r * 4 + 2] * P[2];
+    Pc[r] = (float)((double)t0 + (double)a.T[r * 4 + 3]);
+  }
+  bool ok = !(Pc[2] < 0.0f);
+  const float invz = 1.0f / Pc[2];
+  const float u = a.fx * Pc[0] * invz + a.cx, v = a.fy * Pc[1] * invz + a.cy;
+  if (u < a.min_x || u > a.max_x || v < a.min_y || v > a.max_y) ok = false;
+  const float maxD = 1.2f * a.max_dist[q], minD = 0.8f * a.min_dist[q];
+  const float PO[3] = {P[0] - a.Ow[0], P[1] - a.Ow[1], P[2] - a.Ow[2]};
+  const double nn = (double)PO[0] * PO[0] + (double)PO[1] * PO[1] + (double)PO[2] * PO[2];
+  const float dist = (float)sqrt(nn);
+  if (dist < minD || dist > maxD) ok = false;
+  const float* Pn = a.normal + 3 * (size_t)q;
+  const double dot = (double)PO[0] * Pn[0] + (double)PO[1] * Pn[1] + (double)PO[2] * Pn[2];
+  const float vc = (float)(dot / dist);
+  if (vc < a.cos_limit) ok = false;
+  if (ok) {
+    const float ratio = a.max_dist[q] / dist;
+    int lvl = 0;
+    for (int k = 1; k < a.n_levels; ++k) lvl += ratio >= a.level_thr[k];
+    float r = vc > 0.998 ? 2.5f : 4.0f;
+    if (a.bfactor) r *= a.th;
+    Q = WinQuery{u, v, r * a.scale[lvl], lvl - 1, lvl, a.rows ? a.rows[q] : q};
+  }
+  return Q;
+}
+__device__ inline WinQuery make_query(const ProjectArgs& a, const WinQuery*, const int i, const bool) {
+  WinQuery Q{0.f, 0.f, 0.f, 0, 0, -1};
+  const bool has = a.has_mp[i] != 0;
+  const float X[3] = {a.Xw[3 * (size_t)i], a.Xw[3 * (size_t)i + 1], a.Xw[3 * (size_t)i + 2]};
+  const int oct = __float_as_int(a.kp_last[i].z), row = a.rows ? a.rows[i] : i;
+  if (has) {
+    float Xc[3];
+    for (int r = 0; r < 3; ++r) {
+      const float t0 = a.T[r * 4 + 0] * X[0] + a.T[r * 4 + 1] * X[1] + a.T[r * 4 + 2] * X[2];
+      Xc[r] = (float)((double)t0 + (double)a.T[r * 4 + 3]);
+    }
+    const float invzc = (float)(1.0 / (double)Xc[2]);
+    if (!(invzc < 0)) {
+      const float u = a.fx * Xc[0] * invzc + a.cx;
+      const float v = a.fy * Xc[1] * invzc + a.cy;
+      if (!(u < a.min_x || u > a.max_x) && !(v < a.min_y || v > a.max_y)) {
+        Q = WinQuery{u, v, a.th * a.scale[oct], oct - 1, oct + 1, row};
+      }
+    }
+  }
+  return Q;
+}
+
 #ifndef ASD_SEARCH_WAVES
 #define ASD_SEARCH_WAVES 8
 #endif
 constexpr int kSearchWaves = ASD_SEARCH_WAVES;
+inline int search_blocks(int nq) { return (nq + kSearchWaves - 1) / kSearchWaves; }
 constexpr int kSearchCols = 16;
 constexpr int kSearchList = 128;
 struct SortArgs {
@@ -31,19 +136,22 @@
   float th_cut;
   uint16_t* top_idx;
 };
-template <bool SORT>
+constexpr int kDistLanes = 4;
+constexpr int kDistChunk = 64 / kDistLanes;
+template <bool SORT, class QA>
 __global__ __launch_bounds__(64 * kSearchWaves) void k_window_search(GridDev G, const WinQuery* __restrict__ queries, int nq,
                                                        const float* __restrict__ qdesc, const float* __restrict__ cdesc,
                                                        int* __restrict__ q_off, int* __restrict__ q_cnt,
                                                        int* __restrict__ total, int cap, int* __restrict__ out_idx,
-                                                       float* __restrict__ out_dist, SortArgs S) {
+                                                       float* __restrict__ out_dist, SortArgs S, QA qa) {
+  if (query_tail_block(qa)) return;
   const int lane = threadIdx.x & 63, wave = threadIdx.x >> 6;
   const int q = blockIdx.x * kSearchWaves + wave;
   __shared__ int wg_cnt[kSearchWaves], wg_base;
   __shared__ int cand_l[kSearchWaves][kSearchList];
   __shared__ unsigned dist_l[SORT ? kSearchWaves : 1][kSearchList];
   const bool live = q < nq;
-  const WinQuery Q = live ? queries[q] : WinQuery{0.f, 0.f, 0.f, 0, 0, -1};
+  const WinQuery Q = live ? make_query(qa, queries, q, lane == 0) : WinQuery{0.f, 0.f, 0.f, 0, 0, -1};
   int cnt = 0, off = 0;
   bool empty = Q.qrow < 0;
   const int nMinCellX = max(0, (int)floorf((Q.x - G.min_x - Q.r) * G.inv_w));
@@ -153,6 +261,27 @@
   } else if (!empty) {
     cnt = walk(0);
   }
+  const int sub = lane & (kDistLanes - 1), grp = lane / kDistLanes;
+  const int n_fast = SORT && fast ? cnt : 0;
+  float4 qv[8], ya[8];
+  auto load_rows = [&](int base, float4 (&y)[8]) {
+    if (base + grp < n_fast) {
+      const float4* b = reinterpret_cast<const float4*>(cdesc + (size_t)cand_l[wave][base + grp] * 128) + 8 * sub;
+#pragma unroll
+      for (int k = 0; k < 8; ++k) y[k] = b[k];
+    } else {
+#pragma unroll
+      for (int k = 0; k < 8; ++k) y[k] = make_float4(0.f, 0.f, 0.f, 0.f);
+    }
+  };
+  if (n_fast > 0) {
+    asm volatile("s_waitcnt lgkmcnt(0)" ::: "memory");
+    __builtin_amdgcn_wave_barrier();
+    const float4* a = reinterpret_cast<const float4*>(qdesc + (size_t)Q.qrow * 128) + 8 * sub;
+#pragma unroll
+    for (int k = 0; k < 8; ++k) qv[k] = a[k];
+    load_rows(0, ya);
+  }
   if (lane == 0) wg_cnt[wave] = cnt;
   asd_syncthreads();
   if (threadIdx.x == 0) {
@@ -187,12 +316,35 @@
     if (fast) {
       const bool v0 = lane < cnt, v1 = lane + 64 < cnt;
       const int i0 = v0 ? cand_l[wave][lane] : 0, i1 = v1 ? cand_l[wave][lane + 64] : 0;
-      const float d0 = v0 ? distance(i0) : 0.f, d1 = v1 ? distance(i1) : 0.f;
-      const unsigned b0 = __float_as_uint(d0), b1 = __float_as_uint(d1);
-      if (v0) dist_l[wave][lane] = b0;
-      if (v1) dist_l[wave][lane + 64] = b1;
+      auto finish_rows = [&](int base, float4 (&y)[8]) {
+#pragma unroll
+        for (int k = 0; k < 8; ++k) {
+          float d;
+          d = qv[k].x - y[k].x; y[k].x = d * d;
+          d = qv[k].y - y[k].y; y[k].y = d * d;
+          d = qv[k].z - y[k].z; y[k].z = d * d;
+          d = qv[k].w - y[k].w; y[k].w = d * d;
+        }
+        float sqd = 0.f;
+#pragma unroll
+        for (int j = 0; j < kDistLanes; ++j) {
+          const float prev = __shfl_up(sqd, 1, kDistLanes);
+          if (sub == j) {
+            sqd = j ? prev : 0.f;
+#pragma unroll
+            for (int k = 0; k < 8; ++k) { sqd = sqd + y[k].x; sqd = sqd + y[k].y; sqd = sqd + y[k].z; sqd = sqd + y[k].w; }
+          }
+        }
+        if (sub == kDistLanes - 1 && base + grp < cnt) dist_l[wave][base + grp] = __float_as_uint(sqd);
+      };
+      for (int base = 0; base < cnt; base += kDistChunk) {
+        if (base) load_rows(base, ya);
+        finish_rows(base, ya);
+      }
       asm volatile("s_waitcnt lgkmcnt(0)" ::: "memory");
       __builtin_amdgcn_wave_barrier();
+      const unsigned b0 = v0 ? dist_l[wave][lane] : 0u, b1 = v1 ? dist_l[wave][lane + 64] : 0u;
+      const float d0 = __uint_as_float(b0), d1 = __uint_as_float(b1);
       int r0 = 0, r1 = 0;
       for (int i = 0; i < cnt; ++i) {
         const unsigned di = dist_l[wave][i];
@@ -370,109 +522,6 @@
   resolve2_body<KIND, QPT, kResolve2Threads>(a);
 }
 
-struct UploadTail {
-  const uint4* src; uint4* dst;
-  size_t first16, n16;
-  int q_blocks;
-};
-__device__ inline bool upload_tail_block(const UploadTail& u) {
-  if ((int)blockIdx.x < u.q_blocks) return false;
-  const size_t nb = gridDim.x - u.q_blocks;
-  for (size_t i = u.first16 + (size_t)(blockIdx.x - u.q_blocks) * 256 + threadIdx.x; i < u.n16; i += nb * 256) u.dst[i] = u.src[i];
-  return true;
-}
-constexpr int kUploadTailBlocks = 64;
-
-struct FrustumArgs {
-  int n, n_levels, bfactor;
-  const float* Xw; const float* normal; const float* min_dist; const float* max_dist;
-  const int* rows;
-  float T[16], Ow[3];
-  float fx, fy, cx, cy, min_x, max_x, min_y, max_y, cos_limit, th;
-  float level_thr[ASD_MAX_LEVELS], scale[ASD_MAX_LEVELS];
-  WinQuery* queries;
-  UploadTail up;
-  const float* T_dev; const float* attr; const uint8_t* skip; float* xw_out;
-};
-__global__ __launch_bounds__(256) void k_frustum_queries(FrustumArgs a) {
-  if (upload_tail_block(a.up)) return;
-  const int q = blockIdx.x * 256 + threadIdx.x;
-  if (q >= a.n) return;
-  WinQuery Q{0.f, 0.f, 0.f, 0, 0, -1};
-  if (a.attr) {
-    if (a.T_dev) asd_frustum_bank_point(a, a.T_dev, a.skip, q);
-    else {
-      float Tl[19];
-      for (int i = 0; i < 16; ++i) Tl[i] = a.T[i];
-      for (int i = 0; i < 3; ++i) Tl[16 + i] = a.Ow[i];
-      asd_frustum_bank_point(a, Tl, a.skip, q);
-    }
-    return;
-  }
-  const float* P = a.Xw + 3 * (size_t)q;
-  float Pc[3];
-  for (int r = 0; r < 3; ++r) {
-    const float t0 = a.T[r * 4 + 0] * P[0] + a.T[r * 4 + 1] * P[1] + a.T[r * 4 + 2] * P[2];
-    Pc[r] = (float)((double)t0 + (double)a.T[r * 4 + 3]);
-  }
-  bool ok = !(Pc[2] < 0.0f);
-  const float invz = 1.0f / Pc[2];
-  const float u = a.fx * Pc[0] * invz + a.cx, v = a.fy * Pc[1] * invz + a.cy;
-  if (u < a.min_x || u > a.max_x || v < a.min_y || v > a.max_y) ok = false;
-  const float maxD = 1.2f * a.max_dist[q], minD = 0.8f * a.min_dist[q];
-  const float PO[3] = {P[0] - a.Ow[0], P[1] - a.Ow[1], P[2] - a.Ow[2]};
-  const double nn = (double)PO[0] * PO[0] + (double)PO[1] * PO[1] + (double)PO[2] * PO[2];
-  const float dist = (float)sqrt(nn);
-  if (dist < minD || dist > maxD) ok = false;
-  const float* Pn = a.normal + 3 * (size_t)q;
-  const double dot = (double)PO[0] * Pn[0] + (double)PO[1] * Pn[1] + (double)PO[2] * Pn[2];
-  const float vc = (float)(dot / dist);
-  if (vc < a.cos_limit) ok = false;
-  if (ok) {
-    const float ratio = a.max_dist[q] / dist;
-    int lvl = 0;
-    for (int k = 1; k < a.n_levels; ++k) lvl += ratio >= a.level_thr[k];
-    float r = vc > 0.998 ? 2.5f : 4.0f;
-    if (a.bfactor) r *= a.th;
-    Q = WinQuery{u, v, r * a.scale[lvl], lvl - 1, lvl, a.rows ? a.rows[q] : q};
-  }
-  a.queries[q] = Q;
-}
-
-struct ProjectArgs {
-  int n;
-  const uint8_t* has_mp; const float* Xw; const int* rows; const float4* kp_last;
-  float T[16];
-  float fx, fy, cx, cy, min_x, max_x, min_y, max_y, th;
-  float scale[ASD_MAX_LEVELS];
-  WinQuery* queries;
-  UploadTail up;
-};
-__global__ __launch_bounds__(256) void k_project_queries(ProjectArgs a) {
-  if (upload_tail_block(a.up)) return;
-  const int i = blockIdx.x * 256 + threadIdx.x;
-  if (i >= a.n) return;
-  WinQuery Q{0.f, 0.f, 0.f, 0, 0, -1};
-  if (a.has_mp[i]) {
-    const float* X = a.Xw + 3 * (size_t)i;
-    float Xc[3];
-    for (int r = 0; r < 3; ++r) {
-      const float t0 = a.T[r * 4 + 0] * X[0] + a.T[r * 4 + 1] * X[1] + a.T[r * 4 + 2] * X[2];
-      Xc[r] = (float)((double)t0 + (double)a.T[r * 4 + 3]);
-    }
-    const float invzc = (float)(1.0 / (double)Xc[2]);
-    if (!(invzc < 0)) {
-      const float u = a.fx * Xc[0] * invzc + a.cx;
-      const float v = a.fy * Xc[1] * invzc + a.cy;
-      if (!(u < a.min_x || u > a.max_x) && !(v < a.min_y || v > a.max_y)) {
-        const int oct = __float_as_int(a.kp_last[i].z);
-        Q = WinQuery{u, v, a.th * a.scale[oct], oct - 1, oct + 1, a.rows ? a.rows[i] : i};
-      }
-    }
-  }
-  a.queries[i] = Q;
-}
-
 int ensure_cands_dev(asd_ctx* ctx, MatcherState* m, size_t n) {
   if (n <= (size_t)m->cand_cap) return ASD_OK;
   if (n > ((size_t)1 << 30)) { ctx->set_error("candidate buffers: %zu entries asked for", n); return ASD_ERR_CAPACITY; }
@@ -518,6 +567,12 @@
   ASD_HIP_CHECK(ctx, hipMalloc(&m->d_q_off, ((size_t)2 * cap + 4) * sizeof(int)));
   ASD_HIP_CHECK(ctx, hipHostMalloc(&m->h_q, ((size_t)2 * cap + 4) * sizeof(int)));
   m->q_cap = cap;
+  return ASD_OK;
+}
+int matcher_total(asd_ctx* ctx, MatcherState* m) {
+  if (m->d_total) return ASD_OK;
+  ASD_HIP_CHECK(ctx, hipMalloc(&m->d_total, 4 * sizeof(int)));
+  ASD_HIP_CHECK(ctx, hipMemset(m->d_total, 0, 4 * sizeof(int)));
   return ASD_OK;
 }
 int matcher_ensure_qdesc(asd_ctx* ctx, MatcherState* m, int n) {
@@ -562,8 +617,9 @@
     ASD_HIP_CHECK(ctx, hipMemsetAsync(d_total, 0, sizeof(int), st));
     GridDev G{F.d_kp, F.d_cell_start, F.d_cell_items, F.min_x, F.min_y, F.inv_w, F.inv_h};
     ASD_HIP_CHECK(ctx, hipEventRecord(ctx->ev0, st));
-    hipLaunchKernelGGL(k_window_search<false>, dim3((nq + kSearchWaves - 1) / kSearchWaves), dim3(64 * kSearchWaves), 0, st, G, m->d_queries, nq, d_q, F.d_desc, d_off, d_cnt,
-                       d_total, m->cand_cap, m->d_idx, m->d_dist, SortArgs{});
+    hipLaunchKernelGGL((k_window_search<false, TableQueries>), dim3(search_blocks(nq)), dim3(64 * kSearchWaves), 0, st, G, m->d_queries, nq, d_q, F.d_desc, d_off, d_cnt,
+                       d_total, m->cand_cap, m->d_idx, m->d_dist, SortArgs{}, TableQueries{});
+    m->last_lists = LastLists{nq, false, d_off, d_cnt, nullptr};
     ASD_HIP_CHECK(ctx, hipGetLastError());
     ASD_HIP_CHECK(ctx, hipEventRecord(ctx->ev1, st));
     ASD_HIP_CHECK(ctx, hipMemcpyAsync(m->h_q, d_off, ((size_t)2 * nq + 1) * sizeof(int), hipMemcpyDeviceToHost, st));
@@ -646,8 +702,7 @@
 };
 
 UploadTail upload_tail(const AsdXfer& up, int nq, bool carried) {
-  return UploadTail{reinterpret_cast<const uint4*>(up.h), reinterpret_cast<uint4*>(up.d), carried ? ((size_t)nq * sizeof(WinQuery) + 255) / 256 * 16 : 0,
-                    carried ? (up.used + 15) / 16 : 0, (nq + 255) / 256};
+  return UploadTail{reinterpret_cast<const uint4*>(up.h), reinterpret_cast<uint4*>(up.d), 0, carried ? (up.used + 15) / 16 : 0, search_blocks(nq)};
 }
 
 ProjectArgs project_args(const asd_ctx* ctx, const AsdFrameSlot& C, const AsdFrameSlot& L, const float* Tcw, const float* K, float th) {
@@ -709,26 +764,24 @@
   return s.has_solver && pose_chain_fused_ok(ctx, s.kind, s.nq, s.F->n, resolve2_args(m, s, &a));
 }
 
-int enqueue_stage(asd_ctx* ctx, const MatcherState* m, const TrackStage& s, bool fuse) {
+int enqueue_stage(asd_ctx* ctx, MatcherState* m, const TrackStage& s, bool fuse) {
   hipStream_t st = ctx->stream;
   const AsdFrameSlot& F = *s.F;
   int rc;
   if (s.upload == kUploadCopy) ASD_HIP_CHECK(ctx, ctx->up.upload(st));
-  if (s.source == kQueriesProject) {
-    const UploadTail& t = s.project.up;
-    hipLaunchKernelGGL(k_project_queries, dim3(t.q_blocks + (t.n16 ? kUploadTailBlocks : 0)), dim3(256), 0, st, s.project);
-    ASD_HIP_CHECK(ctx, hipGetLastError());
-  } else if (s.source == kQueriesFrustum) {
-    const UploadTail& t = s.frustum.up;
-    hipLaunchKernelGGL(k_frustum_queries, dim3(t.q_blocks + (t.n16 ? kUploadTailBlocks : 0)), dim3(256), 0, st, s.frustum);
-    ASD_HIP_CHECK(ctx, hipGetLastError());
-  }
   if (s.timed) ASD_HIP_CHECK(ctx, hipEventRecord(ctx->ev0, st));
   const GridDev G{F.d_kp, F.d_cell_start, F.d_cell_items, F.min_x, F.min_y, F.inv_w, F.inv_h};
   const SortArgs sa{s.d_occupied, s.kind == 0 ? TH_HIGH : __builtin_huge_valf(), s.d_top};
-  hipLaunchKernelGGL(k_window_search<true>, dim3((s.nq + kSearchWaves - 1) / kSearchWaves), dim3(64 * kSearchWaves), 0, st, G, s.d_queries, s.nq, s.d_qdesc, F.d_desc, s.d_off,
-                     s.d_cnt, s.d_total, m->cand_cap, m->d_idx, m->d_dist, sa);
+  const int q_blocks = search_blocks(s.nq);
+  auto search = [&](const auto& qa, int tail_blocks) {
+    hipLaunchKernelGGL((k_window_search<true, std::decay_t<decltype(qa)>>), dim3(q_blocks + tail_blocks), dim3(64 * kSearchWaves), 0, st, G, s.d_queries, s.nq, s.d_qdesc,
+                       F.d_desc, s.d_off, s.d_cnt, s.d_total, m->cand_cap, m->d_idx, m->d_dist, sa, qa);
+  };
+  if (s.source == kQueriesProject) search(s.project, s.project.up.n16 ? kUploadTailBlocks : 0);
+  else if (s.source == kQueriesFrustum) search(s.frustum, s.frustum.up.n16 ? kUploadTailBlocks : 0);
+  else search(TableQueries{}, 0);
   ASD_HIP_CHECK(ctx, hipGetLastError());
+  m->last_lists = LastLists{s.nq, true, s.d_off, s.d_cnt, s.d_top};
   Resolve2Args ra;
   const size_t lds = resolve2_args(m, s, &ra);
   if (!fuse) {
@@ -817,18 +870,17 @@
   TrackStage s{};
   s.kind = kind; s.nq = nq; s.F = &F;
   s.source = in.source;
-  s.upload = in.source != kQueriesUploaded && tail_upload ? kUploadCarried : kUploadCopy;
+  s.upload = in.source != kQueriesUploaded && tail_upload && kind == 0 ? kUploadCarried : kUploadCopy;
   s.d_qdesc = in.d_qdesc; s.kp_last = in.kp_last; s.check_ori = in.check_ori; s.nn_ratio = in.nn_ratio;
   s.d_off = m->d_q_off; s.d_cnt = m->d_q_off + nq;
   s.d_top = ctx->scratch.carve<uint16_t>((size_t)nq * kTop);
   s.timed = timing;
-  const size_t o_q = in.source == kQueriesUploaded ? up.add(m->h_queries, (size_t)nq * sizeof(WinQuery)) : up.reserve((size_t)nq * sizeof(WinQuery));
-  const size_t o_total = up.zeros(sizeof(int));
-  s.d_queries = up.dev<WinQuery>(o_q);
-  s.d_total = up.dev<int>(o_total);
+  if (in.source == kQueriesUploaded) s.d_queries = up.dev<WinQuery>(up.add(m->h_queries, (size_t)nq * sizeof(WinQuery)));
+  if ((rc = matcher_total(ctx, m)) != ASD_OK) return rc;
+  s.d_total = m->d_total;
+  const bool carried = s.upload == kUploadCarried;
   if (in.obs_pos) s.d_obs_pos = up.dev<uint8_t>(up.add(in.obs_pos, nq));
-  if (kind == 1) s.d_occupied = up.dev<uint8_t>(up.add(in.occupied, n_cur));
-  const bool carried = s.upload == kUploadCarried;
+  if (kind == 1) { const size_t o = up.add(in.occupied, n_cur); s.d_occupied = carried ? up.host<uint8_t>(o) : up.dev<uint8_t>(o); }
   const void *q_points = nullptr, *q_has = nullptr, *q_normal = nullptr, *q_min = nullptr, *q_max = nullptr, *q_rows = nullptr;
   auto table = [&](const void* src, size_t bytes, const void** for_query) -> const void* {
     if (!src) return nullptr;
@@ -848,14 +900,12 @@
   if (in.source == kQueriesProject) {
     s.project = in.project;
     s.project.Xw = static_cast<const float*>(q_points); s.project.has_mp = static_cast<const uint8_t*>(q_has); s.project.rows = static_cast<const int*>(q_rows);
-    s.project.queries = up.dev<WinQuery>(o_q);
     s.project.up = upload_tail(up, nq, carried);
   } else if (in.source == kQueriesFrustum) {
     s.frustum = in.frustum;
     s.frustum.Xw = static_cast<const float*>(q_points); s.frustum.normal = static_cast<const float*>(q_normal);
     s.frustum.min_dist = static_cast<const float*>(q_min); s.frustum.max_dist = static_cast<const float*>(q_max);
     s.frustum.rows = static_cast<const int*>(q_rows);
-    s.frustum.queries = up.dev<WinQuery>(o_q);
     s.frustum.up = upload_tail(up, nq, carried);
   }
   const size_t o_out = down.reserve(((size_t)n_cur + 16) * sizeof(int));
@@ -869,7 +919,6 @@
     v.io = down.host<double>(down.reserve(io_bytes));
     if (solver_io) *solver_io = v.io;
   }
-  int* const h_total = up.host<int>(o_total);
   const int* const h_out = s.h_out;
 
   auto attempt = [ctx, m, s]() -> int {
@@ -889,7 +938,6 @@
       }
       if (total > m->cand_cap && round == 0) {
         if ((rc = ensure_cands_dev(ctx, m, (size_t)total)) != ASD_OK) return rc;
-        *h_total = 0;
         if ((rc = attempt()) != ASD_OK) return rc;
         continue;
       }
@@ -934,7 +982,7 @@
   }
   if (ctx->matcher) {
     MatcherState* m = static_cast<MatcherState*>(ctx->matcher);
-    void* dev[] = {m->d_queries, m->d_q_off, m->d_idx, m->d_dist, m->d_qdesc, m->d_bank, m->d_attr};
+    void* dev[] = {m->d_queries, m->d_q_off, m->d_total, m->d_idx, m->d_dist, m->d_qdesc, m->d_bank, m->d_attr};
     for (void* p : dev) if (p) (void)hipFree(p);
     void* host[] = {m->h_queries, m->h_q, m->h_idx, m->h_dist, m->h_qdesc, m->h_attr[0], m->h_attr[1]};
     for (void* p : host) if (p) (void)hipHostFree(p);
@@ -1026,6 +1074,46 @@
   } else {
     ASD_HIP_CHECK(ctx, hipStreamSynchronize(st));
   }
+  return ASD_OK;
+}
+
+int32_t asd_debug_window_lists(asd_ctx* ctx, int32_t* nq, int32_t* sorted, int32_t q_cap, int32_t* q_cnt, int32_t* q_off, uint16_t* top_idx,
+                               int32_t list_cap, int32_t* idx, uint32_t* dist_bits, int64_t* n_list) {
+  if (!ctx || !nq || q_cap < 0 || list_cap < 0) return ASD_ERR_INVALID;
+  if (asd_track_busy(ctx, "asd_debug_window_lists")) return ASD_ERR_INVALID;
+  MatcherState* m = matcher_state(ctx);
+  const LastLists& L = m->last_lists;
+  if (!L.d_off) { ctx->set_error("asd_debug_window_lists: no window search has run on this context"); return ASD_ERR_INVALID; }
+  (void)hipSetDevice(ctx->cfg.device);
+  ASD_HIP_CHECK(ctx, hipStreamSynchronize(ctx->stream));
+  const int n = L.nq;
+  *nq = n;
+  if (sorted) *sorted = L.sorted;
+  std::vector<int> off(n), cnt(n);
+  std::vector<uint16_t> top((size_t)n * kTop, (uint16_t)0xffffu);
+  if (n > 0) {
+    ASD_HIP_CHECK(ctx, hipMemcpy(off.data(), L.d_off, (size_t)n * sizeof(int), hipMemcpyDeviceToHost));
+    ASD_HIP_CHECK(ctx, hipMemcpy(cnt.data(), L.d_cnt, (size_t)n * sizeof(int), hipMemcpyDeviceToHost));
+    if (L.d_top) ASD_HIP_CHECK(ctx, hipMemcpy(top.data(), L.d_top, (size_t)n * kTop * sizeof(uint16_t), hipMemcpyDeviceToHost));
+  }
+  const size_t n_buf = 2 * (size_t)m->cand_cap;
+  int64_t at = 0;
+  for (int q = 0; q < n; ++q) {
+    if (cnt[q] < 0 || (cnt[q] > 0 && (off[q] < 0 || (size_t)off[q] + (size_t)cnt[q] > n_buf))) {
+      ctx->set_error("asd_debug_window_lists: query %d has list [%d, +%d) outside the candidate buffers (%zu entries): the search overflowed them", q, off[q], cnt[q], n_buf);
+      return ASD_ERR_CAPACITY;
+    }
+    if (q < q_cap) {
+      if (q_cnt) q_cnt[q] = cnt[q];
+      if (q_off) q_off[q] = off[q];
+      if (top_idx) memcpy(top_idx + (size_t)q * kTop, top.data() + (size_t)q * kTop, kTop * sizeof(uint16_t));
+    }
+    const int take = (int)std::max<int64_t>(0, std::min<int64_t>(cnt[q], (int64_t)list_cap - at));
+    if (take > 0 && idx) ASD_HIP_CHECK(ctx, hipMemcpy(idx + at, m->d_idx + off[q], (size_t)take * sizeof(int), hipMemcpyDeviceToHost));
+    if (take > 0 && dist_bits) ASD_HIP_CHECK(ctx, hipMemcpy(dist_bits + at, m->d_dist + off[q], (size_t)take * sizeof(float), hipMemcpyDeviceToHost));
+    at += cnt[q];
+  }
+  if (n_list) *n_list = at;
   return ASD_OK;
 }
 
@@ -1538,8 +1626,8 @@
   float* d_cXw = ctx->scratch.carve<float>((size_t)ncand * 3);
   float* d_T1 = ctx->scratch.carve<float>(32);
   double* d_io1 = reinterpret_cast<double*>(ctx->scratch.carve<char>(io_bytes));
-  const size_t o_q1 = up.reserve((size_t)nl * sizeof(WinQuery));
-  s1.d_total = up.dev<int>(up.zeros(sizeof(int))); s2.d_total = up.dev<int>(up.zeros(sizeof(int)));
+  if ((rc = matcher_total(ctx, m)) != ASD_OK) return rc;
+  s1.d_total = s2.d_total = m->d_total;
   if (A.last_obs_positive) s1.d_obs_pos = up.dev<uint8_t>(up.add(A.last_obs_positive, nl));
   if (A.cand_obs_positive) s2.d_obs_pos = up.dev<uint8_t>(up.add(A.cand_obs_positive, ncand));
   const size_t o_has = up.add(A.has_mp, nl), o_Xw = up.add(A.Xw_last, (size_t)nl * 12), o_rows1 = up.add(A.last_rows, (size_t)nl * 4);
@@ -1560,9 +1648,7 @@
   s1.source = kQueriesProject; s1.upload = kUploadCarried;
   s1.project = project_args(ctx, *C, *L, A.Tcw, A.K, A.th);
   s1.project.Xw = up.host<float>(o_Xw); s1.project.has_mp = up.host<uint8_t>(o_has); s1.project.rows = up.host<int>(o_rows1);
-  s1.project.queries = up.dev<WinQuery>(o_q1);
   s1.project.up = upload_tail(up, nl, true);
-  s1.d_queries = up.dev<WinQuery>(o_q1);
   s1.kp_last = L->d_kp; s1.check_ori = A.check_orientation;
   s1.has_solver = true;
   s1.solver.d_points = up.dev<float>(o_Xw);
diff --git a/asd-slam_amd/csrc/resolve2.h b/asd-slam_amd/csrc/resolve2.h
--- a/asd-slam_amd/csrc/resolve2.h
+++ b/asd-slam_amd/csrc/resolve2.h
@@ -14,7 +14,7 @@
   int nq, n_cur;
   const int* q_off; const int* q_cnt; const int* idx; const float* dist;
   const uint16_t* top_idx;
-  const int* total; int cap;
+  int* total; int cap;
   const uint8_t* obs_pos;
   const float4* kp_cur;
   const float4* kp_last;
@@ -50,7 +50,8 @@
   const int total = *a.total;
   if (total > a.cap || total == 0) {
     for (int j = t; j < a.n_cur; j += NT) OUT(j, -1);
-    if (t == 0) { CNT(0, 0); CNT(1, total); CNT(2, 0); }
+    asd_syncthreads();
+    if (t == 0) { CNT(0, 0); CNT(1, total); CNT(2, 0); *a.total = 0; }
     return;
   }
   int cnt[QPT], pick[QPT], qoff[QPT];
@@ -327,7 +328,7 @@
     asd_syncthreads();
   }
   for (int j = t; j < a.n_cur; j += NT) OUT(j, last[j]);
-  if (t == 0) { CNT(0, (KIND == 1 ? 2 : 1) * n_written - n_removed); CNT(1, total); CNT(2, it + 1);
+  if (t == 0) { CNT(0, (KIND == 1 ? 2 : 1) * n_written - n_removed); CNT(1, total); CNT(2, it + 1); *a.total = 0;
     CNT(3, (int)(ts1 - ts0)); CNT(4, (int)(ts2 - ts1)); CNT(5, (int)(__builtin_amdgcn_s_memrealtime() - ts2)); CNT(6, (int)(ts_it0 - ts1));
     CNT(7, ph_work); CNT(8, ph_bar); CNT(9, (int)(ts0 & 0x7fffffffull)); CNT(10, (int)(__builtin_amdgcn_s_memrealtime() & 0x7fffffffull)); }
 }
diff --git a/asd-slam_amd/host/track_loop.cpp b/asd-slam_amd/host/track_loop.cpp
--- a/asd-slam_amd/host/track_loop.cpp
+++ b/asd-slam_amd/host/track_loop.cpp
@@ -76,6 +76,8 @@
   std::vector<double> ba_poses, ba_points, ba_chi2;
   std::vector<uint8_t> ba_dpos, ba_out1;
   double wait_ms = 0.0, ba_ms = 0.0;
+  double last_wait_ms = 0.0;
+  int ba_hold = 1;
   double ba_prep_ms = 0.0;
   double seg_ms[8] = {};
   double kern_ms[4] = {};
@@ -99,6 +101,7 @@
   memcpy(h->scale32, scale32, sizeof h->scale32);
   h->ba = *ba;
   h->kf_interval = kf_interval; h->lookahead = lookahead;
+  if (const char* e = getenv("ASD_TRACK_BA_HOLD")) asd_track_set_ba_hold(h, atoi(e));
   h->kps.resize(1 << 13);
   h->desc_sync.resize((size_t)(1 << 13) * 128);
   return h;
@@ -108,6 +111,7 @@
 void asd_track_set_async_ba(asd_track_handle* h, int32_t on) { if (h) h->async_ba = on != 0; }
 void asd_track_set_split(asd_track_handle* h, int32_t on) { if (h) h->split = on != 0; }
 void asd_track_set_chain(asd_track_handle* h, int32_t on) { if (h) h->chain = on != 0; }
+void asd_track_set_ba_hold(asd_track_handle* h, int32_t mode) { if (h && mode >= 0 && mode <= 2) h->ba_hold = mode; }
 void asd_track_set_map_copies(asd_track_handle* h, int32_t copies) {
   if (!h || copies < 1 || copies > 16 || copies == h->map_copies) return;
   h->map_copies = copies;
@@ -241,7 +245,8 @@
     const auto w0 = std::chrono::steady_clock::now();
     if ((rc = asd_extract_wait_view(ctx, &kps, &d, &n)) != ASD_OK) return rc;
     if (ctxr && (rc = asd_extract_wait_view(ctxr, &kps_r, &d, &n_r)) != ASD_OK) return rc;
-    h->wait_ms += std::chrono::duration<double, std::milli>(std::chrono::steady_clock::now() - w0).count();
+    h->last_wait_ms = std::chrono::duration<double, std::milli>(std::chrono::steady_clock::now() - w0).count();
+    h->wait_ms += h->last_wait_ms;
     h->pending.pop_front();
   } else {
     if ((rc = drop_pending()) != ASD_OK) return rc;
@@ -521,7 +526,8 @@
     const float* d = nullptr;
     const auto w0 = std::chrono::steady_clock::now();
     if ((rc = asd_extract_wait_view(ctx, &kps, &d, &n)) != ASD_OK) return rc;
-    h->wait_ms += std::chrono::duration<double, std::milli>(std::chrono::steady_clock::now() - w0).count();
+    h->last_wait_ms = std::chrono::duration<double, std::milli>(std::chrono::steady_clock::now() - w0).count();
+    h->wait_ms += h->last_wait_ms;
     h->pending.pop_front();
   } else {
     while (!h->pending.empty()) {
@@ -723,11 +729,12 @@
   memset(&h->ba_r, 0, sizeof h->ba_r);
   h->ba_r.edge_chi2 = h->ba_chi2.data(); h->ba_r.edge_depth_pos = h->ba_dpos.data(); h->ba_r.edge_outlier1 = h->ba_out1.data();
   h->ba_prep_ms += std::chrono::duration<double, std::milli>(std::chrono::steady_clock::now() - p0).count();
+  constexpr double kHoldReadyMs = 0.02;
   struct ExtractHold {
     asd_ctx *a, *b;
     ExtractHold(asd_ctx* a_, asd_ctx* b_, bool on) : a(on ? a_ : nullptr), b(on ? b_ : nullptr) { if (a) (void)asd_extract_hold(a, 1); if (b) (void)asd_extract_hold(b, 1); }
     ~ExtractHold() { if (a) (void)asd_extract_hold(a, 0); if (b) (void)asd_extract_hold(b, 0); }
-  } hold(ctx, h->ctx_r, !h->async_ba);
+  } hold(ctx, h->ctx_r, !h->async_ba && (h->ba_hold == 1 || (h->ba_hold == 2 && h->last_wait_ms < kHoldReadyMs)));
   if (h->dm && !h->async_ba && (rc = do_mapping_stage(h)) != ASD_OK) return rc;
   const auto b0 = std::chrono::steady_clock::now();
   if (h->async_ba) {
diff --git a/asd-slam_amd/host/track_loop.h b/asd-slam_amd/host/track_loop.h
--- a/asd-slam_amd/host/track_loop.h
+++ b/asd-slam_amd/host/track_loop.h
@@ -24,6 +24,7 @@
 void asd_track_set_async_ba(asd_track_handle* h, int32_t on);
 void asd_track_set_split(asd_track_handle* h, int32_t on);
 void asd_track_set_chain(asd_track_handle* h, int32_t on);
+void asd_track_set_ba_hold(asd_track_handle* h, int32_t mode);
 void asd_track_set_map_copies(asd_track_handle* h, int32_t copies);
 void asd_track_set_frames_on_host(asd_track_handle* h, int32_t on);
 int asd_track_set_stereo(asd_track_handle* h, asd_ctx* ctx_right, const void* const* d_frames_right, float mb, float mbf);
diff --git a/include/asd_slam.h b/include/asd_slam.h
--- a/include/asd_slam.h
+++ b/include/asd_slam.h
@@ -611,6 +611,9 @@
 
 int32_t asd_debug_bank_get(asd_ctx* ctx, int32_t first_row, int32_t n, float* desc, float* attr);
 
+int32_t asd_debug_window_lists(asd_ctx* ctx, int32_t* nq, int32_t* sorted, int32_t q_cap, int32_t* q_cnt, int32_t* q_off, uint16_t* top_idx,
+                               int32_t list_cap, int32_t* idx, uint32_t* dist_bits, int64_t* n_list);
+
 int asd_describe_timed(asd_ctx* ctx, const uint8_t* d_patches, int32_t n, float* d_desc,
                        int32_t reps, float* avg_ms);
 
```
